# neka-nat/cupoch

Measured on AMD Instinct MI355X. Metric: ICP iterations/sec (incl. kNN) on 10M-pt point-to-plane, 1/2/4/8 MI355X, higher is better.
Workload: dtype f32; 1 GPU; 10M-vs-10M point-to-plane ICP, radius 1-NN on an 8-ary kd-cell tree, r=2*N^(-1/3), uniform random clouds (BASELINE.md section 3); points=10000000, parallelism=single GPU, accumulate=f64

## Files before the change

cupoch_amd/_lib.py:

```python
import ctypes as C
import os
import shutil
import subprocess

_HERE = os.path.dirname(os.path.abspath(__file__))
ROOT = os.path.dirname(_HERE)
CSRC = os.path.join(_HERE, "csrc")
LIB_DIR = os.path.join(_HERE, "lib")
LIB_PATH = os.path.join(LIB_DIR, "libmi_icp.so")
INCLUDE = os.path.join(ROOT, "include")

HIPCC_FLAGS = ["--offload-arch=gfx950", "-O3", "-std=c++17", "-ffp-contract=off", "-fPIC", "-I/opt/rocm/include"]
UNITS = ["mi_icp", "mi_build", "mi_geometry", "mi_voxel", "mi_rgbd", "mi_tsdf", "mi_knn", "mi_comm", "mi_debug"]
OBJ_DIR = os.path.join(LIB_DIR, "obj")

MI_ICP_HOST, MI_ICP_DEVICE = 0, 1
EST_POINT_TO_POINT, EST_POINT_TO_PLANE, EST_SYMMETRIC, EST_GENERALIZED = 1, 2, 3, 5
EST_COLORED = 4


class MiIcpError(RuntimeError):
    pass


def _sources():
    return sorted(os.path.join(CSRC, f) for f in os.listdir(CSRC)
                  if f.endswith((".hip", ".h"))) + [os.path.join(INCLUDE, "mi_icp.h"),
                                                 os.path.join(INCLUDE, "mi_icp_debug.h")]


def needs_build():
    if not os.path.exists(LIB_PATH):
        return True
    t = os.path.getmtime(LIB_PATH)
    return any(os.path.getmtime(s) > t for s in _sources())


def build(force=False, verbose=False, variant=None, defines=()):
    lib_path = LIB_PATH if not variant else os.path.join(LIB_DIR, "libmi_icp_%s.so" % variant)
    obj_dir = OBJ_DIR if not variant else OBJ_DIR + "_" + variant
    if not force and not variant and not needs_build():
        return LIB_PATH
    hipcc = shutil.which("hipcc") or "/opt/rocm/bin/hipcc"
    if not os.path.exists(hipcc):
        raise MiIcpError("hipcc not found; cannot build libmi_icp.so")
    os.makedirs(obj_dir, exist_ok=True)
    import fcntl
    import hashlib
    with open(os.path.join(LIB_DIR, ".build.lock"), "w") as lock:
        fcntl.flock(lock, fcntl.LOCK_EX)
        try:
            if not force and not variant and not needs_build():
                return LIB_PATH
            return _build_locked(hipcc, lib_path, obj_dir, force, verbose, tuple(defines), hashlib)
        finally:
            fcntl.flock(lock, fcntl.LOCK_UN)


def _build_locked(hipcc, lib_path, obj_dir, force, verbose, defines, hashlib):
    headers = [s for s in _sources() if s.endswith(".h")]
    newest_header = max(os.path.getmtime(h) for h in headers)
    flags_hash = hashlib.sha1(" ".join(HIPCC_FLAGS + list(defines)).encode()).hexdigest()
    stamp = os.path.join(obj_dir, "flags.stamp")
    if not (os.path.exists(stamp) and open(stamp).read().strip() == flags_hash):
        force = True

    def compile_unit(u):
        src, obj = os.path.join(CSRC, u + ".hip"), os.path.join(obj_dir, u + ".o")
        if not force and os.path.exists(obj) and os.path.getmtime(obj) > max(newest_header, os.path.getmtime(src)):
            return obj
        tmp = "%s.tmp.%d" % (obj, os.getpid())
        cmd = [hipcc] + HIPCC_FLAGS + list(defines) + ["-c", src, "-o", tmp]
        if verbose:
            print(" ".join(cmd[:-1] + [obj]), flush=True)
        subprocess.check_call(cmd)
        os.replace(tmp, obj)
        return obj

    from concurrent.futures import ThreadPoolExecutor
    with ThreadPoolExecutor(max_workers=len(UNITS)) as pool:
        objs = list(pool.map(compile_unit, UNITS))
    with open(stamp + ".tmp", "w") as f:
        f.write(flags_hash + "\n")
    os.replace(stamp + ".tmp", stamp)
    tmp = "%s.tmp.%d" % (lib_path, os.getpid())
    cmd = [hipcc, "--offload-arch=gfx950", "-shared", "-fPIC"] + objs + ["-o", tmp]
    if verbose:
        print(" ".join(cmd), flush=True)
    subprocess.check_call(cmd)
    os.replace(tmp, lib_path)
    return lib_path


ITERATION_FN = C.CFUNCTYPE(None, C.c_void_p, C.c_int, C.c_float, C.c_float)


class Params(C.Structure):
    _fields_ = [("relative_fitness", C.c_float), ("relative_rmse", C.c_float),
                ("max_iteration", C.c_int32), ("det_thresh", C.c_float)]


class Result(C.Structure):
    _fields_ = [("transformation", C.c_float * 16), ("fitness", C.c_float),
                ("inlier_rmse", C.c_float), ("n_correspondences", C.c_int64),
                ("iterations", C.c_int32), ("nn_passes", C.c_int32)]


class OdometryOption(C.Structure):
    _fields_ = [("num_levels", C.c_int32), ("iterations", C.c_int32 * 8), ("max_depth_diff", C.c_float),
                ("min_depth", C.c_float), ("max_depth", C.c_float), ("nu", C.c_float), ("sigma2_init", C.c_float),
                ("inv_sigma_mat_diag", C.c_float * 6)]


_P, _I, _L, _F = C.c_void_p, C.c_int, C.c_int64, C.c_float
SIGNATURES = {
    "mi_icp_create": (_I, [_I, C.POINTER(_P)]),
    "mi_icp_destroy": (None, [_P]),
    "mi_icp_last_error": (C.c_char_p, [_P]),
    "mi_icp_version": (C.c_char_p, []),
    "mi_icp_set_stream": (_I, [_P, _P]),
    "mi_icp_synchronize": (_I, [_P]),
    "mi_icp_set_target": (_I, [_P, _P, _P, _P, _L, _I]),
    "mi_icp_set_source": (_I, [_P, _P, _P, _P, _L, _I]),
    "mi_icp_search_radius_1nn": (_I, [_P, _P, _F, _P, _P, _I, _P]),
    "mi_icp_get_correspondences": (_I, [_P, _P, _L, C.POINTER(_L), _I]),
    "mi_icp_set_correspondences": (_I, [_P, _P, _L, _I]),
    "mi_icp_compute_system": (_I, [_P, _I, _P, _P]),
    "mi_icp_compute_transformation": (_I, [_P, _I, _P, _F, _P]),
    "mi_icp_compute_rmse": (_I, [_P, _I, _P, C.POINTER(_F)]),
    "mi_icp_solve_system": (_I, [_P, _F, _P]),
    "mi_icp_kabsch_from_sums": (_I, [_P, _L, _P]),
    "mi_icp_vector6_to_matrix4": (None, [_P, _P]),
    "mi_icp_lzf_decompress": (_L, [_P, _L, _P, _L]),
    "mi_icp_lzf_compress": (_L, [_P, _L, _P, _L]),
    "mi_icp_evaluate_registration": (_I, [_P, _F, _P, C.POINTER(Result)]),
    "mi_icp_registration_icp": (_I, [_P, _I, _F, _P, C.POINTER(Params), C.POINTER(Result)]),
    "mi_icp_icp_begin": (_I, [_P, _I, _F, _P, _F, C.POINTER(Result)]),
    "mi_icp_icp_iterate": (_I, [_P, _I, C.POINTER(Result)]),
    "mi_icp_transform": (_I, [_P, _P, _P, _P, _P, _L, _I]),
    "mi_icp_compute_bounds": (_I, [_P, _P, _L, _I, _P, _P, _P]),
    "mi_icp_affine": (_I, [_P, _P, _F, _I, _P, _P, _P, _P, _P, _L, _I]),
    "mi_icp_voxel_downsample": (_I, [_P, _P, _P, _P, _L, _F, _P, _P, _P, C.POINTER(_L), _I]),
    "mi_icp_select_by_index": (_I, [_P, _P, _P, _P, _L, _P, _L, _I, _P, _P, _P, C.POINTER(_L), _I]),
    "mi_icp_select_by_mask": (_I, [_P, _P, _P, _P, _L, _P, _L, _I, _P, _P, _P, C.POINTER(_L), _I]),
    "mi_icp_uniform_downsample": (_I, [_P, _P, _P, _P, _L, _L, _P, _P, _P, C.POINTER(_L), _I]),
    "mi_icp_remove_statistical_outliers": (_I, [_P, _P, _P, _P, _L, _I, _F, _P, _P, _P, _P, _P, C.POINTER(_L), _I]),
    "mi_icp_remove_radius_outliers": (_I, [_P, _P, _P, _P, _L, _I, _F, _P, _P, _P, _P, _P, C.POINTER(_L), _I]),
    "mi_icp_cluster_dbscan": (_I, [_P, _P, _L, _F, _L, _I, _P, _P, C.POINTER(_L), _I]),
    "mi_icp_segment_plane": (_I, [_P, _P, _L, _F, _L, _L, C.c_uint64, _P, _P, _P, C.POINTER(_L), C.POINTER(_L), C.POINTER(_L), _I]),
    "mi_icp_iss_keypoints": (_I, [_P, _P, _L, _F, _F, _F, _F, _I, _I, _P, _P, _P, _P, _P, C.POINTER(_L), _I]),
    "mi_icp_farthest_point_downsample": (_I, [_P, _P, _P, _P, _L, _L, _P, _P, _P, _P, C.POINTER(_L), _I]),
    "mi_icp_pass_through_filter": (_I, [_P, _P, _P, _P, _L, _I, _F, _F, _P, _P, _P, _P, C.POINTER(_L), _I]),
    "mi_icp_crop_aabb": (_I, [_P, _P, _P, _P, _L, _P, _P, _P, _P, _P, _P, C.POINTER(_L), _I]),
    "mi_icp_remove_none_finite": (_I, [_P, _P, _P, _P, _L, _I, _I, _P, _P, _P, _P, C.POINTER(_L), _I]),
    "mi_icp_gaussian_filter": (_I, [_P, _P, _P, _P, _L, _F, _F, _I, _P, _P, _P, _I]),
    "mi_icp_create_from_depth": (_I, [_P, _P, _I, _P, _I, _I, _I, _P, _P, _F, _F, _F, _I, _I, _I, _I,
                                      _P, _P, _P, C.POINTER(_L), _I]),
    "mi_icp_compute_rgbd_odometry": (_I, [_P, _P, _P, _P, _P, _I, _I, _P, _P, _I, _P, C.POINTER(_I), _P, _P, _I]),
    "mi_icp_compute_weighted_rgbd_odometry": (_I, [_P, _P, _P, _P, _P, _I, _I, _P, _P, _P, _P, C.POINTER(_I), _P, _P, _P, _I]),
    "mi_icp_tsdf_create": (_I, [_P, _F, _I, _F, _I, _P, C.POINTER(_P)]),
    "mi_icp_tsdf_destroy": (_I, [_P, _P]),
    "mi_icp_tsdf_reset": (_I, [_P, _P]),
    "mi_icp_tsdf_integrate": (_I, [_P, _P, _P, _I, _I, _I, _I, _P, _I, _I, _I, _I, _I, _I, _P, _P, _I]),
    "mi_icp_tsdf_extract_point_cloud": (_I, [_P, _P, _P, _P, _P, _L, C.POINTER(_L), _I]),
    "mi_icp_tsdf_extract_voxel_point_cloud": (_I, [_P, _P, _P, _P, _L, C.POINTER(_L), _I]),
    "mi_icp_tsdf_raycast": (_I, [_P, _P, _I, _I, _P, _P, _F, _I, _P, _P, _P, _L, C.POINTER(_L), _I]),
    "mi_icp_tsdf_get_voxels": (_I, [_P, _P, _P, _P, _P, _I]),
    "mi_icp_covariances_from_normals": (_I, [_P, _P, _L, _F, _P, _I]),
    "mi_icp_estimate_normals_knn": (_I, [_P, _P, _L, _I, _P, _I]),
    "mi_icp_estimate_normals_radius": (_I, [_P, _P, _L, _F, _I, _P, _I]),
    "mi_icp_search_knn": (_I, [_P, _P, _L, _I, _F, _P, _P, C.POINTER(_L), _I]),
    "mi_icp_set_target_colors": (_I, [_P, _P, _I]),
    "mi_icp_set_source_colors": (_I, [_P, _P, _I]),
    "mi_icp_set_lambda_geometric": (_I, [_P, _F]),
    "mi_icp_compute_color_gradients": (_I, [_P, _F, _I, _P, _I]),
    "mi_icp_registration_colored_icp": (_I, [_P, _F, _P, C.POINTER(Params), _F, C.POINTER(Result)]),
    "mi_icp_comm_unique_id": (_I, [_P]),
    "mi_icp_comm_init": (_I, [_P, _P, _I, _I]),
    "mi_icp_comm_init_local": (_I, [_P, C.c_char_p, _I, _I]),
    "mi_icp_comm_kind": (_I, [_P]),
    "mi_icp_comm_autotune": (_I, [_P, _I, _P, _P]),
    "mi_icp_comm_destroy": (_I, [_P]),
    "mi_icp_set_global_source_count": (_I, [_P, _L]),
    "mi_icp_spatial_order": (_I, [_P, _P, _L, _P, _I]),
    "mi_icp_set_iteration_callback": (_I, [_P, _P, _P]),
    "mi_icp_set_profiling": (_I, [_P, _I]),
    "mi_icp_get_profile": (_I, [_P, _P]),
    "mi_icp_debug_sort_pairs": (_I, [_P, _P, _P, _L, _I]),
    "mi_icp_debug_exclusive_scan": (_I, [_P, _P, _P, _L, _P]),
    "mi_icp_debug_morton_order": (_I, [_P, _P, _L, _P]),
    "mi_icp_debug_nn_stats": (_I, [_P, _P, _F, _I, _P]),
    "mi_icp_debug_nn_stats8": (_I, [_P, _P, _F, _I, _P]),
    "mi_icp_debug_get_tree": (_I, [_P, C.POINTER(_L), _P, _P]),
    "mi_icp_debug_drop_seeds": (_I, [_P]),
    "mi_icp_debug_last_search_kind": (_I, [_P]),
    "mi_icp_debug_last_voxel_path": (_I, [_P]),
    "mi_icp_debug_occupancy": (_I, [_I]),
    "mi_icp_debug_loop_counters": (_I, [_P, _P]),
    "mi_icp_debug_search_skip": (_I, [_P, _P, _P, _L, C.POINTER(_L), C.POINTER(_I)]),
    "mi_icp_debug_locate": (_I, [_P, _P, _P]),
    "mi_icp_debug_set_step_stamps": (_I, [_P, _I]),
    "mi_icp_debug_get_step_stamps": (_I, [_P, _P, C.POINTER(C.c_double)]),
    "mi_icp_debug_solve_both": (_I, [_I, _P, _I, C.c_float, _P, _P, _P, _P]),
    "mi_icp_debug_get_leaf_regions": (_I, [_P, _P]),
    "mi_icp_debug_get_leaf_halos": (_I, [_P, _P]),
    "mi_icp_debug_eigen3": (_I, [_I, _P, _L, _P, _P, _P]),
    "mi_icp_debug_odometry_image": (_I, [_P, _I, _I, _P, C.POINTER(_I), C.POINTER(_I)]),
}

_lib = None


def load():
    global _lib
    if _lib is not None:
        return _lib
    override = os.environ.get("MI_ICP_LIB_PATH")
    path = override or LIB_PATH
    if not os.path.exists(path):
        raise MiIcpError(
            "libmi_icp.so is not built (%s). Run `python -c 'import __graft_entry__ as g; "
            "g.build()'` or cupoch_amd._lib.build(); there is no CPU fallback." % LIB_PATH)
    try:
        lib = C.CDLL(path, mode=C.RTLD_GLOBAL)
    except OSError as e:
        raise MiIcpError("cannot load %s: %s" % (path, e))
    for name, (res, args) in SIGNATURES.items():
        if override and name.startswith("mi_icp_debug_") and not hasattr(lib, name):
            continue
        fn = getattr(lib, name)
        fn.restype = res
        fn.argtypes = args
    _lib = lib
    return lib
```

cupoch_amd/csrc/ctx.h:

```cpp
#pragma once
#include <hip/hip_runtime.h>
#include <rccl/rccl.h>

#include <algorithm>
#include <cmath>
#include <cstdarg>
#include <cstdio>
#include <cstdlib>
#include <cstring>
#include <string>
#include <vector>

#include "../../include/mi_icp.h"
#include "../../include/mi_icp_debug.h"
#include "device_utils.h"
#include "host_solver.h"
#include "loop.h"
#include "loop_policy.h"
#include "mailbox.h"
#include "primitives.h"

namespace mi {
namespace eng {

using host::Mat4;

struct DevBuf {
    void* p = nullptr;
    size_t bytes = 0;
};

}
}

struct mi_icp_ctx {
    int device = 0;
    hipStream_t stream = nullptr;
    std::string err;

    int64_t nt = 0;
    int nleaf = 0;
    int64_t nts = 0;
    uint32_t leaf_first = 1, nrecords = 0;
    bool t_has_nrm = false, t_has_cov = false, t_has_int = false, t_has_grad = false, t_has_rec = false;
    mi::eng::DevBuf tblk, tnrm, trec, tcov, tgrad, nodes, inv_t, tidx, thalo, tlinks_tmp;
    mi::eng::DevBuf cell_planes, cell_samples, cell_cstart, cell_gstart, cell_boxes, cell_hist;
    mi::eng::DevBuf gplanes;
    int cell_levels = -1;
    uint32_t* cell_total_host = nullptr;
    bool inv_t_valid = false;
    bool links_ready = false, links_allowed = false;
    hipStream_t side = nullptr;
    hipEvent_t ev_fork = nullptr, ev_links = nullptr;
    bool links_inflight = false;
    int last_search_kind = -1;
    int last_voxel_path = -1;
    mi::eng::HaloPolicy halo;
    bool halo_use = false;
    mi::eng::DevBuf halo_want;

    int64_t ns = 0, ns_global = 0;
    bool s_has_nrm = false, s_has_cov = false, s_has_int = false;
    float lambda_geometric = 0.968f;
    mi::eng::DevBuf sx, sy, sz, sperm, snrm, scov, sint, nn_idx, nn_d2, inv_s;
    mi::eng::DevBuf alt[9];
    bool inv_s_valid = false;
    bool nn_valid = false;
    mi::eng::DevBuf expiry;
    bool expiry_live = false;
    float skip_r2 = NAN;
    mi::eng::DevBuf src_bounds;
    mi::eng::Relocation relocate;

    mi::eng::DevBuf user_pairs;
    int64_t n_user_pairs = -1;

    mi::eng::DevBuf keys0, keys1, vals0, vals1, hist, scan_tmp, bounds_part, bounds;
    mi::eng::DevBuf partial, sys_dev, dense_idx, flags, pairs_out, seg_start;
    mi::eng::DevBuf stage[6];
    mi::eng::DevBuf tscale;
    mi::eng::DevBuf knn_idx, knn_flags;
    mi::eng::DevBuf dbs[4];
    mi::eng::DevBuf seg[4];
    float vx_refused_voxel = 0.0f;
    int64_t vx_refused_n = 0;
    int vx_order = 0;
    mi::eng::DevBuf vx_tab;
    mi::eng::DevBuf vpay[6];
    double* sys_host = nullptr;
    float* f_host = nullptr;
    uint32_t* u_host = nullptr;
    void* od_host = nullptr;
    int od_levels = 0, od_lw[MI_ICP_ODOMETRY_MAX_LEVELS] = {}, od_lh[MI_ICP_ODOMETRY_MAX_LEVELS] = {};
    const float* od_img[MI_ICP_ODOMETRY_MAX_LEVELS][8] = {};

    mi::eng::DevBuf loop_dev, ticket;
    mi::DevLoop* loop_host = nullptr;
    bool loop_active = false;
    mi_icp_iteration_fn iter_fn = nullptr;
    void* iter_user = nullptr;
    mi::eng::DevBuf loop_hist;
    float* hist_host = nullptr;
    int iter_reported = 0;
    float loop_r2 = 0.0f;
    int loop_est = 0;

    ncclComm_t comm = nullptr;
    int nranks = 1, rank = 0;
    mi::MailBox* mail_host = nullptr;
    mi::MailBox* mail_dev = nullptr;
    size_t mail_bytes = 0;
    std::string mail_name;
    bool mail_linked = false;
    unsigned long long* inbox = nullptr;
    unsigned long long* inbox_peer[mi::kMailRanks] = {};
    mi::eng::DevBuf inbox_table;
    bool comm_broken = false;
    int xchg = 0;
    uint32_t tune_epoch = 0;
    mi::eng::DevBuf mail_state;

    mi_icp_ctx* aux = nullptr;

    std::vector<mi_icp_tsdf*> tsdf_volumes;

    mi::eng::DevBuf stamps;
    bool stamps_on = false;
    bool profiling = false;
    static constexpr int kEvPairs = 16;
    hipEvent_t ev[4] = {nullptr, nullptr, nullptr, nullptr};
    hipEvent_t evp[2][kEvPairs][2] = {};
    int evp_n[2] = {0, 0};
    bool ev_pending_nn = false, ev_pending_red = false;
    double prof[8] = {0, 0, 0, 0, 0, 0, 0, 0};
};

namespace mi {
namespace eng {

inline float* lreg_of(const mi_icp_ctx* c) { return c->tblk.p ? (float*)c->tblk.p + mi::kLeafRegOffset : nullptr; }

inline int fail(mi_icp_ctx* c, int code, const char* fmt, ...) {
    char buf[512];
    va_list ap;
    va_start(ap, fmt);
    vsnprintf(buf, sizeof(buf), fmt, ap);
    va_end(ap);
    if (c) c->err = buf;
    return code;
}

#define HIPCHK(c, expr)                                                                       \
    do {                                                                                      \
        hipError_t e_ = (expr);                                                               \
        if (e_ != hipSuccess)                                                                 \
            return fail((c), MI_ICP_ERR_HIP, "%s failed: %s (%s:%d)", #expr,                  \
                        hipGetErrorString(e_), __FILE__, __LINE__);                           \
    } while (0)

#define KCHK(c) HIPCHK(c, hipGetLastError())

#define TRY(expr)                \
    do {                         \
        int rc_ = (expr);        \
        if (rc_ != MI_ICP_OK) return rc_; \
    } while (0)

template <class T>
int ensure(mi_icp_ctx* c, DevBuf& b, size_t count, T** out) {
    const size_t bytes = std::max<size_t>(count * sizeof(T), 256);
    if (b.bytes < bytes) {
        if (b.p) {
            HIPCHK(c, hipStreamSynchronize(c->stream));
            HIPCHK(c, hipFree(b.p));
            b.p = nullptr;
            b.bytes = 0;
        }
        HIPCHK(c, hipMalloc(&b.p, bytes));
        b.bytes = bytes;
    }
    *out = (T*)b.p;
    return MI_ICP_OK;
}

inline void release(DevBuf& b) {
    if (b.p) (void)hipFree(b.p);
    b.p = nullptr;
    b.bytes = 0;
}

template <class T>
int to_device(mi_icp_ctx* c, const T* src, size_t count, int mem_kind, DevBuf& stage,
              const T** out) {
    if (!src || count == 0) {
        *out = nullptr;
        return MI_ICP_OK;
    }
    if (mem_kind == MI_ICP_DEVICE) {
        *out = src;
        return MI_ICP_OK;
    }
    T* d;
    TRY(ensure(c, stage, count, &d));
    HIPCHK(c, hipMemcpyAsync(d, src, count * sizeof(T), hipMemcpyHostToDevice, c->stream));
    *out = d;
    return MI_ICP_OK;
}

template <class T>
int out_slot(mi_icp_ctx* c, T* dst, size_t count, int mem_kind, DevBuf& stage, T** out) {
    if (!dst || mem_kind == MI_ICP_DEVICE) {
        *out = dst;
        return MI_ICP_OK;
    }
    return ensure(c, stage, count, out);
}

template <class T>
int from_device(mi_icp_ctx* c, const T* dev, T* dst, size_t count, int mem_kind) {
    if (!dst || dst == dev || count == 0) return MI_ICP_OK;
    HIPCHK(c, hipMemcpyAsync(dst, dev, count * sizeof(T),
                             mem_kind == MI_ICP_DEVICE ? hipMemcpyDeviceToDevice
                                                       : hipMemcpyDeviceToHost,
                             c->stream));
    return MI_ICP_OK;
}

inline int drop_expiry(mi_icp_ctx* c) {
    c->skip_r2 = NAN;
    if (c->expiry_live && c->expiry.p) HIPCHK(c, hipMemsetAsync(c->expiry.p, 0xff, c->expiry.bytes, c->stream));
    c->expiry_live = false;
    return MI_ICP_OK;
}

static_assert(sizeof(DevLoop::live) == kSkipSamples, "loop_policy.h skip_pays reads DevLoop::live[]");

inline int blocks_for(int64_t n, int per = 256) { return (int)std::max<int64_t>(1, (n + per - 1) / per); }

inline Xform make_xform(const Mat4& T) { return xform_from(T); }

inline Mat4 load_T(const float* T) {
    if (!T) return host::identity4();
    Mat4 m;
    std::memcpy(m.data(), T, sizeof(float) * 16);
    return m;
}

struct EvTimer {
    mi_icp_ctx* c;
    int slot;
    hipEvent_t stop = nullptr;
    bool pooled;
    EvTimer(mi_icp_ctx* ctx, int s, bool in_loop) : c(ctx), slot(s), pooled(in_loop) {
        if (!c->profiling) return;
        if (pooled) {
            if (c->evp_n[slot] >= mi_icp_ctx::kEvPairs) return;
            const int i = c->evp_n[slot]++;
            (void)hipEventRecord(c->evp[slot][i][0], c->stream);
            stop = c->evp[slot][i][1];
        } else {
            (void)hipEventRecord(c->ev[slot * 2], c->stream);
            stop = c->ev[slot * 2 + 1];
        }
    }
    ~EvTimer() {
        if (!stop) return;
        (void)hipEventRecord(stop, c->stream);
        if (!pooled) (slot == 0 ? c->ev_pending_nn : c->ev_pending_red) = true;
    }
};

inline void collect_events(mi_icp_ctx* c) {
    float ms = 0.0f;
    if (c->ev_pending_nn && hipEventElapsedTime(&ms, c->ev[0], c->ev[1]) == hipSuccess) {
        c->prof[0] += ms;
        c->prof[1] += 1;
    }
    if (c->ev_pending_red && hipEventElapsedTime(&ms, c->ev[2], c->ev[3]) == hipSuccess) {
        c->prof[2] += ms;
        c->prof[3] += 1;
    }
    c->ev_pending_nn = c->ev_pending_red = false;
}

inline void collect_pooled(mi_icp_ctx* c, int executed) {
    for (int slot = 0; slot < 2; ++slot) {
        for (int i = 0; i < c->evp_n[slot] && i < executed; ++i) {
            float ms = 0.0f;
            if (hipEventElapsedTime(&ms, c->evp[slot][i][0], c->evp[slot][i][1]) == hipSuccess) {
                c->prof[slot * 2] += ms;
                c->prof[slot * 2 + 1] += 1;
            }
        }
        c->evp_n[slot] = 0;
    }
}

inline bool mail_on(const mi_icp_ctx* c) { return c->mail_dev != nullptr && (c->xchg == 1 || c->xchg == 2); }

inline int check_ctx(mi_icp_ctx* c) {
    if (!c) return MI_ICP_ERR_INVALID;
    hipError_t e = hipSetDevice(c->device);
    if (e != hipSuccess) return fail(c, MI_ICP_ERR_HIP, "hipSetDevice(%d): %s", c->device, hipGetErrorString(e));
    return MI_ICP_OK;
}

inline int check_ctx(mi_icp_ctx* c, int mem_kind, const char* what) {
    TRY(check_ctx(c));
    if (mem_kind != MI_ICP_HOST && mem_kind != MI_ICP_DEVICE) return fail(c, MI_ICP_ERR_INVALID, "%s: bad mem_kind", what);
    return MI_ICP_OK;
}

inline int check_sizes(mi_icp_ctx* c, const char* what, int64_t n, int64_t* m, int mem_kind) {
    TRY(check_ctx(c, mem_kind, what));
    if (!m) return fail(c, MI_ICP_ERR_INVALID, "%s: m is null", what);
    *m = 0;
    if (n < 0 || n > 0x7fffff00ll) return fail(c, MI_ICP_ERR_INVALID, "%s: bad size", what);
    return MI_ICP_OK;
}

struct Cloud {
    const float* in[3];
    float* out[3];
};

inline int cloud_check(mi_icp_ctx* c, const char* what, const Cloud& a) {
    if (!a.in[0] || !a.out[0] || (a.in[1] && !a.out[1]) || (a.in[2] && !a.out[2]))
        return fail(c, MI_ICP_ERR_INVALID, "%s: null buffer", what);
    return MI_ICP_OK;
}

inline int cloud_upload(mi_icp_ctx* c, Cloud* a, int64_t n, int mem_kind, DevBuf* stage) {
    for (int k = 0; k < 3; ++k) TRY(to_device(c, a->in[k], (size_t)n * 3, mem_kind, stage[k], &a->in[k]));
    return MI_ICP_OK;
}

inline int cloud_in(mi_icp_ctx* c, const char* what, Cloud* a, int64_t n, int mem_kind, DevBuf* stage) {
    TRY(cloud_check(c, what, *a));
    return cloud_upload(c, a, n, mem_kind, stage);
}

inline int cloud_out(mi_icp_ctx* c, const float* const in[3], float* const out[3], int64_t count, int mem_kind,
                     DevBuf* stage, float* dst[3]) {
    for (int k = 0; k < 3; ++k) TRY(out_slot(c, in[k] ? out[k] : nullptr, (size_t)count * 3, mem_kind, stage[k], &dst[k]));
    return MI_ICP_OK;
}

inline int cloud_out_back(mi_icp_ctx* c, float* const dst[3], float* const out[3], int64_t m, int mem_kind) {
    for (int k = 0; k < 3; ++k)
        if (dst[k]) TRY(from_device(c, (const float*)dst[k], out[k], (size_t)m * 3, mem_kind));
    return MI_ICP_OK;
}

template <class Launch>
int cloud_emit(mi_icp_ctx* c, const float* const in[3], float* const out[3], int64_t count, int64_t m, int mem_kind,
               DevBuf* stage, Launch launch) {
    float* dst[3];
    TRY(cloud_out(c, in, out, count, mem_kind, stage, dst));
    launch(dst);
    KCHK(c);
    TRY(cloud_out_back(c, dst, out, m, mem_kind));
    HIPCHK(c, hipStreamSynchronize(c->stream));
    return MI_ICP_OK;
}

inline int scan_into(mi_icp_ctx* c, const uint32_t* flags, uint32_t* pos, int64_t n, const uint32_t** total) {
    uint32_t* tmp;
    TRY(ensure(c, c->scan_tmp, (size_t)scan_num_tiles(n) + 2, &tmp));
    exclusive_scan_u32(c->stream, flags, pos, n, tmp);
    KCHK(c);
    *total = tmp + scan_num_tiles(n);
    return MI_ICP_OK;
}

inline int scan_flags(mi_icp_ctx* c, const uint32_t* flags, int64_t n, uint32_t** pos, const uint32_t** total) {
    TRY(ensure(c, c->dense_idx, (size_t)n, pos));
    return scan_into(c, flags, *pos, n, total);
}

inline int read_total(mi_icp_ctx* c, const uint32_t* total, int slot = 0) {
    HIPCHK(c, hipMemcpyAsync(c->u_host + slot, total, sizeof(uint32_t), hipMemcpyDeviceToHost, c->stream));
    return MI_ICP_OK;
}

template <class Launch>
int cloud_emit_counted(mi_icp_ctx* c, const char* what, const uint32_t* flags, int64_t n, float* const out_all[3],
                       const bool (&want)[3], int64_t capacity, int64_t* m, int mem_kind, Launch launch) {
    uint32_t* pos;
    const uint32_t* total;
    TRY(scan_flags(c, flags, n, &pos, &total));
    TRY(read_total(c, total));
    HIPCHK(c, hipStreamSynchronize(c->stream));
    const int64_t cnt = (int64_t)c->u_host[0];
    *m = cnt;
    if (cnt == 0 || capacity < cnt) return MI_ICP_OK;
    float* out[3];
    for (int k = 0; k < 3; ++k) {
        if (want[k] && !out_all[k]) return fail(c, MI_ICP_ERR_INVALID, "%s: null buffer", what);
        out[k] = want[k] ? out_all[k] : nullptr;
    }
    return cloud_emit(c, out, out, cnt, cnt, mem_kind, c->vpay, [&](float* const dst[3]) { launch(pos, dst); });
}

template <class Body>
int in_scratch(mi_icp_ctx* c, const char* what, Body body) {
    if (!c->aux) {
        const int rc = mi_icp_create(c->device, &c->aux);
        if (rc != MI_ICP_OK) return fail(c, rc, "%s: cannot create the scratch context", what);
    }
    mi_icp_ctx* a = c->aux;
    a->stream = c->stream;
    const int rc = body(a);
    if (rc != MI_ICP_OK) return fail(c, rc, "%s: %s", what, a->err.c_str());
    return MI_ICP_OK;
}

int compute_bounds(mi_icp_ctx* c, const float* pts, int64_t n, float** bounds_out);
int sort_buffers(mi_icp_ctx* c, int64_t n, SortBuffers* sb);
int morton_order(mi_icp_ctx* c, const float* pts, int64_t n, const uint32_t** order, const float* grid_bounds = nullptr,
                 int grid_bits = 0, float** own_bounds = nullptr);
int ensure_links(mi_icp_ctx* c);
int start_links_async(mi_icp_ctx* c);
bool halo_poll(mi_icp_ctx* c);
int drain_links(mi_icp_ctx* c);
void release_links_scratch(mi_icp_ctx* c);
int resort_source_by_match(mi_icp_ctx* c);
int occupancy_build(int which);
int launch_nn(mi_icp_ctx* c, const Mat4& T, float r2, bool seed, unsigned long long* stats = nullptr,
              const DevLoop* loop = nullptr);
int occupancy_loop(int which);
bool planes_available(const mi_icp_ctx* c);
int launch_locate_by_planes(mi_icp_ctx* c, const Xform& X, const DevLoop* loop, int gated);
int occupancy_geometry(int which);
void tsdf_release_all(mi_icp_ctx* c);
int compact_by_flags(mi_icp_ctx* c, const uint32_t* flags, int64_t n, const float* const in[3], float* const out[3],
                     int64_t* out_idx, int mem_kind, const uint32_t* status, int64_t* m, uint32_t* status_out);
MailArgs mail_args(const mi_icp_ctx* c);
void mailbox_close(mi_icp_ctx* c);
int comm_failed(mi_icp_ctx* c, const char* what);
int comm_usable(mi_icp_ctx* c);
int allreduce_system(mi_icp_ctx* c);
void comm_release(mi_icp_ctx* c);

}
}
```

cupoch_amd/csrc/mi_build.hip:

```cpp
#include "ctx.h"
#include "kd_build.h"
#include "kd_cells.h"
#include "kd_planes.h"
#include "kd_refine.h"
#include "lbvh.h"
#include "leaf_halo.h"

using namespace mi;
using namespace mi::eng;
using host::Mat4;

namespace mi {
namespace eng {

int morton_bits_for(int64_t n) {
    int lg = 0;
    while ((1ll << lg) < n) ++lg;
    const int per_axis = (lg + 2) / 3;
    const int fine = std::min(21, std::max(6, per_axis + 2));
    const int coarse = (((3 * fine + 7) / 8 - 1) * 8) / 3;
    return coarse >= std::max(6, per_axis) ? coarse : fine;
}

int compute_bounds(mi_icp_ctx* c, const float* pts, int64_t n, float** bounds_out) {
// ... 129 lines not shown
    if (ngroups <= 0 || ngroups > (int64_t)ncells + n / kKdGroup + 1)
        return fail(c, MI_ICP_ERR_HIP, "kd cell layout: implausible group count %lld", (long long)ngroups);
    out->vals = sb.vals[cur];
    out->cstart = cstart;
    out->gstart = gstart;
    out->ncells = ncells;
    out->ngroups = ngroups;
    out->planes = planes;
    out->levels = lv;
    return MI_ICP_OK;
}

int build_links(mi_icp_ctx* c, hipStream_t st) {
    if (!c->links_allowed) return MI_ICP_OK;
    float* halo;
    const size_t ntiles = ((size_t)c->nleaf + 63) / 64;
    TRY(ensure(c, c->thalo, ntiles * 64 * kHaloLines * kHaloLineFloats, &halo));
    uint2* cand;
    TRY(ensure(c, c->tlinks_tmp, ntiles * 64 * kLinkCand, &cand));
    const uint32_t lblocks = (uint32_t)ntiles;
    leaf_halo_collect<<<((lblocks + 7u) / 8u) * 8u, 64, 0, st>>>(
            (const float*)c->nodes.p, c->leaf_first, c->nleaf, lblocks, lreg_of(c), cand);
    KCHK(c);
    leaf_halo_build<<<(unsigned)(((size_t)c->nleaf + kHaloTile - 1) / kHaloTile), 64, 0, st>>>(lreg_of(c), c->nleaf, cand, (const float*)c->tblk.p, halo);
    KCHK(c);
    return MI_ICP_OK;
}

int ensure_links(mi_icp_ctx* c) {
    if (c->nt <= 0) return MI_ICP_OK;
    if (c->links_inflight) {
        HIPCHK(c, hipStreamWaitEvent(c->stream, c->ev_links, 0));
        c->links_inflight = false;
        c->links_ready = true;
    }
    if (c->links_ready) return MI_ICP_OK;
    TRY(build_links(c, c->stream));
    c->links_ready = true;
    return MI_ICP_OK;
}

void release_links_scratch(mi_icp_ctx* c) {
    constexpr size_t kKeepBelow = (size_t)64 << 20;
    if (c->links_ready && !c->links_inflight && c->tlinks_tmp.p && c->tlinks_tmp.bytes >= kKeepBelow) release(c->tlinks_tmp);
}

bool halo_poll(mi_icp_ctx* c) {
    if (c->links_inflight && hipEventQuery(c->ev_links) == hipSuccess) {
        c->links_inflight = false;
        c->links_ready = true;
    }
    (void)hipGetLastError();
    return c->links_ready && c->links_allowed && c->thalo.p != nullptr;
}

int start_links_async(mi_icp_ctx* c) {
    if (c->nt <= 0 || c->links_ready || c->links_inflight || !c->links_allowed) return MI_ICP_OK;
    HIPCHK(c, hipEventRecord(c->ev_fork, c->stream));
    HIPCHK(c, hipStreamWaitEvent(c->side, c->ev_fork, 0));
    TRY(build_links(c, c->side));
    HIPCHK(c, hipEventRecord(c->ev_links, c->side));
    c->links_inflight = true;
    return MI_ICP_OK;
}

int drain_links(mi_icp_ctx* c) {
    if (c->links_inflight) {
        HIPCHK(c, hipStreamWaitEvent(c->stream, c->ev_links, 0));
        HIPCHK(c, hipStreamSynchronize(c->side));
        c->links_inflight = false;
    }
    c->links_ready = false;
    return MI_ICP_OK;
}

int resort_source_by_match(mi_icp_ctx* c) {
    const int64_t n = c->ns;
    if (n <= 0 || c->nt <= 0 || !c->nn_valid) return MI_ICP_OK;
    TRY(drop_expiry(c));
    SortBuffers sb;
    TRY(sort_buffers(c, n, &sb));
    int bits = 1;
    while (bits < 32 && (1ull << bits) <= (uint64_t)c->nleaf) ++bits;
    match_order_keys<<<blocks_for(n), 256, 0, c->stream>>>((const int32_t*)c->nn_idx.p, (int)n, (uint32_t)c->nleaf,
                                                           (uint32_t*)sb.keys[0], sb.vals[0]);
    KCHK(c);
    const uint32_t* ord = sb.vals[radix_sort_pairs<uint32_t>(c->stream, sb, n, bits)];
    KCHK(c);
    SourceArrays in, out;
    in.sx = (float*)c->sx.p; in.sy = (float*)c->sy.p; in.sz = (float*)c->sz.p;
    in.sperm = (int32_t*)c->sperm.p;
    in.snrm = c->s_has_nrm ? (float4*)c->snrm.p : nullptr;
    in.scov = c->s_has_cov ? (float*)c->scov.p : nullptr;
    in.sint = c->s_has_int ? (float*)c->sint.p : nullptr;
    in.nn_idx = (int32_t*)c->nn_idx.p; in.nn_d2 = (float*)c->nn_d2.p;
    TRY(ensure(c, c->alt[0], (size_t)n, &out.sx));
    TRY(ensure(c, c->alt[1], (size_t)n, &out.sy));
    TRY(ensure(c, c->alt[2], (size_t)n, &out.sz));
    TRY(ensure(c, c->alt[3], (size_t)n, &out.sperm));
    TRY(ensure(c, c->alt[4], (size_t)n, &out.nn_idx));
    TRY(ensure(c, c->alt[5], (size_t)n, &out.nn_d2));
    out.snrm = nullptr;
    out.scov = nullptr;
    out.sint = nullptr;
    if (in.snrm) TRY(ensure(c, c->alt[6], (size_t)n, &out.snrm));
    if (in.scov) TRY(ensure(c, c->alt[7], (size_t)n * 9, &out.scov));
    if (in.sint) TRY(ensure(c, c->alt[8], (size_t)n, &out.sint));
    permute_source<<<blocks_for(n), 256, 0, c->stream>>>(ord, (int)n, in, out);
    KCHK(c);
    std::swap(c->sx, c->alt[0]);
    std::swap(c->sy, c->alt[1]);
    std::swap(c->sz, c->alt[2]);
    std::swap(c->sperm, c->alt[3]);
    std::swap(c->nn_idx, c->alt[4]);
    std::swap(c->nn_d2, c->alt[5]);
    if (in.snrm) std::swap(c->snrm, c->alt[6]);
    if (in.scov) std::swap(c->scov, c->alt[7]);
    if (in.sint) std::swap(c->sint, c->alt[8]);
    c->inv_s_valid = false;
    return MI_ICP_OK;
}

int occupancy_build(int which) {
    int blocks = -1;
    hipError_t e = hipErrorInvalidValue;
    if (which == 0) e = hipOccupancyMaxActiveBlocksPerMultiprocessor(&blocks, kd_build_groups, kKdThreads, 0);
    else if (which == 4) e = hipOccupancyMaxActiveBlocksPerMultiprocessor(&blocks, leaf_halo_build, 64, 0);
    else return -1;
    return e == hipSuccess ? blocks : -2;
}

}
}

extern "C" {

int mi_icp_set_target(mi_icp_ctx* c, const float* xyz, const float* normals, const float* covs,
                      int64_t n, int mem_kind) {
    TRY(check_ctx(c, mem_kind, "set_target"));
    if (n < 0 || n > 0x7fffff00ll || (n > 0 && !xyz)) return fail(c, MI_ICP_ERR_INVALID, "set_target: bad size/pointer");
    TRY(drain_links(c));
    TRY(drop_expiry(c));
    c->nt = 0;
    c->inv_t_valid = false;
    c->nn_valid = false;
    c->n_user_pairs = -1;
    c->loop_active = false;
    c->t_has_nrm = normals != nullptr && n > 0;
    c->t_has_cov = covs != nullptr && n > 0;
    c->t_has_int = c->t_has_grad = false;
    c->t_has_rec = false;
    if (n == 0) return MI_ICP_OK;
    hipEvent_t e0 = c->ev[2], e1 = c->ev[3];
    if (c->profiling) {
        (void)hipStreamSynchronize(c->stream);
        collect_events(c);
        (void)hipEventRecord(e0, c->stream);
    }

    const float *d_pts, *d_nrm, *d_cov;
    TRY(to_device(c, xyz, (size_t)n * 3, mem_kind, c->stage[0], &d_pts));
    TRY(to_device(c, normals, (size_t)n * 3, mem_kind, c->stage[1], &d_nrm));
    TRY(to_device(c, covs, (size_t)n * 9, mem_kind, c->stage[2], &d_cov));

    CellLayout lay;
    TRY(kd_cell_layout(c, d_pts, n, &lay));
    const int64_t nts = lay.ngroups * kKdGroup;

    const int nleaf = (int)((nts + kLeaf - 1) / kLeaf);
    int levels = 1;
    uint32_t leaf_first = 1u;
    while ((uint64_t)leaf_first * 8u < (uint64_t)nleaf) {
        leaf_first *= 8u;
        ++levels;
    }
    if (levels > kMaxLevels) return fail(c, MI_ICP_ERR_INVALID, "set_target: cloud too large for the 64-bit traversal stack");
    const uint32_t used_last = (uint32_t)((nleaf + 7) / 8);
    const uint32_t nrecords = full_levels_below(leaf_first) + used_last;
    if ((uint64_t)nrecords * kRecordFloats * sizeof(float) >= (1ull << 32))
        return fail(c, MI_ICP_ERR_INVALID, "set_target: cloud too large for 32-bit record offsets");
    float* tblk;
    float4* tnrm = nullptr;
    float* tcov = nullptr;
    float* nodes;
    TRY(ensure(c, c->tblk, (size_t)nleaf * kLeafFloats, &tblk));
    TRY(ensure(c, c->nodes, (size_t)nrecords * kRecordFloats, &nodes));
    float* lreg = tblk + kLeafRegOffset;
    int32_t* tidx;
    TRY(ensure(c, c->tidx, (size_t)nleaf * kLeaf, &tidx));
    float* trec = nullptr;
    if (d_nrm) TRY(ensure(c, c->tnrm, (size_t)nts, &tnrm));
    if (d_nrm) TRY(ensure(c, c->trec, (size_t)nts * 6, &trec));
    c->t_has_rec = trec != nullptr;
    if (d_cov) TRY(ensure(c, c->tcov, (size_t)nts * 9, &tcov));
    const uint32_t upper_flag = (lay.ngroups == (int64_t)lay.ncells) ? 1u : 0u;
    GroupBuildArgs ga;
    ga.pts = d_pts;
    ga.nrm = d_nrm;
    ga.cov = d_cov;
    ga.vals = lay.vals;
    ga.cstart = lay.cstart;
    ga.gstart = lay.gstart;
    ga.ncells = lay.ncells;
    ga.planes = lay.planes;
    ga.cell_levels = lay.levels;
    ga.ngroups = (uint32_t)lay.ngroups;
    ga.leaf_first = leaf_first;
    ga.tblk = tblk;
    ga.tnrm = tnrm;
    ga.trec = trec;
    ga.tcov = tcov;
    ga.records = nodes;
    ga.lreg = lreg;
    ga.tidx = tidx;
    TRY(ensure(c, c->gplanes, (size_t)lay.ngroups * 512, &ga.gplanes));
    ga.link_delta = 0.25f;
    ga.region_margin = 0.5f;
    kd_build_groups<<<(unsigned)lay.ngroups, kKdThreads, 0, c->stream>>>(ga);
    KCHK(c);
    uint32_t first = leaf_first >> 9;
    uint32_t used = ((uint32_t)lay.ngroups + 7u) / 8u;
    int above_groups = 1;
    for (; first > 1u; first /= 8u, ++above_groups) {
        const uint32_t count = ((used + 7u) / 8u) * 8u;
        const int region_depth = cell_depth(lay.levels) - 3 * above_groups;
        const uint32_t flag = (upper_flag && (!cell_tri(lay.levels) || region_depth >= 2)) ? 1u : 0u;
        build_level<<<blocks_for(count), 256, 0, c->stream>>>(nodes, first, used, count, flag, lay.planes,
                                                              lay.levels, region_depth);
        KCHK(c);
        used = (used + 7u) / 8u;
    }
    {
        float* ts;
        TRY(ensure(c, c->tscale, 4, &ts));
        HIPCHK(c, hipMemsetAsync(ts, 0, 16, c->stream));
        tree_scale<<<std::min(256u, (used_last + 255u) / 256u), 256, 0, c->stream>>>(nodes, leaf_first, used_last, ts);
        KCHK(c);
    }
    c->links_ready = false;
    c->halo.on_new_target();
    c->links_allowed = (uint32_t)nleaf <= kLinkIdMask;
    c->nt = n;
    c->nts = nts;
    c->nleaf = nleaf;
    c->leaf_first = leaf_first;
    c->nrecords = nrecords;
    c->cell_levels = lay.levels;
    if (c->halo.start_ahead(n, c->links_allowed)) TRY(start_links_async(c));
    if (c->profiling) {
        (void)hipEventRecord(e1, c->stream);
        (void)hipStreamSynchronize(c->stream);
        float ms = 0;
        if (hipEventElapsedTime(&ms, e0, e1) == hipSuccess) c->prof[4] = ms;
    }
    return MI_ICP_OK;
}

int mi_icp_set_source(mi_icp_ctx* c, const float* xyz, const float* normals, const float* covs,
                      int64_t n, int mem_kind) {
    TRY(check_ctx(c, mem_kind, "set_source"));
    if (n < 0 || n > 0x7fffff00ll || (n > 0 && !xyz)) return fail(c, MI_ICP_ERR_INVALID, "set_source: bad size/pointer");
    c->ns = 0;
    c->inv_s_valid = false;
    c->nn_valid = false;
    c->n_user_pairs = -1;
    c->loop_active = false;
    c->s_has_nrm = normals != nullptr && n > 0;
    c->s_has_cov = covs != nullptr && n > 0;
    c->s_has_int = false;
    if (c->nranks == 1) c->ns_global = 0;
    if (n == 0) return MI_ICP_OK;
    hipEvent_t e0 = c->ev[2], e1 = c->ev[3];
    if (c->profiling) {
        (void)hipStreamSynchronize(c->stream);
        collect_events(c);
        (void)hipEventRecord(e0, c->stream);
    }

    const float *d_pts, *d_nrm, *d_cov;
    TRY(to_device(c, xyz, (size_t)n * 3, mem_kind, c->stage[3], &d_pts));
    TRY(to_device(c, normals, (size_t)n * 3, mem_kind, c->stage[4], &d_nrm));
    TRY(to_device(c, covs, (size_t)n * 9, mem_kind, c->stage[5], &d_cov));

    const uint32_t* order;
    float* own_bounds = nullptr;
    TRY(morton_order(c, d_pts, n, &order, nullptr, 0, &own_bounds));
    {
        float* sb;
        TRY(ensure(c, c->src_bounds, 8, &sb));
        HIPCHK(c, hipMemcpyAsync(sb, own_bounds, 8 * sizeof(float), hipMemcpyDeviceToDevice, c->stream));
    }

    float *sx, *sy, *sz, *scov = nullptr, *d2;
    int32_t *sperm, *idx;
    float4* snrm = nullptr;
    TRY(ensure(c, c->sx, (size_t)n, &sx));
    TRY(ensure(c, c->sy, (size_t)n, &sy));
    TRY(ensure(c, c->sz, (size_t)n, &sz));
    TRY(ensure(c, c->sperm, (size_t)n, &sperm));
    TRY(ensure(c, c->nn_idx, (size_t)n, &idx));
    TRY(ensure(c, c->nn_d2, (size_t)n, &d2));
    {
        double* lim;
        TRY(ensure(c, c->expiry, (size_t)((n + 63) / 64), &lim));
        c->expiry_live = true;
        TRY(drop_expiry(c));
    }
    if (d_nrm) TRY(ensure(c, c->snrm, (size_t)n, &snrm));
    if (d_cov) TRY(ensure(c, c->scov, (size_t)n * 9, &scov));
    gather_source<<<blocks_for(n), 256, 0, c->stream>>>(order, d_pts, d_nrm, d_cov, (int)n, sx, sy, sz,
                                                        sperm, snrm, scov);
    KCHK(c);
    c->ns = n;
    if (c->profiling) {
        (void)hipEventRecord(e1, c->stream);
        (void)hipStreamSynchronize(c->stream);
        float ms = 0;
        if (hipEventElapsedTime(&ms, e0, e1) == hipSuccess) c->prof[5] = ms;
    }
    return MI_ICP_OK;
}

int mi_icp_spatial_order(mi_icp_ctx* c, const float* xyz, int64_t n, uint32_t* order_out, int mem_kind) {
    TRY(check_ctx(c, mem_kind, "spatial_order"));
    if (n < 0 || n > 0x7fffff00ll || (n > 0 && (!xyz || !order_out)))
        return fail(c, MI_ICP_ERR_INVALID, "spatial_order: bad arguments");
    if (n == 0) return MI_ICP_OK;
    const float* d_pts;
    TRY(to_device(c, xyz, (size_t)n * 3, mem_kind, c->stage[0], &d_pts));
    const uint32_t* order;
    TRY(morton_order(c, d_pts, n, &order));
    TRY(from_device(c, order, order_out, (size_t)n, mem_kind));
    HIPCHK(c, hipStreamSynchronize(c->stream));
    return MI_ICP_OK;
}

int mi_icp_debug_morton_order(mi_icp_ctx* c, const float* xyz, int64_t n, uint32_t* order_out) {
    if (n <= 0) return fail(c, MI_ICP_ERR_INVALID, "debug_morton_order: bad arguments");
    return mi_icp_spatial_order(c, xyz, n, order_out, MI_ICP_HOST);
}

}
```

cupoch_amd/csrc/mi_debug.hip:

```cpp
#include "ctx.h"
#include <vector>
#include "halo_format.h"
#include "traverse.h"
#include "wave_solver.h"
#include "eigen3.h"

using namespace mi;
using namespace mi::eng;
using host::Mat4;

namespace mi {
__global__ __launch_bounds__(64) void solve_both_kernel(const double* systems, float det_thresh, float* out_serial,
                                                        float* out_wave, int32_t* ok_serial, int32_t* ok_wave) {
    __shared__ double s_sys[32];
    const int n = (int)blockIdx.x;
    if (threadIdx.x < 32) s_sys[threadIdx.x] = systems[(int64_t)n * 32 + threadIdx.x];
    __syncthreads();
    host::Mat4 W;
    const bool okw = wave_solve_system(s_sys, det_thresh, W);
    if (threadIdx.x < 16) out_wave[(int64_t)n * 16 + threadIdx.x] = select16(W.m, (int)threadIdx.x);
    if (threadIdx.x == 0) {
        ok_wave[n] = okw ? 1 : 0;
        host::Mat4 S;
        ok_serial[n] = host::solve_system(s_sys, det_thresh, S) ? 1 : 0;
        for (int e = 0; e < 16; ++e) out_serial[(int64_t)n * 16 + e] = S.m[e];
    }
}
__host__ __device__ inline void eigen3_one(const float* A9, float* eval, float* evec, float* S) {
    M3 A;
    for (int r = 0; r < 3; ++r)
        for (int c = 0; c < 3; ++c) A.m[r][c] = A9[r * 3 + c];
    float ev[3], e[3][3], s[3][3];
    fast_eigen3x3(A, ev, e);
    gicp_weight(A, s);
    for (int k = 0; k < 3; ++k) {
        if (eval) eval[k] = ev[k];
        for (int d = 0; d < 3; ++d) {
            if (evec) evec[d * 3 + k] = e[k][d];
            if (S) S[k * 3 + d] = s[k][d];
        }
    }
}
__global__ __launch_bounds__(256) void eigen3_kernel(const float* A, int64_t n, float* eval, float* evec, float* S) {
    const int64_t i = (int64_t)blockIdx.x * blockDim.x + threadIdx.x;
    if (i < n) eigen3_one(A + 9 * i, eval ? eval + 3 * i : nullptr, evec ? evec + 9 * i : nullptr, S ? S + 9 * i : nullptr);
}
}

extern "C" {

int mi_icp_debug_sort_pairs(mi_icp_ctx* c, uint64_t* keys, uint32_t* vals, int64_t n, int key_bits) {
    TRY(check_ctx(c));
    if (n < 0 || key_bits < 1 || key_bits > 64 || (n > 0 && (!keys || !vals)))
        return fail(c, MI_ICP_ERR_INVALID, "debug_sort_pairs: bad arguments");
    if (n == 0) return MI_ICP_OK;
    SortBuffers sb;
    TRY(sort_buffers(c, n, &sb));
    HIPCHK(c, hipMemcpyAsync(sb.keys[0], keys, (size_t)n * 8, hipMemcpyHostToDevice, c->stream));
    HIPCHK(c, hipMemcpyAsync(sb.vals[0], vals, (size_t)n * 4, hipMemcpyHostToDevice, c->stream));
    const int cur = radix_sort_pairs<uint64_t>(c->stream, sb, n, key_bits);
    KCHK(c);
    HIPCHK(c, hipMemcpyAsync(keys, sb.keys[cur], (size_t)n * 8, hipMemcpyDeviceToHost, c->stream));
    HIPCHK(c, hipMemcpyAsync(vals, sb.vals[cur], (size_t)n * 4, hipMemcpyDeviceToHost, c->stream));
    HIPCHK(c, hipStreamSynchronize(c->stream));
    return MI_ICP_OK;
}

int mi_icp_debug_exclusive_scan(mi_icp_ctx* c, const uint32_t* in, uint32_t* out, int64_t n,
                                uint64_t* total) {
    TRY(check_ctx(c));
    if (n < 0 || (n > 0 && (!in || !out))) return fail(c, MI_ICP_ERR_INVALID, "debug_exclusive_scan: bad arguments");
    if (total) *total = 0;
    if (n == 0) return MI_ICP_OK;
    uint32_t* d;
    const uint32_t* sum;
    TRY(ensure(c, c->flags, (size_t)n, &d));
    HIPCHK(c, hipMemcpyAsync(d, in, (size_t)n * 4, hipMemcpyHostToDevice, c->stream));
    TRY(scan_into(c, d, d, n, &sum));
    HIPCHK(c, hipMemcpyAsync(out, d, (size_t)n * 4, hipMemcpyDeviceToHost, c->stream));
    TRY(read_total(c, sum));
    HIPCHK(c, hipStreamSynchronize(c->stream));
    if (total) *total = c->u_host[0];
    return MI_ICP_OK;
}

int mi_icp_debug_nn_stats8(mi_icp_ctx* c, const float* T, float radius, int use_seed, uint64_t* out8) {
    TRY(check_ctx(c));
    if (!out8 || c->ns <= 0 || c->nt <= 0) return fail(c, MI_ICP_ERR_INVALID, "debug_nn_stats: bad state/arguments");
    unsigned long long* d;
    TRY(ensure(c, c->flags, 16, (unsigned long long**)&d));
    HIPCHK(c, hipMemsetAsync(d, 0, 16 * sizeof(unsigned long long), c->stream));
    TRY(launch_nn(c, load_T(T), radius * radius, use_seed != 0, d));
    HIPCHK(c, hipMemcpyAsync(c->sys_host, d, 16 * sizeof(unsigned long long), hipMemcpyDeviceToHost, c->stream));
    HIPCHK(c, hipStreamSynchronize(c->stream));
    collect_events(c);
    std::memcpy(out8, c->sys_host, 8 * sizeof(uint64_t));
    return MI_ICP_OK;
}

int mi_icp_debug_nn_stats(mi_icp_ctx* c, const float* T, float radius, int use_seed, uint64_t* out4) {
    uint64_t all[8];
    if (!out4) return MI_ICP_ERR_INVALID;
    TRY(mi_icp_debug_nn_stats8(c, T, radius, use_seed, all));
    std::memcpy(out4, all, 4 * sizeof(uint64_t));
    return MI_ICP_OK;
}

int mi_icp_debug_get_leaf_regions(mi_icp_ctx* c, float* regions_out) {
    TRY(check_ctx(c));
    if (!regions_out || c->nt <= 0) return fail(c, MI_ICP_ERR_INVALID, "debug_get_leaf_regions: no target / bad arguments");
    HIPCHK(c, hipMemcpy2DAsync(regions_out, kLeafRegFloats * sizeof(float), lreg_of(c), kLeafRegStride * sizeof(float),
                               kLeafRegFloats * sizeof(float), (size_t)c->nleaf, hipMemcpyDeviceToHost, c->stream));
    HIPCHK(c, hipStreamSynchronize(c->stream));
    return MI_ICP_OK;
}

int mi_icp_debug_get_leaf_halos(mi_icp_ctx* c, float* halos_out) {
    TRY(check_ctx(c));
    if (!halos_out || c->nt <= 0) return fail(c, MI_ICP_ERR_INVALID, "debug_get_leaf_halos: no target / bad arguments");
    TRY(ensure_links(c));
    const size_t count = (size_t)c->nleaf * kHaloLines * kHaloLineFloats;
    if (!c->thalo.p) {
        std::memset(halos_out, 0, count * sizeof(float));
        return MI_ICP_OK;
    }
    HIPCHK(c, hipMemcpyAsync(halos_out, c->thalo.p, count * sizeof(float), hipMemcpyDeviceToHost, c->stream));
    HIPCHK(c, hipStreamSynchronize(c->stream));
    return MI_ICP_OK;
}

int mi_icp_debug_last_search_kind(const mi_icp_ctx* c) { return c ? c->last_search_kind : -1; }
int mi_icp_debug_last_voxel_path(const mi_icp_ctx* c) { return c ? c->last_voxel_path : -1; }

int mi_icp_debug_occupancy(int which) {
    if (which == 0 || which == 4) return occupancy_build(which);
    if (which >= 1 && which <= 3) return occupancy_loop(which);
    if (which >= 5 && which <= 8) return occupancy_geometry(which);
    return -1;
}

int mi_icp_debug_solve_both(int device, const double* systems, int n, float det_thresh, float* out_serial,
                            float* out_wave, int32_t* ok_serial, int32_t* ok_wave) {
    if (!systems || n <= 0 || !out_serial || !out_wave || !ok_serial || !ok_wave) return MI_ICP_ERR_INVALID;
    if (hipSetDevice(device) != hipSuccess) return MI_ICP_ERR_NO_DEVICE;
    double* d_sys = nullptr;
    float* d_out = nullptr;
    int32_t* d_ok = nullptr;
    int rc = MI_ICP_ERR_HIP;
    if (hipMalloc(&d_sys, (size_t)n * 32 * sizeof(double)) == hipSuccess &&
        hipMalloc(&d_out, (size_t)n * 32 * sizeof(float)) == hipSuccess &&
        hipMalloc(&d_ok, (size_t)n * 2 * sizeof(int32_t)) == hipSuccess &&
        hipMemcpy(d_sys, systems, (size_t)n * 32 * sizeof(double), hipMemcpyHostToDevice) == hipSuccess) {
        mi::solve_both_kernel<<<n, 64>>>(d_sys, det_thresh, d_out, d_out + (size_t)n * 16, d_ok, d_ok + n);
        if (hipDeviceSynchronize() == hipSuccess &&
            hipMemcpy(out_serial, d_out, (size_t)n * 16 * sizeof(float), hipMemcpyDeviceToHost) == hipSuccess &&
            hipMemcpy(out_wave, d_out + (size_t)n * 16, (size_t)n * 16 * sizeof(float), hipMemcpyDeviceToHost) == hipSuccess &&
            hipMemcpy(ok_serial, d_ok, (size_t)n * sizeof(int32_t), hipMemcpyDeviceToHost) == hipSuccess &&
            hipMemcpy(ok_wave, d_ok + n, (size_t)n * sizeof(int32_t), hipMemcpyDeviceToHost) == hipSuccess)
            rc = MI_ICP_OK;
    }
    (void)hipFree(d_sys);
    (void)hipFree(d_out);
    (void)hipFree(d_ok);
    return rc;
}

int mi_icp_debug_set_step_stamps(mi_icp_ctx* c, int enable) {
    TRY(check_ctx(c));
    c->stamps_on = enable != 0;
    return MI_ICP_OK;
}

int mi_icp_debug_get_step_stamps(mi_icp_ctx* c, uint64_t* out32, double* ticks_per_us) {
    TRY(check_ctx(c));
    if (!out32 || !c->stamps.p) return fail(c, MI_ICP_ERR_STATE, "debug_get_step_stamps: no stamped loop has run on this context");
    HIPCHK(c, hipStreamSynchronize(c->stream));
    HIPCHK(c, hipMemcpy(out32, c->stamps.p, sizeof(uint64_t) * kStampWords, hipMemcpyDeviceToHost));
    if (ticks_per_us) {
        int khz = 0;
        *ticks_per_us = (hipDeviceGetAttribute(&khz, hipDeviceAttributeWallClockRate, c->device) == hipSuccess && khz > 0) ? khz / 1000.0 : 100.0;
    }
    return MI_ICP_OK;
}

int mi_icp_debug_loop_counters(mi_icp_ctx* c, int32_t* out4) {
    TRY(check_ctx(c));
    if (!out4 || !c->loop_host) return fail(c, MI_ICP_ERR_INVALID, "debug_loop_counters: bad arguments");
    HIPCHK(c, hipStreamSynchronize(c->stream));
    out4[0] = c->loop_host->iterations;
    out4[1] = c->loop_host->passes;
    out4[2] = c->loop_host->relocations;
    out4[3] = c->relocate.armed ? 1 : 0;
    return MI_ICP_OK;
}

int mi_icp_debug_drop_seeds(mi_icp_ctx* c) {
    TRY(check_ctx(c));
    c->nn_valid = false;
    return drop_expiry(c);
}

int mi_icp_debug_search_skip(mi_icp_ctx* c, double* state2, double* limits_out, int64_t capacity, int64_t* npackets, int* armed) {
    TRY(check_ctx(c));
    if (!state2 || !npackets || !armed || capacity < 0) return fail(c, MI_ICP_ERR_INVALID, "debug_search_skip: bad arguments");
    if (!c->loop_active || !c->loop_dev.p || !c->expiry.p || c->ns <= 0)
        return fail(c, MI_ICP_ERR_STATE, "debug_search_skip: no registration loop on this context");
    const int64_t n = (c->ns + 63) / 64;
    *npackets = n;
    *armed = (c->expiry_live && c->skip_r2 == c->loop_r2 && skip_pays(c->loop_host->live, c->ns)) ? 1 : 0;
    const char* st = (const char*)c->loop_dev.p;
    HIPCHK(c, hipMemcpyAsync(state2, st + offsetof(DevLoop, travel), sizeof(double), hipMemcpyDeviceToHost, c->stream));
    HIPCHK(c, hipMemcpyAsync(state2 + 1, st + offsetof(DevLoop, fuzz), sizeof(double), hipMemcpyDeviceToHost, c->stream));
    if (limits_out && capacity >= n)
        HIPCHK(c, hipMemcpyAsync(limits_out, c->expiry.p, (size_t)n * sizeof(double), hipMemcpyDeviceToHost, c->stream));
    HIPCHK(c, hipStreamSynchronize(c->stream));
    return MI_ICP_OK;
}

int mi_icp_debug_locate(mi_icp_ctx* c, const float* T, int32_t* leaf_out) {
    TRY(check_ctx(c));
    if (!leaf_out || c->ns <= 0 || c->nt <= 0) return fail(c, MI_ICP_ERR_INVALID, "debug_locate: bad state/arguments");
    if (!planes_available(c)) return fail(c, MI_ICP_ERR_INVALID, "debug_locate: this tree has no split planes");
    TRY(drop_expiry(c));
    TRY(launch_locate_by_planes(c, make_xform(load_T(T)), nullptr, 0));
    c->nn_valid = true;
    c->n_user_pairs = -1;
    std::vector<int32_t> seeds((size_t)c->ns), perm((size_t)c->ns);
    HIPCHK(c, hipMemcpyAsync(seeds.data(), c->nn_idx.p, sizeof(int32_t) * (size_t)c->ns, hipMemcpyDeviceToHost, c->stream));
    HIPCHK(c, hipMemcpyAsync(perm.data(), c->sperm.p, sizeof(int32_t) * (size_t)c->ns, hipMemcpyDeviceToHost, c->stream));
    HIPCHK(c, hipStreamSynchronize(c->stream));
    for (int64_t i = 0; i < c->ns; ++i) leaf_out[perm[(size_t)i]] = seeds[(size_t)i] >> 3;
    return MI_ICP_OK;
}

int mi_icp_debug_get_tree(mi_icp_ctx* c, int64_t* info5, float* records_out, float* leaf_lines_out) {
    TRY(check_ctx(c));
    if (!info5 || c->nt <= 0) return fail(c, MI_ICP_ERR_INVALID, "debug_get_tree: no target / bad arguments");
    info5[0] = c->nts;
    info5[1] = c->nleaf;
    info5[2] = (int64_t)c->leaf_first;
    info5[3] = (int64_t)c->nrecords;
    info5[4] = c->nt;
    if (records_out)
        HIPCHK(c, hipMemcpyAsync(records_out, c->nodes.p, (size_t)c->nrecords * kRecordFloats * sizeof(float),
                                 hipMemcpyDeviceToHost, c->stream));
    if (leaf_lines_out) {
        HIPCHK(c, hipMemcpyAsync(leaf_lines_out, c->tblk.p, (size_t)c->nleaf * kLeafFloats * sizeof(float),
                                 hipMemcpyDeviceToHost, c->stream));
        HIPCHK(c, hipMemcpy2DAsync(leaf_lines_out + kLeafRegOffset, kLeafFloats * sizeof(float), c->tidx.p, kLeaf * sizeof(int32_t),
                                   kLeaf * sizeof(int32_t), (size_t)c->nleaf, hipMemcpyDeviceToHost, c->stream));
    }
    HIPCHK(c, hipStreamSynchronize(c->stream));
    return MI_ICP_OK;
}

int mi_icp_debug_odometry_image(mi_icp_ctx* c, int level, int which, float* out, int* width, int* height) {
    TRY(check_ctx(c));
    if (c->od_levels <= 0) return fail(c, MI_ICP_ERR_INVALID, "debug_odometry_image: no odometry call has run on this context");
    if (level < 0 || level >= c->od_levels || which < 0 || which > 7)
        return fail(c, MI_ICP_ERR_INVALID, "debug_odometry_image: level %d / image %d out of range", level, which);
    if (width) *width = c->od_lw[level];
    if (height) *height = c->od_lh[level];
    if (!out) return MI_ICP_OK;
    const size_t n = (size_t)c->od_lw[level] * c->od_lh[level];
    HIPCHK(c, hipMemcpyAsync(out, c->od_img[level][which], n * sizeof(float), hipMemcpyDeviceToHost, c->stream));
    HIPCHK(c, hipStreamSynchronize(c->stream));
    return MI_ICP_OK;
}

int mi_icp_debug_eigen3(int device, const float* A, int64_t n, float* eval, float* evec, float* S) {
    if (n < 0 || (n > 0 && !A)) return MI_ICP_ERR_INVALID;
    if (n == 0) return MI_ICP_OK;
    if (device < 0) {
        for (int64_t i = 0; i < n; ++i)
            eigen3_one(A + 9 * i, eval ? eval + 3 * i : nullptr, evec ? evec + 9 * i : nullptr, S ? S + 9 * i : nullptr);
        return MI_ICP_OK;
    }
    if (hipSetDevice(device) != hipSuccess) return MI_ICP_ERR_NO_DEVICE;
    float *dA = nullptr, *de = nullptr, *dv = nullptr, *dS = nullptr;
    int rc = MI_ICP_ERR_HIP;
    if (hipMalloc(&dA, (size_t)n * 36) == hipSuccess && hipMalloc(&de, (size_t)n * 12) == hipSuccess &&
        hipMalloc(&dv, (size_t)n * 36) == hipSuccess && hipMalloc(&dS, (size_t)n * 36) == hipSuccess &&
        hipMemcpy(dA, A, (size_t)n * 36, hipMemcpyHostToDevice) == hipSuccess) {
        hipLaunchKernelGGL(eigen3_kernel, dim3((unsigned)((n + 255) / 256)), dim3(256), 0, 0, dA, n, de, dv, dS);
        bool ok = hipDeviceSynchronize() == hipSuccess;
        if (ok && eval) ok = hipMemcpy(eval, de, (size_t)n * 12, hipMemcpyDeviceToHost) == hipSuccess;
        if (ok && evec) ok = hipMemcpy(evec, dv, (size_t)n * 36, hipMemcpyDeviceToHost) == hipSuccess;
        if (ok && S) ok = hipMemcpy(S, dS, (size_t)n * 36, hipMemcpyDeviceToHost) == hipSuccess;
        if (ok) rc = MI_ICP_OK;
    }
    (void)hipFree(dA);
    (void)hipFree(de);
    (void)hipFree(dv);
    (void)hipFree(dS);
    return rc;
}

}
```

cupoch_amd/csrc/mi_icp.hip:

```cpp
#include "ctx.h"
#include "fused_small.h"
#include "lzf.h"
#include "nn_search.h"
#include "reduce.h"

using namespace mi;
using namespace mi::eng;
using host::Mat4;

namespace mi {

static __global__ __launch_bounds__(kStepThreads) void loop_step_kernel(DevLoop* st_g, double* sys_in, int resume, MailArgs mail) {
    __shared__ DevLoop st_s;
    loop_step_block(st_g, sys_in, resume, st_s, StepPre{false, 0u, 0.0, 0u}, mail);
}

namespace eng {

constexpr int64_t kPt2PlTwoFrom = (int64_t)4 << 20;

static int64_t coarse_first_min() {
    static const int64_t v = [] { const char* s = std::getenv("MI_ICP_COARSE_MIN"); return s ? std::atoll(s) : (int64_t)1 << 16; }();
    return v;
}

bool planes_available(const mi_icp_ctx* c) {
    return c->cell_levels >= 0 && c->gplanes.p != nullptr && c->cell_planes.p != nullptr && c->cell_gstart.p != nullptr &&
           c->leaf_first > 1u && c->nleaf > 0;
}

int launch_locate_by_planes(mi_icp_ctx* c, const Xform& X, const DevLoop* loop, int gated) {
    const int grid = (int)std::min<int64_t>(blocks_for(c->ns), 8192);
    locate_by_planes<<<grid, 256, 0, c->stream>>>((const float*)c->sx.p, (const float*)c->sy.p, (const float*)c->sz.p, (int)c->ns,
                                                 (const float2*)c->cell_planes.p, c->cell_levels, (const uint32_t*)c->cell_gstart.p,
                                                 (const float2*)c->gplanes.p, (uint32_t)c->nleaf, X, loop, gated, (int32_t*)c->nn_idx.p,
                                                 (double*)c->expiry.p);
    KCHK(c);
    return MI_ICP_OK;
}

static int loop_halo(mi_icp_ctx* c, bool* have_halo, uint32_t** want) {
    static const bool always_wait = std::getenv("MI_ICP_WAIT_LINKS") != nullptr;
    if (always_wait) {
        TRY(start_links_async(c));
        TRY(ensure_links(c));
        c->halo_use = halo_poll(c);
    }
    *have_halo = c->halo_use;
    *want = (!*have_halo && !c->links_inflight && c->links_allowed) ? (uint32_t*)c->halo_want.p : nullptr;
    return MI_ICP_OK;
}

struct PacketGrid { uint32_t npackets, nblocks, grid; };
static PacketGrid packet_grid(int64_t ns, uint32_t per_block) {
    const uint32_t npackets = (uint32_t)((ns + 63) / 64);
    const uint32_t nblocks = (npackets + per_block - 1) / per_block;
    return PacketGrid{npackets, nblocks, ((nblocks + 7u) / 8u) * 8u};
}

static decltype(&nn_packet_kernel<false, false>) nn_kernel(bool seeded, bool stats, bool stamp, bool gate) {
    if (gate) return stamp ? nn_packet_kernel<true, false, true, true> : nn_packet_kernel<true, false, false, true>;
    if (stats) return seeded ? nn_packet_kernel<true, true> : nn_packet_kernel<false, true>;
    if (seeded && stamp) return nn_packet_kernel<true, false, true>;
    return seeded ? nn_packet_kernel<true, false> : nn_packet_kernel<false, false>;
}

int launch_nn(mi_icp_ctx* c, const Mat4& T, float r2, bool seed, unsigned long long* stats, const DevLoop* loop) {
    if (c->ns <= 0) return MI_ICP_OK;
    int32_t* idx = (int32_t*)c->nn_idx.p;
    if (c->nt <= 0) {
        TRY(drop_expiry(c));
        fill_i32<<<blocks_for(c->ns), 256, 0, c->stream>>>(idx, c->ns, -1);
        KCHK(c);
        c->nn_valid = true;
        c->n_user_pairs = -1;
        return MI_ICP_OK;
    }
    const Xform X = make_xform(T);
    bool have_halo;
    uint32_t* want = nullptr;
    if (loop) {
        TRY(loop_halo(c, &have_halo, &want));
    } else {
        if (seed && c->nn_valid) TRY(ensure_links(c));
        have_halo = halo_poll(c);
    }
    EvTimer t(c, 0, loop != nullptr);
    const SearchPlan p = plan_search(loop != nullptr, seed, c->nn_valid, stats != nullptr, c->ns, coarse_first_min(), have_halo, planes_available(c),
                                     c->expiry.p != nullptr, c->expiry_live, c->skip_r2, r2, c->loop_host->live, kSkipRun);
    if (!p.may_skip) TRY(drop_expiry(c));
    if (p.self_seeded) TRY(launch_locate_by_planes(c, X, loop, 0));
    c->last_search_kind = p.kind;
    const PacketGrid g = packet_grid(c->ns, p.run);
    nn_kernel(p.use_seed || p.self_seeded, stats != nullptr, loop && c->stamps_on, p.run > 1u)<<<g.grid, kNNThreads, 0, c->stream>>>(
            (const float*)c->sx.p, (const float*)c->sy.p, (const float*)c->sz.p, (int)c->ns, (const float*)c->nodes.p,
            (const float*)c->tblk.p, (const float*)lreg_of(c), have_halo ? (const float*)c->thalo.p : nullptr, c->leaf_first,
            X, loop, r2, g.nblocks, idx, loop ? nullptr : (float*)c->nn_d2.p, stats, want,
            p.limits ? (double*)c->expiry.p : nullptr,
            p.limits ? reinterpret_cast<uint8_t*>(c->loop_dev.p) + offsetof(DevLoop, live) : nullptr, skip_live_shift(c->ns), p.run);
    KCHK(c);
    if (p.limits) c->expiry_live = true, c->skip_r2 = r2;
    c->nn_valid = true;
    c->n_user_pairs = -1;
    return MI_ICP_OK;
}

int occupancy_loop(int which) {
    int blocks = -1;
    hipError_t e = hipErrorInvalidValue;
    if (which == 1) e = hipOccupancyMaxActiveBlocksPerMultiprocessor(&blocks, nn_packet_kernel<true, false>, kNNThreads, 0);
    else if (which == 2) e = hipOccupancyMaxActiveBlocksPerMultiprocessor(&blocks, nn_packet_kernel<false, false>, kNNThreads, 0);
    else if (which == 3) e = hipOccupancyMaxActiveBlocksPerMultiprocessor(&blocks, reduce_pt2pl_kernel<2, 1>, kReduceThreads, 0);
    else return -1;
    return e == hipSuccess ? blocks : -2;
}

}
}

namespace {

int ensure_inverse_maps(mi_icp_ctx* c) {
    if (!c->inv_s_valid && c->ns > 0) {
        int32_t* inv;
        TRY(ensure(c, c->inv_s, (size_t)c->ns, &inv));
        invert_perm_source<<<blocks_for(c->ns), 256, 0, c->stream>>>((const int32_t*)c->sperm.p, (int)c->ns, inv);
        KCHK(c);
        c->inv_s_valid = true;
    }
    if (!c->inv_t_valid && c->nt > 0) {
        int32_t* inv;
        TRY(ensure(c, c->inv_t, (size_t)c->nt, &inv));
        HIPCHK(c, hipMemsetAsync(inv, 0xff, sizeof(int32_t) * (size_t)c->nt, c->stream));
        invert_perm_target<<<blocks_for(c->nts), 256, 0, c->stream>>>((const int32_t*)c->tidx.p, (int)c->nts, inv);
        KCHK(c);
        c->inv_t_valid = true;
    }
    return MI_ICP_OK;
}

constexpr int kReduceElemsPerThread = 16;


bool known_estimator(int est) {
    return est == kEstP2P || est == kEstPt2Pl || est == kEstSym || est == kEstColored || est == kEstGICP;
}

bool estimator_ready(const mi_icp_ctx* c, int est) {
    switch (est) {
        case kEstP2P: return true;
        case kEstPt2Pl: return c->t_has_nrm;
        case kEstSym: return c->t_has_nrm && c->s_has_nrm;
        case kEstGICP: return c->t_has_cov && c->s_has_cov;
        case kEstColored:
            return c->t_has_nrm && c->t_has_int && c->t_has_grad && c->s_has_int;
        default: return false;
    }
}

int reduce_buffers(mi_icp_ctx* c, size_t rows, double** partial, double** sys, uint32_t** ticket) {
    TRY(ensure(c, c->partial, rows * kSysSize, partial));
    TRY(ensure(c, c->sys_dev, kSysSize, sys));
    if (!c->ticket.p) {
        TRY(ensure(c, c->ticket, 64, ticket));
        HIPCHK(c, hipMemsetAsync(*ticket, 0, 256, c->stream));
    }
    *ticket = (uint32_t*)c->ticket.p;
    return MI_ICP_OK;
}

bool pt2pl_reduction(const mi_icp_ctx* c, int est, int mode) {
    return est == kEstPt2Pl && mode == 0 && estimator_ready(c, est) && c->n_user_pairs < 0 && c->t_has_rec &&
           c->trec.p != nullptr && c->ns > 0 && c->nt > 0 && c->nn_valid;
}

template <int kU>
decltype(&reduce_pt2pl_kernel<kU, 0>) pt2pl_kernel(int step, bool stamp) {
    if (step == 2) return stamp ? reduce_pt2pl_kernel<kU, 2, true> : reduce_pt2pl_kernel<kU, 2>;
    if (step == 1) return stamp ? reduce_pt2pl_kernel<kU, 1, true> : reduce_pt2pl_kernel<kU, 1>;
    return reduce_pt2pl_kernel<kU, 0>;
}

template <int MODE>
decltype(&reduce_kernel<kEstP2P, MODE>) generic_reduce_kernel(int est) {
    switch (est) {
        case kEstP2P: return reduce_kernel<kEstP2P, MODE>;
        case kEstPt2Pl: return reduce_kernel<kEstPt2Pl, MODE>;
        case kEstSym: return reduce_kernel<kEstSym, MODE>;
        case kEstColored: return reduce_kernel<kEstColored, MODE>;
        case kEstGICP: return reduce_kernel<kEstGICP, MODE>;
        default: return nullptr;
    }
}

int launch_reduce(mi_icp_ctx* c, int est, int mode, const Mat4& T, DevLoop* loop = nullptr, int step = 0) {
    double *partial, *sys;
    uint32_t* ticket;
    TRY(reduce_buffers(c, kReduceBlocks, &partial, &sys, &ticket));
    ReduceArgs a;
    a.sx = (const float*)c->sx.p;
    a.sy = (const float*)c->sy.p;
    a.sz = (const float*)c->sz.p;
    a.snrm = (const float4*)c->snrm.p;
    a.scov = (const float*)c->scov.p;
    a.tblk = (const float*)c->tblk.p;
    a.tnrm = (const float4*)c->tnrm.p;
    a.trec = c->t_has_rec ? (const float*)c->trec.p : nullptr;
    a.tcov = (const float*)c->tcov.p;
    a.tgrad = (const float4*)c->tgrad.p;
    a.sint = (const float*)c->sint.p;
    a.sqrt_lambda_geometric = std::sqrt(c->lambda_geometric);
    a.sqrt_lambda_photometric = std::sqrt(1.0f - c->lambda_geometric);
    a.nn_idx = (const int32_t*)c->nn_idx.p;
    a.pairs = nullptr;
    a.inv_s = a.inv_t = nullptr;
    a.ns = (int)c->ns;
    a.nt = (int)c->nt;
    a.count = c->ns;
    if (c->n_user_pairs >= 0) {
        TRY(ensure_inverse_maps(c));
        a.pairs = (const int32_t*)c->user_pairs.p;
        a.inv_s = (const int32_t*)c->inv_s.p;
        a.inv_t = (const int32_t*)c->inv_t.p;
        a.count = c->n_user_pairs;
    }
    if (c->ns <= 0 || c->nt <= 0 || (!a.pairs && !c->nn_valid)) a.count = 0;
    const int64_t wide = std::min<int64_t>(256, blocks_for(a.count, kReduceThreads));
    const int grid = (int)std::max<int64_t>(
            wide, std::min<int64_t>(kReduceBlocks, blocks_for(a.count, kReduceThreads * kReduceElemsPerThread)));
    const Xform X = make_xform(T);
    if (pt2pl_reduction(c, est, mode)) {
        const auto kernel = (a.count >= kPt2PlTwoFrom) ? pt2pl_kernel<2>(step, c->stamps_on) : pt2pl_kernel<4>(step, c->stamps_on);
        EvTimer t(c, 1, loop != nullptr);
        kernel<<<std::min(grid, 512), kReduceThreads, 0, c->stream>>>(a, X, loop, partial, ticket, sys,
                                                                     (step == 2) ? mail_args(c) : MailArgs{});
        KCHK(c);
        return MI_ICP_OK;
    }
    if (!estimator_ready(c, est)) {
        est = kEstP2P;
        mode = 1;
    }
    const auto kernel = mode ? generic_reduce_kernel<1>(est) : generic_reduce_kernel<0>(est);
    if (!kernel) return fail(c, MI_ICP_ERR_INVALID, "unknown estimation type %d", est);
    EvTimer t(c, 1, loop != nullptr);
    kernel<<<grid, kReduceThreads, 0, c->stream>>>(a, X, loop, partial, ticket, sys);
    KCHK(c);
    return MI_ICP_OK;
}

int fetch_system(mi_icp_ctx* c, double* out) {
    double* sys = (double*)c->sys_dev.p;
    TRY(allreduce_system(c));
    HIPCHK(c, hipMemcpyAsync(c->sys_host, sys, kSysSize * sizeof(double), hipMemcpyDeviceToHost, c->stream));
    const bool mail = mail_on(c);
    int32_t* err_host = reinterpret_cast<int32_t*>(c->sys_host + 40);
    if (mail) HIPCHK(c, hipMemcpyAsync(err_host, (const int32_t*)c->mail_state.p + 1, sizeof(int32_t), hipMemcpyDeviceToHost, c->stream));
    HIPCHK(c, hipStreamSynchronize(c->stream));
    collect_events(c);
    if (mail && *err_host) return comm_failed(c, "the ranks' exchange timed out (mailbox): a peer did not post its sums");
    std::memcpy(out, c->sys_host, kSysSize * sizeof(double));
    return MI_ICP_OK;
}

Mat4 solve_update(const mi_icp_ctx* c, int est, const double* sys, float det_thresh) {
    const int64_t n_model = c->ns_global > 0 ? c->ns_global : c->ns;
    return mi::solve_update(est, estimator_ready(c, est), sys, det_thresh, n_model);
}

void stats_from_system(const mi_icp_ctx* c, const double* sys, float* fitness, float* rmse) {
    mi::stats_from_system(sys, c->ns_global > 0 ? c->ns_global : c->ns, fitness, rmse);
}

}

extern "C" {

const char* mi_icp_version(void) { return "mi_icp 0.1 (gfx950)"; }

int mi_icp_create(int device, mi_icp_ctx** out) {
    if (!out) return MI_ICP_ERR_INVALID;
    *out = nullptr;
    int count = 0;
    if (hipGetDeviceCount(&count) != hipSuccess || count <= 0 || device < 0 || device >= count)
        return MI_ICP_ERR_NO_DEVICE;
    if (hipSetDevice(device) != hipSuccess) return MI_ICP_ERR_NO_DEVICE;
    mi_icp_ctx* c = new mi_icp_ctx();
    c->device = device;
    bool ok = hipHostMalloc((void**)&c->sys_host, 64 * sizeof(double), hipHostMallocDefault) == hipSuccess &&
              hipHostMalloc((void**)&c->f_host, 64 * sizeof(float), hipHostMallocDefault) == hipSuccess &&
              hipHostMalloc((void**)&c->u_host, (16 + kWantSlots) * sizeof(uint32_t), hipHostMallocDefault) == hipSuccess;
    ok = ok && hipHostMalloc((void**)&c->loop_host, sizeof(DevLoop), hipHostMallocDefault) == hipSuccess;
    for (int i = 0; i < 4 && ok; ++i) ok = hipEventCreate(&c->ev[i]) == hipSuccess;
    int prio_least = 0, prio_greatest = 0;
    (void)hipDeviceGetStreamPriorityRange(&prio_least, &prio_greatest);
    ok = ok && hipStreamCreateWithPriority(&c->side, hipStreamNonBlocking, prio_least) == hipSuccess &&
         hipEventCreateWithFlags(&c->ev_fork, hipEventDisableTiming) == hipSuccess &&
         hipEventCreateWithFlags(&c->ev_links, hipEventDisableTiming) == hipSuccess;
    for (int k = 0; k < 2 && ok; ++k)
        for (int i = 0; i < mi_icp_ctx::kEvPairs && ok; ++i)
            ok = hipEventCreate(&c->evp[k][i][0]) == hipSuccess && hipEventCreate(&c->evp[k][i][1]) == hipSuccess;
    if (!ok) {
        mi_icp_destroy(c);
        return MI_ICP_ERR_HIP;
    }
    *out = c;
    return MI_ICP_OK;
}

void mi_icp_destroy(mi_icp_ctx* c) {
    if (!c) return;
    (void)hipSetDevice(c->device);
    (void)hipStreamSynchronize(c->stream);
    if (c->aux) mi_icp_destroy(c->aux);
    tsdf_release_all(c);
    if (c->side) {
        (void)hipStreamSynchronize(c->side);
        (void)hipStreamDestroy(c->side);
    }
    if (c->ev_fork) (void)hipEventDestroy(c->ev_fork);
    if (c->ev_links) (void)hipEventDestroy(c->ev_links);
    comm_release(c);
    DevBuf* all[] = {&c->trec, &c->tidx, &c->thalo, &c->tlinks_tmp, &c->halo_want, &c->loop_hist, &c->tblk, &c->tnrm, &c->tcov, &c->tgrad, &c->sint, &c->nodes, &c->inv_t, &c->cell_planes, &c->cell_samples, &c->cell_cstart,
                     &c->cell_gstart, &c->sx, &c->sy, &c->sz,
                     &c->sperm, &c->snrm, &c->scov, &c->nn_idx, &c->nn_d2, &c->expiry, &c->inv_s,
                     &c->user_pairs, &c->keys0, &c->keys1, &c->vals0, &c->vals1, &c->hist,
                     &c->scan_tmp, &c->bounds_part, &c->bounds, &c->partial, &c->sys_dev,
                     &c->dense_idx, &c->flags, &c->pairs_out, &c->seg_start, &c->loop_dev, &c->ticket, &c->mail_state, &c->alt[0],
                     &c->alt[1], &c->alt[2], &c->alt[3], &c->alt[4], &c->alt[5], &c->alt[6], &c->alt[7], &c->alt[8], &c->stage[0],
                     &c->stage[1], &c->stage[2], &c->stage[3], &c->stage[4], &c->stage[5], &c->knn_idx, &c->tscale, &c->vpay[0], &c->vpay[1],
                     &c->vpay[2], &c->vpay[3], &c->vpay[4], &c->vpay[5], &c->stamps, &c->knn_flags, &c->gplanes, &c->src_bounds, &c->cell_boxes, &c->cell_hist, &c->vx_tab,
                     &c->dbs[0], &c->dbs[1], &c->dbs[2], &c->dbs[3], &c->seg[0], &c->seg[1], &c->seg[2], &c->seg[3]};
    for (DevBuf* b : all) release(*b);
    if (c->sys_host) (void)hipHostFree(c->sys_host);
    if (c->cell_total_host) (void)hipHostFree(c->cell_total_host);
    if (c->f_host) (void)hipHostFree(c->f_host);
    if (c->u_host) (void)hipHostFree(c->u_host);
    if (c->od_host) (void)hipHostFree(c->od_host);
    if (c->loop_host) (void)hipHostFree(c->loop_host);
    if (c->hist_host) (void)hipHostFree(c->hist_host);
    for (int k = 0; k < 2; ++k)
        for (int i = 0; i < mi_icp_ctx::kEvPairs; ++i)
            for (int e = 0; e < 2; ++e)
                if (c->evp[k][i][e]) (void)hipEventDestroy(c->evp[k][i][e]);
    for (int i = 0; i < 4; ++i)
        if (c->ev[i]) (void)hipEventDestroy(c->ev[i]);
    delete c;
}

const char* mi_icp_last_error(const mi_icp_ctx* c) { return c ? c->err.c_str() : "null context"; }

int mi_icp_set_iteration_callback(mi_icp_ctx* c, mi_icp_iteration_fn fn, void* user) {
    if (!c) return MI_ICP_ERR_INVALID;
    c->iter_fn = fn;
    c->iter_user = user;
    return MI_ICP_OK;
}

int mi_icp_set_stream(mi_icp_ctx* c, void* hip_stream) {
    if (c && c->aux) c->aux->stream = (hipStream_t)hip_stream;
    TRY(check_ctx(c));
    HIPCHK(c, hipStreamSynchronize(c->stream));
    c->stream = (hipStream_t)hip_stream;
    return MI_ICP_OK;
}

int mi_icp_synchronize(mi_icp_ctx* c) {
    TRY(check_ctx(c));
    HIPCHK(c, hipStreamSynchronize(c->stream));
    collect_events(c);
    return MI_ICP_OK;
}

int mi_icp_set_profiling(mi_icp_ctx* c, int enable) {
    TRY(check_ctx(c));
    c->profiling = enable != 0;
    for (double& v : c->prof) v = 0.0;
    c->ev_pending_nn = c->ev_pending_red = false;
    return MI_ICP_OK;
}

int mi_icp_get_profile(mi_icp_ctx* c, double* out8) {
    if (!c || !out8) return MI_ICP_ERR_INVALID;
    std::memcpy(out8, c->prof, sizeof(c->prof));
    return MI_ICP_OK;
}

int mi_icp_set_global_source_count(mi_icp_ctx* c, int64_t n_total) {
    if (!c || n_total < 0) return MI_ICP_ERR_INVALID;
    c->ns_global = n_total;
    return MI_ICP_OK;
}

static int export_dense_idx(mi_icp_ctx* c, int32_t** dense_out) {
    int32_t* dense;
    TRY(ensure(c, c->dense_idx, (size_t)std::max<int64_t>(c->ns, 1), &dense));
    if (c->ns > 0) {
        export_dense<<<blocks_for(c->ns), 256, 0, c->stream>>>(
                (const int32_t*)c->nn_idx.p, (const float*)c->nn_d2.p, (const int32_t*)c->sperm.p,
                (const int32_t*)c->tidx.p, (int)c->ns, dense, nullptr);
        KCHK(c);
    }
    *dense_out = dense;
    return MI_ICP_OK;
}

int mi_icp_search_radius_1nn(mi_icp_ctx* c, const float* T, float radius, int32_t* idx_out,
                             float* d2_out, int mem_kind, double* stats) {
    TRY(check_ctx(c, mem_kind, "search"));
    if (c->ns <= 0) return fail(c, MI_ICP_ERR_STATE, "search: no source set");
    const Mat4 M = load_T(T);
    const float r2 = radius * radius;
    TRY(launch_nn(c, M, r2, true));
    if (c->nt <= 0) {
        float* d2 = (float*)c->nn_d2.p;
        fill_i32<<<blocks_for(c->ns), 256, 0, c->stream>>>((int32_t*)d2, c->ns, 0x7f800000);
        KCHK(c);
    }
    if (idx_out || d2_out) {
        int32_t* dense;
        float* dense_d2 = nullptr;
        TRY(ensure(c, c->dense_idx, (size_t)c->ns, &dense));
        if (d2_out) TRY(ensure(c, c->flags, (size_t)c->ns, (float**)&dense_d2));
        export_dense<<<blocks_for(c->ns), 256, 0, c->stream>>>(
                (const int32_t*)c->nn_idx.p, (const float*)c->nn_d2.p, (const int32_t*)c->sperm.p,
                (const int32_t*)c->tidx.p, (int)c->ns, dense, dense_d2);
        KCHK(c);
        TRY(from_device(c, dense, idx_out, (size_t)c->ns, mem_kind));
        if (d2_out) TRY(from_device(c, dense_d2, d2_out, (size_t)c->ns, mem_kind));
    }
    if (stats) {
        double sys[kSysSize];
        TRY(launch_reduce(c, kEstP2P, 1, M));
        TRY(fetch_system(c, sys));
        stats[0] = sys[29];
        stats[1] = sys[28];
        stats[2] = (double)(c->ns_global > 0 ? c->ns_global : c->ns);
    } else {
        HIPCHK(c, hipStreamSynchronize(c->stream));
        collect_events(c);
    }
    return MI_ICP_OK;
}

int mi_icp_get_correspondences(mi_icp_ctx* c, int32_t* pairs, int64_t capacity, int64_t* count,
                               int mem_kind) {
    TRY(check_ctx(c, mem_kind, "get_correspondences"));
    if (!count) return fail(c, MI_ICP_ERR_INVALID, "get_correspondences: count is null");
    *count = 0;
    if (c->n_user_pairs >= 0) {
        *count = c->n_user_pairs;
        if (pairs && capacity >= c->n_user_pairs)
            TRY(from_device(c, (const int32_t*)c->user_pairs.p, pairs, (size_t)c->n_user_pairs * 2, mem_kind));
        HIPCHK(c, hipStreamSynchronize(c->stream));
        return MI_ICP_OK;
    }
    if (!c->nn_valid || c->ns <= 0 || c->nt <= 0) return MI_ICP_OK;
    int32_t* dense;
    TRY(export_dense_idx(c, &dense));
    uint32_t* flags;
    const uint32_t* total;
    int32_t* out;
    TRY(ensure(c, c->flags, (size_t)c->ns, &flags));
    TRY(ensure(c, c->pairs_out, (size_t)c->ns * 2, &out));
    corr_flags<<<blocks_for(c->ns), 256, 0, c->stream>>>(dense, (int)c->ns, flags);
    KCHK(c);
    TRY(scan_into(c, flags, flags, c->ns, &total));
    corr_compact<<<blocks_for(c->ns), 256, 0, c->stream>>>(dense, flags, (int)c->ns, out);
    KCHK(c);
    TRY(read_total(c, total));
    HIPCHK(c, hipStreamSynchronize(c->stream));
    const int64_t m = (int64_t)c->u_host[0];
    *count = m;
    if (pairs && capacity >= m && m > 0) {
        TRY(from_device(c, out, pairs, (size_t)m * 2, mem_kind));
        HIPCHK(c, hipStreamSynchronize(c->stream));
    }
    return MI_ICP_OK;
}

int mi_icp_set_correspondences(mi_icp_ctx* c, const int32_t* pairs, int64_t count, int mem_kind) {
    TRY(check_ctx(c, mem_kind, "set_correspondences"));
    if (count < 0 || (count > 0 && !pairs)) return fail(c, MI_ICP_ERR_INVALID, "set_correspondences: bad arguments");
    int32_t* d;
    TRY(ensure(c, c->user_pairs, (size_t)std::max<int64_t>(count, 1) * 2, &d));
    if (count > 0)
        HIPCHK(c, hipMemcpyAsync(d, pairs, (size_t)count * 2 * sizeof(int32_t),
                                 mem_kind == MI_ICP_DEVICE ? hipMemcpyDeviceToDevice : hipMemcpyHostToDevice,
                                 c->stream));
    HIPCHK(c, hipStreamSynchronize(c->stream));
    c->n_user_pairs = count;
    return MI_ICP_OK;
}

int mi_icp_compute_system(mi_icp_ctx* c, int est, const float* T, double* out32) {
    TRY(check_ctx(c));
    if (!out32) return fail(c, MI_ICP_ERR_INVALID, "compute_system: out is null");
    if (!known_estimator(est))
        return fail(c, MI_ICP_ERR_INVALID, "unknown estimation type %d", est);
    if (!estimator_ready(c, est))
        return fail(c, MI_ICP_ERR_STATE, "estimation type %d needs normals/covariances that were not set", est);
    const Mat4 M = load_T(T);
    TRY(launch_reduce(c, est, 0, M));
    return fetch_system(c, out32);
}

int mi_icp_compute_transformation(mi_icp_ctx* c, int est, const float* T, float det_thresh,
                                  float* update16) {
    TRY(check_ctx(c));
    if (!update16) return fail(c, MI_ICP_ERR_INVALID, "compute_transformation: out is null");
    if (!known_estimator(est))
        return fail(c, MI_ICP_ERR_INVALID, "unknown estimation type %d", est);
    const Mat4 M = load_T(T);
    double sys[kSysSize];
    TRY(launch_reduce(c, est, 0, M));
    TRY(fetch_system(c, sys));
    const Mat4 u = solve_update(c, est, sys, det_thresh);
    std::memcpy(update16, u.data(), sizeof(float) * 16);
    return MI_ICP_OK;
}

int mi_icp_compute_rmse(mi_icp_ctx* c, int est, const float* T, float* rmse) {
    TRY(check_ctx(c));
    if (!rmse) return fail(c, MI_ICP_ERR_INVALID, "compute_rmse: out is null");
    if (!known_estimator(est))
        return fail(c, MI_ICP_ERR_INVALID, "unknown estimation type %d", est);
    *rmse = 0.0f;
    if (!estimator_ready(c, est)) return MI_ICP_OK;
    const Mat4 M = load_T(T);
    double sys[kSysSize];
    TRY(launch_reduce(c, est, 1, M));
    TRY(fetch_system(c, sys));
    if (est == kEstColored) {
        *rmse = (float)sys[27];
    } else if (sys[29] > 0.0) {
        *rmse = std::sqrt((float)sys[27] / (float)sys[29]);
    }
    return MI_ICP_OK;
}

int mi_icp_solve_system(const double* sys32, float det_thresh, float* T16) {
    if (!sys32 || !T16) return MI_ICP_ERR_INVALID;
    Mat4 T;
    const bool ok = host::solve_system(sys32, det_thresh, T);
    std::memcpy(T16, T.data(), sizeof(float) * 16);
    return ok ? 1 : 0;
}

int64_t mi_icp_lzf_decompress(const void* in, int64_t in_len, void* out, int64_t out_capacity) {
    if (!in || !out || in_len < 0 || out_capacity < 0) return 0;
    return (int64_t)lzf::decompress((const uint8_t*)in, (size_t)in_len, (uint8_t*)out, (size_t)out_capacity);
}

int64_t mi_icp_lzf_compress(const void* in, int64_t in_len, void* out, int64_t out_capacity) {
    if (!in || !out || in_len < 0 || out_capacity < 0) return 0;
    return (int64_t)lzf::compress((const uint8_t*)in, (size_t)in_len, (uint8_t*)out, (size_t)out_capacity);
}

int mi_icp_kabsch_from_sums(const double* sys32, int64_t n_model, float* T16) {
    if (!sys32 || !T16 || n_model <= 0) return MI_ICP_ERR_INVALID;
    const Mat4 T = host::kabsch_from_sums(sys32, (long long)n_model);
    std::memcpy(T16, T.data(), sizeof(float) * 16);
    return MI_ICP_OK;
}

void mi_icp_vector6_to_matrix4(const float* x6, float* T16) {
    const Mat4 T = host::vector6_to_matrix4(x6);
    std::memcpy(T16, T.data(), sizeof(float) * 16);
}

int mi_icp_evaluate_registration(mi_icp_ctx* c, float max_distance, const float* T,
                                 mi_icp_result* out) {
    TRY(check_ctx(c));
    if (!out) return fail(c, MI_ICP_ERR_INVALID, "evaluate_registration: out is null");
    const Mat4 M = load_T(T);
    std::memset(out, 0, sizeof(*out));
    std::memcpy(out->transformation, M.data(), sizeof(float) * 16);
    if (max_distance <= 0.0f || (c->ns <= 0 && c->nranks <= 1)) {
        c->nn_valid = false;
        return MI_ICP_OK;
    }
    const Mat4 apply = host::is_identity4(M) ? host::identity4() : M;
    double sys[kSysSize];
    TRY(launch_nn(c, apply, max_distance * max_distance, true));
    TRY(launch_reduce(c, kEstP2P, 1, apply));
    TRY(fetch_system(c, sys));
    stats_from_system(c, sys, &out->fitness, &out->inlier_rmse);
    out->n_correspondences = (int64_t)sys[29];
    out->nn_passes = 1;
    return MI_ICP_OK;
}


static void fill_result(const mi_icp_ctx* c, mi_icp_result* out) {
    const DevLoop& L = *c->loop_host;
    std::memcpy(out->transformation, L.T.data(), sizeof(float) * 16);
    out->fitness = L.fitness;
    out->inlier_rmse = L.rmse;
    out->n_correspondences = (int64_t)L.sys[29];
    out->iterations = L.iterations;
    out->nn_passes = L.passes;
}

static int loop_pull(mi_icp_ctx* c) {
    HIPCHK(c, hipMemcpyAsync(c->loop_host, c->loop_dev.p, sizeof(DevLoop), hipMemcpyDeviceToHost, c->stream));
    HIPCHK(c, hipStreamSynchronize(c->stream));
    if (c->loop_host->error) return comm_failed(c, "the ranks' exchange timed out (mailbox): a peer did not post its sums");
    if (c->iter_fn && c->loop_host->history != 0ull && c->loop_host->iterations > c->iter_reported) {
        const int upto = c->loop_host->iterations;
        const int from = std::max(c->iter_reported, upto - kLoopHistory);
        HIPCHK(c, hipMemcpyAsync(c->hist_host, c->loop_hist.p, sizeof(float) * 2 * kLoopHistory, hipMemcpyDeviceToHost, c->stream));
        HIPCHK(c, hipStreamSynchronize(c->stream));
        c->iter_reported = upto;
        for (int i = from; i < upto; ++i) {
            const float* e = c->hist_host + 2 * (size_t)(i & (kLoopHistory - 1));
            c->iter_fn(c->iter_user, i, e[0], e[1]);
        }
    }
    return MI_ICP_OK;
}

constexpr int64_t kFusedMax = 170000;
constexpr int64_t kFusedMaxP2P = 135000;
static bool fused_iteration_applies(const mi_icp_ctx* c, bool seed) {
    static const bool off = std::getenv("MI_ICP_NO_FUSED_ITERATION") != nullptr;
    const bool pt2pl = c->loop_est == kEstPt2Pl && estimator_ready(c, kEstPt2Pl) && c->t_has_rec && c->trec.p != nullptr;
    const bool p2p = c->loop_est == kEstP2P;
    const int64_t limit = p2p ? kFusedMaxP2P : kFusedMax;
    return !off && seed && c->nn_valid && (pt2pl || p2p) && !c->comm && !c->mail_dev &&
           c->n_user_pairs < 0 && c->ns > 0 && c->ns <= limit && c->nt > 0;
}

static int launch_fused_iteration(mi_icp_ctx* c, DevLoop* d) {
    bool have_halo;
    uint32_t* want;
    TRY(loop_halo(c, &have_halo, &want));
    TRY(drop_expiry(c));
    const PacketGrid g = packet_grid(c->ns, kFusedPackets);
    double *partial, *sys;
    uint32_t* ticket;
    TRY(reduce_buffers(c, std::max<uint32_t>(kReduceBlocks, g.grid), &partial, &sys, &ticket));
    EvTimer t(c, 0, true);
    const auto kernel = (c->loop_est == kEstP2P) ? icp_small_iteration_kernel<kEstP2P> : icp_small_iteration_kernel<kEstPt2Pl>;
    kernel<<<g.grid, kReduceThreads, 0, c->stream>>>(
            (const float*)c->sx.p, (const float*)c->sy.p, (const float*)c->sz.p, (int)c->ns, (const float*)c->nodes.p,
            (const float*)c->tblk.p, (const float*)lreg_of(c), have_halo ? (const float*)c->thalo.p : nullptr, c->leaf_first,
            c->loop_r2, g.npackets, g.nblocks, (int32_t*)c->nn_idx.p, want, (const float*)c->trec.p, d, partial, ticket, sys);
    KCHK(c);
    c->last_search_kind = 1;
    return MI_ICP_OK;
}

static int step_in_reduction(const mi_icp_ctx* c) {
    if (!pt2pl_reduction(c, c->loop_est, 0)) return 0;
    if (mail_on(c)) return 2;
    return (!c->comm && !c->mail_dev) ? 1 : 0;
}

static int loop_enqueue_evaluation(mi_icp_ctx* c, bool seed) {
    DevLoop* d = (DevLoop*)c->loop_dev.p;
    if (seed && c->relocate.armed && c->halo_use && c->nn_valid && c->n_user_pairs < 0 && c->ns > 0 && c->nt > 0) {
        const Xform none = {};
        TRY(launch_locate_by_planes(c, none, d, 1));
    }
    if (fused_iteration_applies(c, seed)) return launch_fused_iteration(c, d);
    const Mat4 I = host::identity4();
    TRY(launch_nn(c, I, c->loop_r2, seed, nullptr, d));
    const int step = step_in_reduction(c);
    TRY(launch_reduce(c, c->loop_est, 0, I, d, step));
    if (step) return MI_ICP_OK;
    const bool mail = mail_on(c);
    if (!mail) TRY(allreduce_system(c));
    loop_step_kernel<<<1, kStepThreads, 0, c->stream>>>(d, (double*)c->sys_dev.p, 0, mail ? mail_args(c) : MailArgs{});
    KCHK(c);
    return MI_ICP_OK;
}

static bool halo_memory_free(const mi_icp_ctx* c) {
    size_t free_b = 0, total_b = 0;
    return hipMemGetInfo(&free_b, &total_b) == hipSuccess && free_b >= (size_t)HaloPolicy::bytes_needed(c->nts);
}

static int loop_run(mi_icp_ctx* c, int budget) {
    ChunkSchedule chunks;
    while (budget > 0) {
        const bool no_halo = !c->links_ready && !c->links_inflight && c->links_allowed && c->nt > 0;
        const bool undecided = no_halo && !c->halo.declined;
        if (c->links_inflight && !c->halo.declined) TRY(ensure_links(c));
        const int n = chunks.plan(budget, HaloPolicy::single_iteration(undecided, c->ns, c->comm != nullptr || c->mail_dev != nullptr));
        const int passes_before = c->loop_host->passes, relocations_before = c->loop_host->relocations;
        c->halo_use = halo_poll(c);
        const bool carried = c->relocate.armed && c->halo_use;
        for (int i = 0; i < n; ++i) TRY(loop_enqueue_evaluation(c, true));
        const bool look = c->halo.wants_look(no_halo);
        if (look) HIPCHK(c, hipMemcpyAsync(c->u_host + 16, c->halo_want.p, kWantSlots * sizeof(uint32_t), hipMemcpyDeviceToHost, c->stream));
        TRY(loop_pull(c));
        const int executed = c->loop_host->passes - passes_before;
        collect_pooled(c, executed);
        c->relocate.after_chunk(carried, c->loop_host->relocations != relocations_before, c->ns);
        budget -= n;
        c->halo.account(executed);
        if (look) {
            uint32_t counted = 0u;
            for (uint32_t k = 0; k < kWantSlots; ++k) counted += c->u_host[16 + k];
            const HaloAction act = c->halo.observe(counted, executed, c->ns, undecided);
            if (act == HaloAction::BuildAndWait || (act == HaloAction::BuildInBackgroundIfMemory && halo_memory_free(c))) {
                ++c->prof[6];
                TRY(start_links_async(c));
            }
        }
        if (c->loop_host->done) break;
        chunks.ran(n);
    }
    return MI_ICP_OK;
}

static int loop_begin(mi_icp_ctx* c, int est, float max_distance, const float* init, float det_thresh,
                      int max_iterations, float rel_fitness, float rel_rmse) {
    if (!known_estimator(est))
        return fail(c, MI_ICP_ERR_INVALID, "unknown estimation type %d", est);
    TRY(comm_usable(c));
    DevLoop& L = *c->loop_host;
    std::memset(&L, 0, sizeof(L));
    L.est = est;
    L.det_thresh = det_thresh;
    L.T = load_T(init);
    L.A = host::is_identity4(L.T) ? host::identity4() : L.T;
    L.X = xform_from(L.A);
    L.max_iterations = max_iterations;
    L.rel_fitness = rel_fitness;
    L.rel_rmse = rel_rmse;
    L.n_source_global = c->ns_global > 0 ? c->ns_global : c->ns;
    L.ready = estimator_ready(c, est) ? 1 : 0;
    L.history = 0ull;
    L.stamps = 0ull;
    L.travel = 0.0;
    L.fuzz = INFINITY;
    TRY(drop_expiry(c));
    const bool can_locate = planes_available(c) && c->ns >= coarse_first_min() && c->src_bounds.p != nullptr && c->nt > 0;
    L.near2_ptr = can_locate ? (uint64_t)(uintptr_t)((const float*)c->nodes.p + kRecordNear2) : 0ull;
    L.src_bounds_ptr = can_locate ? (uint64_t)(uintptr_t)c->src_bounds.p : 0ull;
    c->relocate.on_loop_begin(can_locate);
    if (c->stamps_on) {
        unsigned long long* st;
        TRY(ensure(c, c->stamps, kStampWords, &st));
        unsigned long long init[kStampWords] = {};
        init[0] = init[2] = ~0ull;
        HIPCHK(c, hipMemcpyAsync(st, init, sizeof(init), hipMemcpyHostToDevice, c->stream));
        HIPCHK(c, hipStreamSynchronize(c->stream));
        L.stamps = (uint64_t)(uintptr_t)st;
    }
    c->iter_reported = 0;
    if (c->iter_fn) {
        float* hist;
        TRY(ensure(c, c->loop_hist, (size_t)2 * kLoopHistory, &hist));
        if (!c->hist_host) HIPCHK(c, hipHostMalloc((void**)&c->hist_host, sizeof(float) * 2 * kLoopHistory, hipHostMallocDefault));
        L.history = (uint64_t)(uintptr_t)hist;
    }
    c->loop_active = false;
    c->loop_est = est;
    c->loop_r2 = max_distance * max_distance;
    if (max_distance <= 0.0f || (c->ns <= 0 && c->nranks <= 1)) {
        c->nn_valid = false;
        L.done = 1;
        return MI_ICP_OK;
    }
    DevLoop* d;
    TRY(ensure(c, c->loop_dev, 1, &d));
    HIPCHK(c, hipMemcpyAsync(d, &L, sizeof(DevLoop), hipMemcpyHostToDevice, c->stream));
    c->loop_active = true;
    c->halo.on_loop_begin();
    {
        uint32_t* want;
        TRY(ensure(c, c->halo_want, kWantSlots, &want));
        HIPCHK(c, hipMemsetAsync(want, 0, kWantSlots * sizeof(uint32_t), c->stream));
    }
    c->halo_use = halo_poll(c);
    if (c->halo.sticky && !c->halo_use) {
        if (c->links_inflight) {
            TRY(start_links_async(c));
        } else {
            TRY(ensure_links(c));
            c->halo_use = halo_poll(c);
        }
    }
    const bool resort = c->ns >= 32768 && (max_iterations >= 4 || max_iterations == 0);
    TRY(loop_enqueue_evaluation(c, false));
    if (resort) TRY(resort_source_by_match(c));
    return MI_ICP_OK;
}

int mi_icp_icp_begin(mi_icp_ctx* c, int est, float max_distance, const float* init,
                     float det_thresh, mi_icp_result* out) {
    TRY(check_ctx(c));
    TRY(loop_begin(c, est, max_distance, init, det_thresh, 0, -1.0f, -1.0f));
    if (c->loop_active) {
        TRY(loop_pull(c));
        collect_pooled(c, 1);
    }
    if (out) {
        std::memset(out, 0, sizeof(*out));
        fill_result(c, out);
    }
    return MI_ICP_OK;
}

int mi_icp_icp_iterate(mi_icp_ctx* c, int n_iterations, mi_icp_result* out) {
    TRY(check_ctx(c));
    if (n_iterations < 0) return fail(c, MI_ICP_ERR_INVALID, "icp_iterate: negative count");
    if (c->loop_active && n_iterations > 0) {
        DevLoop* d = (DevLoop*)c->loop_dev.p;
        loop_step_kernel<<<1, kStepThreads, 0, c->stream>>>(d, (double*)c->sys_dev.p, n_iterations, MailArgs{});
        KCHK(c);
        TRY(loop_run(c, n_iterations));
        (void)halo_poll(c);
        release_links_scratch(c);
    }
    if (out) {
        std::memset(out, 0, sizeof(*out));
        fill_result(c, out);
    }
    return MI_ICP_OK;
}

int mi_icp_registration_icp(mi_icp_ctx* c, int est, float max_distance, const float* init,
                            const mi_icp_params* params, mi_icp_result* out) {
    TRY(check_ctx(c));
    if (!out) return fail(c, MI_ICP_ERR_INVALID, "registration_icp: out is null");
    mi_icp_params p = {1e-6f, 1e-6f, 30, 1e-6f};
    if (params) p = *params;
    TRY(loop_begin(c, est, max_distance, init, p.det_thresh, std::max(p.max_iteration, 0),
                   std::max(p.relative_fitness, 0.0f), std::max(p.relative_rmse, 0.0f)));
    if (c->loop_active) {
        TRY(loop_pull(c));
        collect_pooled(c, 1);
        if (!c->loop_host->done) TRY(loop_run(c, std::max(p.max_iteration, 0)));
        (void)halo_poll(c);
        release_links_scratch(c);
    }
    std::memset(out, 0, sizeof(*out));
    fill_result(c, out);
    return MI_ICP_OK;
}

}
```

cupoch_amd/csrc/nn_search.h:

```cpp
#pragma once
#include "device_utils.h"
#include "halo_format.h"
#include "kd_descend.h"
#include "loop.h"
#include "traverse.h"

namespace mi {

constexpr uint32_t kWantSlots = 1024u;
constexpr int kNNThreads = 64;
constexpr int kNNPacketsPerBlock = kNNThreads / 64;

constexpr int kItemQueue = 64 + 8 * 64;

struct PacketShared {
    unsigned long long best[64];
    uint32_t queue[kItemQueue];
};

__device__ __forceinline__ void eval_item(PacketShared& sh, const float* tblk_g, bool have, int ql, uint32_t L,
                                          float ox, float oy, float oz, float r2) {
    if (have) {
        const float4* line = reinterpret_cast<const float4*>(tblk_g + (size_t)L * kLeafFloats);
        const float4 x0 = line[0], x1 = line[1], y0 = line[2], y1 = line[3], z0 = line[4], z1 = line[5];
        const float px[8] = {x0.x, x0.y, x0.z, x0.w, x1.x, x1.y, x1.z, x1.w};
        const float py[8] = {y0.x, y0.y, y0.z, y0.w, y1.x, y1.y, y1.z, y1.w};
        const float pz[8] = {z0.x, z0.y, z0.z, z0.w, z1.x, z1.y, z1.z, z1.w};
        float d[8];
#pragma unroll
        for (int k = 0; k < 8; ++k) {
            const float dx = ox - px[k], dy = oy - py[k], dz = oz - pz[k];
            d[k] = __builtin_fmaf(dz, dz, __builtin_fmaf(dy, dy, dx * dx));
        }
        const float m = fminf(fminf(fminf(d[0], d[1]), fminf(d[2], d[3])), fminf(fminf(d[4], d[5]), fminf(d[6], d[7])));
        if (m < r2) {
            int k = 7;
            k = (d[6] == m) ? 6 : k;
            k = (d[5] == m) ? 5 : k;
            k = (d[4] == m) ? 4 : k;
            k = (d[3] == m) ? 3 : k;
            k = (d[2] == m) ? 2 : k;
            k = (d[1] == m) ? 1 : k;
            k = (d[0] == m) ? 0 : k;
            const unsigned long long cand =
                    ((unsigned long long)__float_as_uint(m) << 32) | (unsigned long long)(L * (uint32_t)kLeaf + (uint32_t)k);
            __hip_atomic_fetch_min(&sh.best[ql], cand, __ATOMIC_RELAXED, __HIP_MEMORY_SCOPE_WORKGROUP);
        }
    }
}

__device__ __forceinline__ void drain_items(PacketShared& sh, const float* tblk_g, uint32_t first, uint32_t count,
                                            float qx, float qy, float qz, float r2) {
    const int lane = lane_id();
    const bool have = (uint32_t)lane < count;
    const uint32_t item = have ? sh.queue[first + (uint32_t)lane] : 0u;
    const int ql = (int)(item >> 26);
    const uint32_t L = item & 0x3ffffffu;
    const float ox = __int_as_float(__builtin_amdgcn_ds_bpermute(ql << 2, __float_as_int(qx)));
    const float oy = __int_as_float(__builtin_amdgcn_ds_bpermute(ql << 2, __float_as_int(qy)));
    const float oz = __int_as_float(__builtin_amdgcn_ds_bpermute(ql << 2, __float_as_int(qz)));
    eval_item(sh, tblk_g, have, ql, L, ox, oy, oz, r2);
}

struct LineMin {
    float m;
    int k;
};
__device__ __forceinline__ LineMin line_min(const float4& x0, const float4& x1, const float4& y0, const float4& y1,
                                            const float4& z0, const float4& z1, float ox, float oy, float oz) {
    const float px[8] = {x0.x, x0.y, x0.z, x0.w, x1.x, x1.y, x1.z, x1.w};
    const float py[8] = {y0.x, y0.y, y0.z, y0.w, y1.x, y1.y, y1.z, y1.w};
    const float pz[8] = {z0.x, z0.y, z0.z, z0.w, z1.x, z1.y, z1.z, z1.w};
    float d[8];
#pragma unroll
    for (int k = 0; k < 8; ++k) {
        const float dx = ox - px[k], dy = oy - py[k], dz = oz - pz[k];
        d[k] = __builtin_fmaf(dz, dz, __builtin_fmaf(dy, dy, dx * dx));
    }
    LineMin r;
    r.m = fminf(fminf(fminf(d[0], d[1]), fminf(d[2], d[3])), fminf(fminf(d[4], d[5]), fminf(d[6], d[7])));
    int k = 7;
    k = (d[6] == r.m) ? 6 : k;
    k = (d[5] == r.m) ? 5 : k;
    k = (d[4] == r.m) ? 4 : k;
    k = (d[3] == r.m) ? 3 : k;
    k = (d[2] == r.m) ? 2 : k;
    k = (d[1] == r.m) ? 1 : k;
    k = (d[0] == r.m) ? 0 : k;
    r.k = k;
    return r;
}

__device__ __forceinline__ void drain_halo(PacketShared& sh, const float* halo_g, uint32_t first, uint32_t count,
                                           uint32_t seed_leaf, float qx, float qy, float qz, float r2) {
    const int lane = lane_id();
    const uint16_t* q16 = reinterpret_cast<const uint16_t*>(sh.queue);
    const bool have = (uint32_t)lane < count;
    const uint32_t item = have ? (uint32_t)q16[first + (uint32_t)lane] : 0u;
    const int ql = (int)(item >> 3);
    const uint32_t f = item & 7u;
    const uint32_t L = (uint32_t)__builtin_amdgcn_ds_bpermute(ql << 2, (int)seed_leaf);
    const float ox = __int_as_float(__builtin_amdgcn_ds_bpermute(ql << 2, __float_as_int(qx)));
    const float oy = __int_as_float(__builtin_amdgcn_ds_bpermute(ql << 2, __float_as_int(qy)));
    const float oz = __int_as_float(__builtin_amdgcn_ds_bpermute(ql << 2, __float_as_int(qz)));
    if (have) {
        const float* lf = halo_g + ((size_t)L * kHaloLines + f) * kHaloLineFloats;
        const float4* line = reinterpret_cast<const float4*>(lf);
        const float4 x0 = line[0], x1 = line[1], y0 = line[2], y1 = line[3], z0 = line[4], z1 = line[5];
        const uint32_t held_bits = (uint32_t)(sh.best[ql] >> 32);
        const LineMin w = line_min(x0, x1, y0, y1, z0, z1, ox, oy, oz);
        if (w.m < r2 && __float_as_uint(w.m) <= held_bits) {
            const uint32_t slot = __float_as_uint(lf[24 + w.k]);
            const unsigned long long cand = ((unsigned long long)__float_as_uint(w.m) << 32) | (unsigned long long)slot;
            __hip_atomic_fetch_min(&sh.best[ql], cand, __ATOMIC_RELAXED, __HIP_MEMORY_SCOPE_WORKGROUP);
        }
    }
}

constexpr float kSkipGrow = 1.0f + 0x1p-19f, kSkipShrink = 1.0f - 0x1p-19f;

template <int CTRL, int ROW_MASK>
__device__ __forceinline__ float dpp_min_hop(float v) {
    return fminf(v, __int_as_float(__builtin_amdgcn_update_dpp(__float_as_int(v), __float_as_int(v), CTRL, ROW_MASK, 0xf, false)));
}
__device__ __forceinline__ float wave_min_last(float v) {
    v = dpp_min_hop<0x111, 0xf>(v);
    v = dpp_min_hop<0x112, 0xf>(v);
    v = dpp_min_hop<0x114, 0xf>(v);
    v = dpp_min_hop<0x118, 0xf>(v);
    v = dpp_min_hop<0x142, 0xa>(v);
    v = dpp_min_hop<0x143, 0xc>(v);
    return v;
}

__device__ __forceinline__ float second_smallest8(const float* d) {
    const float l0 = fminf(d[0], d[1]), l1 = fminf(d[2], d[3]), l2 = fminf(d[4], d[5]), l3 = fminf(d[6], d[7]);
    const float h0 = fmaxf(d[0], d[1]), h1 = fmaxf(d[2], d[3]), h2 = fmaxf(d[4], d[5]), h3 = fmaxf(d[6], d[7]);
    const float s01 = fminf(fmaxf(l0, l1), fminf(h0, h1)), s23 = fminf(fmaxf(l2, l3), fminf(h2, h3));
    return fminf(fmaxf(fminf(l0, l1), fminf(l2, l3)), fminf(s01, s23));
}

struct PacketResult {
    bool valid;
    int i;
    int32_t bidx;
    float best;
    float qx, qy, qz;
};

template <bool SEED, bool STATS>
__device__ __forceinline__ bool nn_packet_body(
        PacketShared& sh, uint32_t packet,
        const float* __restrict__ sx, const float* __restrict__ sy, const float* __restrict__ sz,
        int ns, const float* __restrict__ records_g, const float* __restrict__ tblk_g,
        const float* __restrict__ lreg_g, const float* __restrict__ halo_g, uint32_t leaf_first, Xform Tv, const DevLoop* __restrict__ loop, float r2, int32_t* __restrict__ nn_idx,
        float* __restrict__ nn_d2, unsigned long long* __restrict__ stats, uint32_t* __restrict__ want, PacketResult& out,
        double* __restrict__ expiry = nullptr, uint8_t* __restrict__ live = nullptr, uint32_t live_shift = 0u) {
    const int lane = lane_id();
    const bool limits = SEED && !STATS && loop != nullptr && expiry != nullptr && nn_d2 == nullptr;
    const int i = (int)(packet * 64u) + lane;
    const bool valid = i < ns;
    const int ic = valid ? i : 0;
    int32_t seed_j = -1;
    if (SEED) seed_j = nn_idx[ic];
    const float rx = sx[ic], ry = sy[ic], rz = sz[ic];
    const float cap2 = ((cfloat_p)(uintptr_t)records_g)[kRecordCap2];
    Xform T = Tv;
    if (loop) {
        if (loop->done) return false;
        T = loop->X;
    }
    if (!valid) seed_j = -1;
    float qx = 0.0f, qy = 0.0f, qz = 0.0f;
    if (valid) xform_point(T, rx, ry, rz, qx, qy, qz);
    float best = valid ? r2 : -1.0f;
    int32_t bidx = -1;

    bool retired = !valid;
    bool linked = false;
    uint32_t nlines = 0u;
    uint32_t why = 0u;
    float margin = valid ? -1.0f : INFINITY, margin2 = INFINITY;
    if (SEED) {
        const int32_t j = seed_j;
        const uint32_t Lc = (j >= 0) ? ((uint32_t)j >> 3) : 0u;
        const float4* line = reinterpret_cast<const float4*>(tblk_g + (size_t)Lc * kLeafFloats);
        const float4* rg = reinterpret_cast<const float4*>(lreg_g + (size_t)Lc * kLeafRegStride);
        const float4 x0 = line[0], x1 = line[1], y0 = line[2], y1 = line[3], z0 = line[4], z1 = line[5];
        const float4 g0 = rg[0], g1 = rg[1];
        if (j >= 0) {
            const uint32_t L = Lc;
            const float px[8] = {x0.x, x0.y, x0.z, x0.w, x1.x, x1.y, x1.z, x1.w};
            const float py[8] = {y0.x, y0.y, y0.z, y0.w, y1.x, y1.y, y1.z, y1.w};
            const float pz[8] = {z0.x, z0.y, z0.z, z0.w, z1.x, z1.y, z1.z, z1.w};
            float d[8];
#pragma unroll
            for (int k = 0; k < 8; ++k) d[k] = sq3(qx - px[k], qy - py[k], qz - pz[k]);
            const float m = fminf(fminf(fminf(d[0], d[1]), fminf(d[2], d[3])), fminf(fminf(d[4], d[5]), fminf(d[6], d[7])));
            if (m < best) {
                int k = 7;
                k = (d[6] == m) ? 6 : k;
                k = (d[5] == m) ? 5 : k;
                k = (d[4] == m) ? 4 : k;
                k = (d[3] == m) ? 3 : k;
                k = (d[2] == m) ? 2 : k;
                k = (d[1] == m) ? 1 : k;
                k = (d[0] == m) ? 0 : k;
                best = m;
                bidx = (int32_t)(L * (uint32_t)kLeaf + (uint32_t)k);
            }
            const float rb = __builtin_amdgcn_sqrtf(best) * 1.0000005f;
            const float inside = fminf(fminf(fminf(qx - g0.x, qy - g0.y), fminf(qz - g0.z, g1.x - qx)),
                                       fminf(g1.y - qy, g1.z - qz));
            if (inside >= rb) {
                retired = true;
                if (limits && bidx >= 0) {
                    margin2 = second_smallest8(d);
                    margin = inside * kSkipShrink - rb * kSkipGrow;
                }
            } else {
                Cube cube;
                set_cube(cube, qx, qy, qz, best);
                const float ux = cube.hix - g1.x, uy = cube.hiy - g1.y, uz = cube.hiz - g1.z;
                const float lx = g0.x - cube.lox, ly = g0.y - cube.loy, lz = g0.z - cube.loz;
                const float over = fmaxf(fmaxf(fmaxf(ux, lx), fmaxf(uy, ly)), fmaxf(uz, lz)) * 1.000001f;
                nlines = halo_lines_needed(g0.w, g1.w, over);
                linked = halo_g != nullptr && nlines <= (uint32_t)kHaloLines;
                if (STATS) why = !(g0.x <= g1.x) ? 1u : (__float_as_uint(g1.w) == 0u ? 2u : (!linked ? 3u : 0u));
            }
        }
    }
    if (SEED && __builtin_expect(want != nullptr, 0)) {
        const uint64_t m = __ballot(valid && !retired && seed_j >= 0);
        if (m != 0ull && lane == 0) atomicAdd(want + (packet & (kWantSlots - 1u)), (uint32_t)__popcll(m));
    }
    if (limits) {
        bool has = false;
        if (__ballot(margin < 0.0f) == 0ull) {
            if (valid) {
                const float a1 = __builtin_amdgcn_sqrtf(best) * kSkipGrow;
                const float m = fminf(fminf(0.5f * (__builtin_amdgcn_sqrtf(margin2) * kSkipShrink - a1), 0.5f * margin),
                                      __builtin_amdgcn_sqrtf(r2) * kSkipShrink - a1);
                margin = (m > 0.0f) ? m : 0.0f;
            }
            const float pm = wave_min_last(margin);
            const double room = (double)pm - loop->fuzz;
            has = room > 0.0;
            if (lane == 63) expiry[packet] = has ? loop->travel + room : -(double)INFINITY;
        } else if (lane == 63) {
            expiry[packet] = -(double)INFINITY;
        }
        if (lane == 63 && (packet & ((1u << live_shift) - 1u)) == 0u && (packet >> live_shift) < 64u)
            live[packet >> live_shift] = has ? 1 : 0;
    }
    sh.best[lane] = ((unsigned long long)__float_as_uint(fmaxf(best, 0.0f)) << 32) | (unsigned long long)(uint32_t)bidx;
    __builtin_amdgcn_wave_barrier();

    uint32_t queued = 0u, batches = 0u, halo_items = 0u;
    if (SEED && __builtin_expect(__ballot(linked) != 0ull, 0)) {
        const uint32_t seed_leaf = linked ? ((uint32_t)seed_j >> 3) : 0u;
        const uint32_t nn = linked ? nlines : 0u;
        if (__ballot(nn > 1u) == 0ull) {
            if (STATS) ++batches, halo_items += (uint32_t)__popcll(__ballot(linked));
            const float* lf = halo_g + (size_t)seed_leaf * (kHaloLines * kHaloLineFloats);
            const float4* line = reinterpret_cast<const float4*>(lf);
            const float4 x0 = line[0], x1 = line[1], y0 = line[2], y1 = line[3], z0 = line[4], z1 = line[5];
            if (linked) {
                const LineMin w = line_min(x0, x1, y0, y1, z0, z1, qx, qy, qz);
                if (w.m < r2 && w.m <= best) {
                    const int32_t slot = __float_as_int(lf[24 + w.k]);
                    if (w.m < best || slot < bidx || bidx < 0) {
                        best = w.m;
                        bidx = slot;
                    }
                }
                retired = true;
            }
            if (__ballot(!retired) != 0ull)
                sh.best[lane] = ((unsigned long long)__float_as_uint(fmaxf(best, 0.0f)) << 32) | (unsigned long long)(uint32_t)bidx;
        } else {
            uint16_t* q16 = reinterpret_cast<uint16_t*>(sh.queue);
#pragma unroll
            for (int k = 0; k < kHaloLines; ++k) {
                const bool mine = nn > (uint32_t)k;
                const uint64_t m = __ballot(mine);
                if (m == 0ull) break;
                if (mine) {
                    const uint32_t pos = queued + __builtin_amdgcn_mbcnt_hi((uint32_t)(m >> 32),
                                                                            __builtin_amdgcn_mbcnt_lo((uint32_t)m, 0u));
                    q16[pos] = (uint16_t)(((uint32_t)lane << 3) | (uint32_t)k);
                }
                queued += (uint32_t)__popcll(m);
            }
            __builtin_amdgcn_wave_barrier();
            if (STATS) halo_items += queued;
            for (uint32_t first = 0u; first < queued; first += 64u) {
                if (STATS) ++batches;
                drain_halo(sh, halo_g, first, min(64u, queued - first), seed_leaf, qx, qy, qz, r2);
            }
            queued = 0u;
            __builtin_amdgcn_wave_barrier();
            if (linked) retired = true;
            {
                const unsigned long long bb = sh.best[lane];
                if (valid && (int32_t)(uint32_t)bb != bidx) {
                    best = __uint_as_float((uint32_t)(bb >> 32));
                    bidx = (int32_t)(uint32_t)bb;
                }
            }
        }
    }
    const bool any_walk = SEED ? (__ballot(!retired) != 0ull) : true;
    const uint64_t done_before = __ballot(retired);
    float wcap2 = cap2;
    if (!SEED) wcap2 = fminf(cap2, ((cfloat_p)(uintptr_t)records_g)[kRecordNear2]);
    Cube cube;
    if (retired) {
        cube.lox = cube.loy = cube.loz = INFINITY;
        cube.hix = cube.hiy = cube.hiz = -INFINITY;
    } else {
        set_cube(cube, qx, qy, qz, fminf(best, wcap2));
    }
    constexpr uint32_t kNoItem = 0xffffffffu;
    uint32_t held = kNoItem;
    bool spilled = false;
    auto take_results = [&]() {
        __builtin_amdgcn_wave_barrier();
        const unsigned long long b = sh.best[lane];
        const float nb = __uint_as_float((uint32_t)(b >> 32));
        if (valid && (int32_t)(uint32_t)b != bidx) {
            best = nb;
            bidx = (int32_t)(uint32_t)b;
            if (!retired) set_cube(cube, qx, qy, qz, fminf(best, wcap2));
        }
    };
    auto drain = [&](uint32_t first, uint32_t count) {
        if (STATS) ++batches;
        drain_items(sh, tblk_g, first, count, qx, qy, qz, r2);
        take_results();
    };
    auto on_leaf_record = [&](uint32_t lbase, uint32_t vm, uint32_t hit) {
        if (SEED) {
            const uint32_t seed_leaf = (uint32_t)seed_j >> 3;
            if ((seed_leaf & ~7u) == lbase) vm &= ~(1u << (seed_leaf & 7u));
        }
        if (!spilled) {
            const bool more = (vm & (vm - 1u)) != 0u || (vm != 0u && held != kNoItem);
            if (__ballot(more) == 0ull) {
                if (vm != 0u) held = lbase + (uint32_t)__builtin_ctz(vm);
                return;
            }
            spilled = true;
            const bool h = held != kNoItem;
            const uint64_t m = __ballot(h);
            if (h) {
                const uint32_t pos = queued + __builtin_amdgcn_mbcnt_hi((uint32_t)(m >> 32),
                                                                        __builtin_amdgcn_mbcnt_lo((uint32_t)m, 0u));
                sh.queue[pos] = ((uint32_t)lane << 26) | held;
            }
            queued += (uint32_t)__popcll(m);
            held = kNoItem;
        }
        while (hit) {
            const uint32_t c = (uint32_t)__builtin_ctz(hit);
            hit &= hit - 1u;
            const bool mine = (vm >> c) & 1u;
            const uint64_t m = __ballot(mine);
            if (mine) {
                const uint32_t pos = queued + __builtin_amdgcn_mbcnt_hi((uint32_t)(m >> 32),
                                                                        __builtin_amdgcn_mbcnt_lo((uint32_t)m, 0u));
                sh.queue[pos] = ((uint32_t)lane << 26) | (lbase + c);
            }
            queued += (uint32_t)__popcll(m);
        }
        __builtin_amdgcn_wave_barrier();
        while (queued >= 64u) {
            queued -= 64u;
            drain(queued, 64u);
        }
    };
    uint32_t steps = 0u;
    const uint32_t walkers = STATS ? (uint32_t)__popcll(__ballot(!retired)) : 0u;
    if (STATS && SEED) {
        for (uint32_t w = 0u; w < 5u; ++w) {
            const uint32_t nw = (uint32_t)__popcll(__ballot(!retired && (seed_j < 0 ? 0u : why) == w && (w != 0u || seed_j < 0)));
            if (lane == 0 && nw) atomicAdd(stats + 8 + w, (unsigned long long)nw);
        }
    }
    for (;;) {
        if (!SEED) steps += traverse_from(records_g, leaf_first, 1u, cube, on_leaf_record);
        else if (__builtin_expect(__ballot(!retired) != 0ull, 0)) {
            const uint32_t my_node = (seed_j >= 0) ? leaf_first + ((uint32_t)seed_j >> 6) : 0u;
            steps = traverse_seeded(records_g, leaf_first, my_node, cube, retired, on_leaf_record);
        }
        if (!spilled) {
            if (__ballot(held != kNoItem) != 0ull) {
                if (STATS) ++batches;
                eval_item(sh, tblk_g, held != kNoItem, lane, held, qx, qy, qz, r2);
                take_results();
            }
        } else if (queued) {
            drain(0u, queued);
        }
        if (SEED || !(wcap2 < cap2) || !(r2 > wcap2)) break;
        const bool again = valid && !(best < wcap2);
        if (__ballot(again) == 0ull) break;
        wcap2 = cap2;
        retired = !again;
        if (retired) {
            cube.lox = cube.loy = cube.loz = INFINITY;
            cube.hix = cube.hiy = cube.hiz = -INFINITY;
        } else {
            set_cube(cube, qx, qy, qz, fminf(best, wcap2));
        }
        held = kNoItem;
        spilled = false;
        queued = 0u;
    }
    if (any_walk && r2 > cap2) {
        const bool alone = valid && ((done_before >> lane) & 1ull) == 0ull && !(best < cap2);
        if (__ballot(alone) != 0ull) {
            solo_walk(records_g, leaf_first, alone, qx, qy, qz, [&]() { return best; }, [&](uint32_t L) {
                const float4* line = reinterpret_cast<const float4*>(tblk_g + (size_t)L * kLeafFloats);
                const LineMin w = line_min(line[0], line[1], line[2], line[3], line[4], line[5], qx, qy, qz);
                const int32_t j = (int32_t)(L * (uint32_t)kLeaf + (uint32_t)w.k);
                if (w.m < best || (w.m == best && bidx >= 0 && j < bidx)) {
                    best = w.m;
                    bidx = j;
                }
            });
        }
    }

    if (valid) {
        if (!SEED || bidx != seed_j) nn_idx[i] = bidx;
        if (nn_d2) nn_d2[i] = (bidx >= 0) ? best : INFINITY;
    }
    if (STATS && lane == 0) {
        atomicAdd(stats + 0, (unsigned long long)steps);
        atomicAdd(stats + 1, (unsigned long long)batches);
        atomicAdd(stats + 2, 1ull);
        atomicMax(stats + 3, (unsigned long long)steps + (unsigned long long)batches);
        atomicAdd(stats + 4, (unsigned long long)halo_items);
        atomicAdd(stats + 5, halo_items ? 1ull : 0ull);
        atomicAdd(stats + 6, steps ? 1ull : 0ull);
        atomicAdd(stats + 7, (unsigned long long)walkers);
    }
    out.valid = valid;
    out.i = i;
    out.bidx = bidx;
    out.best = best;
    out.qx = qx;
    out.qy = qy;
    out.qz = qz;
    return true;
}

constexpr uint32_t kSkipRun = 8;
template <bool SEED, bool STATS, bool STAMP = false, bool GATE = false>
__global__ __launch_bounds__(kNNThreads) __attribute__((amdgpu_waves_per_eu(GATE ? 6 : (SEED ? 8 : 7), 8))) void nn_packet_kernel(
        const float* __restrict__ sx, const float* __restrict__ sy, const float* __restrict__ sz,
        int ns, const float* __restrict__ records_g, const float* __restrict__ tblk_g,
        const float* __restrict__ lreg_g, const float* __restrict__ halo_g, uint32_t leaf_first, Xform Tv, const DevLoop* __restrict__ loop, float r2, uint32_t nblocks, int32_t* __restrict__ nn_idx,
        float* __restrict__ nn_d2, unsigned long long* __restrict__ stats, uint32_t* __restrict__ want,
        double* __restrict__ expiry, uint8_t* __restrict__ live, uint32_t live_shift, uint32_t run) {
    __shared__ PacketShared s_pk[kNNPacketsPerBlock];
    uint32_t logical;
    if (!xcd_remap(nblocks, logical)) return;
    PacketResult unused;
    unsigned long long* stamps = (STAMP && loop) ? reinterpret_cast<unsigned long long*>(loop->stamps) : nullptr;
    if (STAMP && stamps && threadIdx.x == 0 && blockIdx.x < 64u) atomicMin(stamps + 0, stamp_now());
    if (!GATE) {
        (void)nn_packet_body<SEED, STATS>(s_pk[0], logical, sx, sy, sz, ns, records_g, tblk_g, lreg_g, halo_g, leaf_first, Tv, loop,
                                          r2, nn_idx, nn_d2, stats, want, unused, expiry, live, live_shift);
    } else {
        const uint32_t npackets = ((uint32_t)ns + 63u) >> 6, lane = (uint32_t)lane_id();
        const uint32_t first = logical * run;
        const bool mine = lane < run && first + lane < npackets;
        const double limit = expiry[mine ? first + lane : first];
        const double reach = loop->travel + loop->fuzz;
        uint32_t need = (loop->done != 0) ? 0u : (uint32_t)__ballot(mine && !(reach < limit));
        while (need != 0u) {
            const uint32_t k = (uint32_t)__builtin_ctz(need);
            need &= need - 1u;
            (void)nn_packet_body<true, false>(s_pk[0], first + k, sx, sy, sz, ns, records_g, tblk_g, lreg_g, halo_g, leaf_first, Xform{},
                                              loop, r2, nn_idx, nullptr, nullptr, want, unused, expiry, live, live_shift);
            __builtin_amdgcn_wave_barrier();
        }
    }
    if (STAMP && stamps && threadIdx.x == 0 && blockIdx.x + 256u >= gridDim.x) atomicMax(stamps + 1, stamp_now());
}

static __global__ __launch_bounds__(256) void locate_by_planes(
        const float* __restrict__ sx, const float* __restrict__ sy, const float* __restrict__ sz, int ns,
        const float2* __restrict__ cell_planes, int cell_levels, const uint32_t* __restrict__ gstart,
        const float2* __restrict__ gplanes, uint32_t nleaf, Xform Tv, const DevLoop* __restrict__ loop, int gated,
        int32_t* __restrict__ nn_idx, double* __restrict__ expiry) {
    Xform T = Tv;
    if (loop) {
        if (loop->done) return;
        if (gated && loop->relocate == 0) return;
        T = loop->X;
    }
    for (int64_t i = (int64_t)blockIdx.x * 256 + threadIdx.x; i < ns; i += (int64_t)gridDim.x * 256) {
        float qx, qy, qz;
        xform_point(T, sx[i], sy[i], sz[i], qx, qy, qz);
        const uint32_t cell = descend_cell(cell_planes, cell_levels, qx, qy, qz);
        const uint32_t g = gstart[cell];
        const uint32_t leaf = min(g * 512u + descend_group(gplanes + (size_t)g * 512u, qx, qy, qz), nleaf - 1u);
        nn_idx[i] = (int32_t)(leaf * (uint32_t)kLeaf);
        if (expiry != nullptr && (i & 63) == 0) expiry[i >> 6] = -(double)INFINITY;
    }
}


static __global__ __launch_bounds__(256) void export_dense(const int32_t* __restrict__ nn_idx,
                                                    const float* __restrict__ nn_d2,
                                                    const int32_t* __restrict__ sperm,
                                                    const int32_t* __restrict__ tidx, int ns,
                                                    int32_t* __restrict__ idx_out,
                                                    float* __restrict__ d2_out) {
    const int64_t i = (int64_t)blockIdx.x * 256 + threadIdx.x;
    if (i >= ns) return;
    const int32_t j = nn_idx[i];
    const int32_t o = sperm[i];
    int32_t tj = -1;
    if (j >= 0) tj = tidx[j];
    if (idx_out) idx_out[o] = tj;
    if (d2_out) d2_out[o] = nn_d2[i];
}

static __global__ __launch_bounds__(256) void corr_flags(const int32_t* __restrict__ dense_idx, int ns,
                                                  uint32_t* __restrict__ flags) {
    const int64_t o = (int64_t)blockIdx.x * 256 + threadIdx.x;
    if (o >= ns) return;
    flags[o] = dense_idx[o] >= 0 ? 1u : 0u;
}

static __global__ __launch_bounds__(256) void corr_compact(const int32_t* __restrict__ dense_idx,
                                                    const uint32_t* __restrict__ pos, int ns,
                                                    int32_t* __restrict__ pairs) {
    const int64_t o = (int64_t)blockIdx.x * 256 + threadIdx.x;
    if (o >= ns) return;
    const int32_t tj = dense_idx[o];
    if (tj >= 0) {
        const int64_t p = pos[o];
        pairs[2 * p] = (int32_t)o;
        pairs[2 * p + 1] = tj;
    }
}

static __global__ __launch_bounds__(256) void fill_i32(int32_t* __restrict__ a, int64_t n, int32_t v) {
    const int64_t i = (int64_t)blockIdx.x * 256 + threadIdx.x;
    if (i < n) a[i] = v;
}

static __global__ __launch_bounds__(256) void invert_perm_source(const int32_t* __restrict__ sperm, int ns,
                                                          int32_t* __restrict__ inv) {
    const int64_t s = (int64_t)blockIdx.x * 256 + threadIdx.x;
    if (s < ns) inv[sperm[s]] = (int32_t)s;
}

static __global__ __launch_bounds__(256) void invert_perm_target(const int32_t* __restrict__ tidx, int nt,
                                                          int32_t* __restrict__ inv) {
    const int64_t s = (int64_t)blockIdx.x * 256 + threadIdx.x;
    if (s < nt) {
        const int32_t o = tidx[s];
        if (o >= 0) inv[o] = (int32_t)s;
    }
}

}
```

cupoch_amd/csrc/reduce.h:

```cpp
#pragma once
#include "device_utils.h"
#include "eigen3.h"
#include "loop.h"

namespace mi {

constexpr int kReduceThreads = 256;
constexpr int kReduceBlocks = 1024;

__device__ __forceinline__ void rotate_cov(const Xform& T, const float* C, M3& out) {
    const float R[3][3] = {{T.r00, T.r01, T.r02}, {T.r10, T.r11, T.r12}, {T.r20, T.r21, T.r22}};
    float RC[3][3];
#pragma unroll
    for (int c = 0; c < 3; ++c)
#pragma unroll
        for (int r = 0; r < 3; ++r)
            RC[r][c] = __builtin_fmaf(R[r][2], C[c * 3 + 2],
                                      __builtin_fmaf(R[r][1], C[c * 3 + 1], R[r][0] * C[c * 3 + 0]));
#pragma unroll
    for (int c = 0; c < 3; ++c)
#pragma unroll
        for (int r = 0; r < 3; ++r)
            out.m[r][c] = __builtin_fmaf(RC[r][2], R[c][2],
                                         __builtin_fmaf(RC[r][1], R[c][1], RC[r][0] * R[c][0]));
// ... 80 lines not shown
#pragma unroll
            for (int u = 0; u < kU; ++u) {
                const int bb = b + u * kParts;
                const double v = pk[(int64_t)(bb < nb ? bb : 0) * kSysSize];
                acc16[u] += (bb < nb) ? v : 0.0;
            }
        }
#pragma unroll
        for (int w = kU / 2; w > 0; w >>= 1)
#pragma unroll
            for (int u = 0; u < w; ++u) acc16[u] += acc16[u + w];
        red[part][k] = acc16[0];
        __syncthreads();
        if (threadIdx.x < kSysSize) {
            double t = 0.0;
#pragma unroll
            for (int p = 0; p < kParts; ++p) t += red[p][k];
            out32[k] = t;
            if (pre) pre->sum = t;
        }
        if (threadIdx.x == 0) __hip_atomic_store(ticket, 0u, __ATOMIC_RELAXED, __HIP_MEMORY_SCOPE_AGENT);
    }
    return true;
}

__device__ __forceinline__ bool block_finish(const double* acc, double* __restrict__ partial,
                                             uint32_t* __restrict__ ticket, double* __restrict__ out32,
                                             StepPre* pre = nullptr, const DevLoop* pre_state = nullptr,
                                             const uint32_t* pre_mail_seq = nullptr, unsigned long long* stamps = nullptr) {
    __shared__ ReduceRows red;
    const int lane = lane_id(), wid = (int)(threadIdx.x >> 6);
#pragma unroll
    for (int k = 0; k < 30; ++k) {
        const double v = wave_sum(acc[k]);
        if (lane == kWaveSumLane) red[wid][k] = v;
    }
    if (lane == kWaveSumLane) {
        red[wid][30] = 0.0;
        red[wid][31] = 0.0;
    }
    return block_finish_rows(red, partial, ticket, out32, pre, pre_state, pre_mail_seq, stamps);
}


__device__ __forceinline__ void leaf_point(const float* tblk, int32_t j, float* vt) {
    const float* line = tblk + (int64_t)(j >> 3) * kLeafFloats + (j & 7);
    vt[0] = line[0];
    vt[1] = line[8];
    vt[2] = line[16];
}

__device__ __forceinline__ void trec_gather(const float* trec, int32_t j, float* vt, float* nt) {
    const F3* r = reinterpret_cast<const F3*>(trec + (int64_t)j * 6);
    const F3 p = r[0], n = r[1];
    vt[0] = p.x;
    vt[1] = p.y;
    vt[2] = p.z;
    nt[0] = n.x;
    nt[1] = n.y;
    nt[2] = n.z;
}

__device__ __forceinline__ void pt2pl_row(const float* vs, const float* vt, const float* nt, float* J, float& r, float& d2) {
    const float d[3] = {vs[0] - vt[0], vs[1] - vt[1], vs[2] - vt[2]};
    d2 = sq3(d[0], d[1], d[2]);
    r = dot3(d, nt);
    cross3(vs, nt, J);
    J[3] = nt[0];
    J[4] = nt[1];
    J[5] = nt[2];
}

template <int MODE>
__device__ __forceinline__ void pt2pl_rows(double* acc, const float* vs, const float* vt, const float* nt) {
    float J[6], r, d2;
    pt2pl_row(vs, vt, nt, J, r, d2);
    acc[28] += (double)d2;
    acc[29] += 1.0;
    if (MODE == 0) accum_row(acc, J, r);
    else acc[27] += (double)(r * r);
}

template <int MODE>
__device__ __forceinline__ void sym_rows(double* acc, const Xform& T, const ReduceArgs& a, int64_t i, int32_t j,
                                         const float* vs, const float* vt, const float* d) {
    const float4 t4 = a.tnrm[j];
    const float4 s4 = a.snrm[i];
    float ns[3];
    rotate(T, s4.x, s4.y, s4.z, ns[0], ns[1], ns[2]);
    const float n[3] = {ns[0] + t4.x, ns[1] + t4.y, ns[2] + t4.z};
    const float r = dot3(d, n);
    if (MODE == 0) {
        const float s[3] = {vs[0] + vt[0], vs[1] + vt[1], vs[2] + vt[2]};
        float J[6];
        cross3(s, n, J);
        J[3] = n[0];
        J[4] = n[1];
        J[5] = n[2];
        accum_row(acc, J, r);
    } else {
        const float e2 = r * r;
        acc[27] += (double)(e2 * e2);
    }
}

template <int MODE>
__device__ __forceinline__ void colored_rows(double* acc, const ReduceArgs& a, int64_t i, int32_t j, const float* vs,
                                             const float* vt, const float* d) {
    const float4 n4 = a.tnrm[j];
    const float4 g4 = a.tgrad[j];
    const float nt[3] = {n4.x, n4.y, n4.z};
    const float dit[3] = {g4.x, g4.y, g4.z};
    const float it = n4.w, is = a.sint[i];
    const float slg = a.sqrt_lambda_geometric, slp = a.sqrt_lambda_photometric;
    const float dn = dot3(d, nt);
    const float r0 = slg * dn;
    const float e[3] = {(vs[0] - dn * nt[0]) - vt[0], (vs[1] - dn * nt[1]) - vt[1], (vs[2] - dn * nt[2]) - vt[2]};
    const float r1 = slp * (is - (dot3(dit, e) + it));
    if (MODE == 0) {
        float J[6], cr[3];
        cross3(vs, nt, cr);
#pragma unroll
        for (int p = 0; p < 3; ++p) {
            J[p] = slg * cr[p];
            J[3 + p] = slg * nt[p];
        }
        accum_row(acc, J, r0);
        float ditM[3];
#pragma unroll
        for (int col = 0; col < 3; ++col) {
            float s = 0.0f;
#pragma unroll
            for (int row = 0; row < 3; ++row) {
                const float m = (row == col) ? (1.0f - nt[row] * nt[col]) : (-(nt[row] * nt[col]));
                s += dit[row] * m;
            }
            ditM[col] = -s;
        }
        cross3(vs, ditM, cr);
#pragma unroll
        for (int p = 0; p < 3; ++p) {
            J[p] = slp * cr[p];
            J[3 + p] = slp * ditM[p];
        }
        accum_row(acc, J, r1);
    } else {
        acc[27] += (double)(r0 * r0 + r1 * r1);
    }
}

template <int MODE>
__device__ __forceinline__ void gicp_rows(double* acc, const Xform& T, const ReduceArgs& a, int64_t i, int32_t j,
                                          const float* vs, const float* d) {
    M3 Cs, M, Mi;
    rotate_cov(T, a.scov + i * 9, Cs);
    const float* Ct = a.tcov + (int64_t)j * 9;
#pragma unroll
    for (int r = 0; r < 3; ++r)
#pragma unroll
        for (int c = 0; c < 3; ++c) M.m[r][c] = Ct[c * 3 + r] + Cs.m[r][c];
    inverse3(M, Mi);
    if (MODE == 0) {
        float S[3][3];
        gicp_weight(Mi, S);
        const float x = vs[0], y = vs[1], z = vs[2];
        const float Sd[3] = {S[0][0] * d[0] + S[0][1] * d[1] + S[0][2] * d[2],
                             S[1][0] * d[0] + S[1][1] * d[1] + S[1][2] * d[2],
                             S[2][0] * d[0] + S[2][1] * d[1] + S[2][2] * d[2]};
        float P[3][3], Q[3][3];
#pragma unroll
        for (int r = 0; r < 3; ++r) {
            P[r][0] = S[r][2] * y - S[r][1] * z;
            P[r][1] = S[r][0] * z - S[r][2] * x;
            P[r][2] = S[r][1] * x - S[r][0] * y;
        }
#pragma unroll
        for (int c = 0; c < 3; ++c) {
            Q[0][c] = y * P[2][c] - z * P[1][c];
            Q[1][c] = z * P[0][c] - x * P[2][c];
            Q[2][c] = x * P[1][c] - y * P[0][c];
        }
        const float g[3] = {y * Sd[2] - z * Sd[1], z * Sd[0] - x * Sd[2], x * Sd[1] - y * Sd[0]};
        int k = 0;
#pragma unroll
        for (int p = 0; p < 6; ++p)
#pragma unroll
            for (int q = p; q < 6; ++q, ++k) {
                const float v = (q < 3) ? Q[p][q] : ((p < 3) ? P[q - 3][p] : S[p - 3][q - 3]);
                acc[k] += (double)v;
            }
#pragma unroll
        for (int p = 0; p < 3; ++p) {
            acc[21 + p] += (double)g[p];
            acc[24 + p] += (double)Sd[p];
        }
        acc[27] += (double)dot3(d, Sd);
    } else {
        M3 W;
        sqrt_matrix3x3(Mi, W);
        float Wd[3];
#pragma unroll
        for (int r = 0; r < 3; ++r) Wd[r] = W.m[r][0] * d[0] + W.m[r][1] * d[1] + W.m[r][2] * d[2];
        acc[27] += (double)dot3(d, Wd);
    }
}

template <int MODE>
__device__ __forceinline__ void p2p_rows(double* acc, const float* vs, const float* vt, const float* d) {
    if (MODE == 0) {
#pragma unroll
        for (int p = 0; p < 3; ++p) {
            acc[p] += (double)vs[p];
            acc[3 + p] += (double)vt[p];
#pragma unroll
            for (int q = 0; q < 3; ++q) acc[6 + p * 3 + q] = __builtin_fma((double)vs[p], (double)vt[q], acc[6 + p * 3 + q]);
        }
        acc[27] += (double)sq3(d[0], d[1], d[2]);
    } else {
        acc[27] += (double)dot3(d, d);
    }
}

template <int EST, int MODE>
__global__ __launch_bounds__(kReduceThreads) void reduce_kernel(ReduceArgs a, Xform Tv,
                                                                const DevLoop* __restrict__ loop,
                                                                double* __restrict__ partial,
                                                                uint32_t* __restrict__ ticket,
                                                                double* __restrict__ out32) {
    Xform T = Tv;
    if (loop) {
        if (loop->done) return;
        T = loop->X;
    }
    double acc[30];
#pragma unroll
    for (int k = 0; k < 30; ++k) acc[k] = 0.0;

    const int64_t stride = (int64_t)gridDim.x * kReduceThreads;
    const int64_t k0 = (int64_t)blockIdx.x * kReduceThreads + threadIdx.x;
    int32_t nj = -1;
    float npx = 0.0f, npy = 0.0f, npz = 0.0f;
    if (!a.pairs && a.count > 0) {
        const int64_t kc = (k0 < a.count) ? k0 : 0;
        nj = a.nn_idx[kc];
        npx = a.sx[kc];
        npy = a.sy[kc];
        npz = a.sz[kc];
    }
    for (int64_t k = k0; k < a.count; k += stride) {
        int64_t i;
        int32_t j;
        float spx, spy, spz;
        if (a.pairs) {
            const int32_t pi = a.pairs[2 * k], pj = a.pairs[2 * k + 1];
            if ((uint32_t)pi >= (uint32_t)a.ns || (uint32_t)pj >= (uint32_t)a.nt) continue;
            i = a.inv_s[pi];
            j = a.inv_t[pj];
            if (j < 0) continue;
            spx = a.sx[i];
            spy = a.sy[i];
            spz = a.sz[i];
        } else {
            i = k;
            j = nj;
            spx = npx;
            spy = npy;
            spz = npz;
            const int64_t kc = (k + stride < a.count) ? k + stride : 0;
            nj = a.nn_idx[kc];
            npx = a.sx[kc];
            npy = a.sy[kc];
            npz = a.sz[kc];
        }
        if (j < 0) continue;
        float vs[3], vt[3];
        xform_point(T, spx, spy, spz, vs[0], vs[1], vs[2]);
        if (EST == kEstPt2Pl) {
            float nt[3];
            if (a.trec) {
                trec_gather(a.trec, j, vt, nt);
            } else {
                leaf_point(a.tblk, j, vt);
                const float4 n4 = a.tnrm[j];
                nt[0] = n4.x;
                nt[1] = n4.y;
                nt[2] = n4.z;
            }
            pt2pl_rows<MODE>(acc, vs, vt, nt);
        } else {
            leaf_point(a.tblk, j, vt);
            const float d[3] = {vs[0] - vt[0], vs[1] - vt[1], vs[2] - vt[2]};
            acc[28] += (double)sq3(d[0], d[1], d[2]);
            acc[29] += 1.0;
            if (EST == kEstSym) sym_rows<MODE>(acc, T, a, i, j, vs, vt, d);
            else if (EST == kEstColored) colored_rows<MODE>(acc, a, i, j, vs, vt, d);
            else if (EST == kEstGICP) gicp_rows<MODE>(acc, T, a, i, j, vs, d);
            else p2p_rows<MODE>(acc, vs, vt, d);
        }
    }

    block_finish(acc, partial, ticket, out32);
}

template <int kU, int STEP, bool STAMP = false>
__global__ __launch_bounds__(kReduceThreads) void reduce_pt2pl_kernel(ReduceArgs a, Xform Tv,
                                                                      DevLoop* __restrict__ loop,
                                                                      double* __restrict__ partial,
                                                                      uint32_t* __restrict__ ticket,
                                                                      double* __restrict__ out32, MailArgs mail) {
    const int64_t stride = (int64_t)gridDim.x * kReduceThreads;
    const int64_t k0 = (int64_t)blockIdx.x * kReduceThreads + threadIdx.x;
    int32_t j[kU];
    float px[kU], py[kU], pz[kU];
    auto fetch = [&](int64_t kb) {
#pragma unroll
        for (int u = 0; u < kU; ++u) {
            const int64_t k = kb + (int64_t)u * stride;
            const int64_t kc = (k < a.count) ? k : 0;
            j[u] = a.nn_idx[kc];
            px[u] = a.sx[kc];
            py[u] = a.sy[kc];
            pz[u] = a.sz[kc];
        }
    };
    fetch(k0);
    Xform T = Tv;
    unsigned long long* stamps = nullptr;
    if (loop) {
        if (loop->done) return;
        T = loop->X;
        if (STAMP) stamps = reinterpret_cast<unsigned long long*>(loop->stamps);
    }
    if (STAMP && stamps && threadIdx.x == 0) atomicMin(stamps + 2, stamp_now());
    double acc[30];
#pragma unroll
    for (int k = 0; k < 30; ++k) acc[k] = 0.0;
    for (int64_t kb = k0; kb < a.count; kb += stride * kU) {
        float vt[kU][3], nt[kU][3];
        bool have[kU];
#pragma unroll
        for (int u = 0; u < kU; ++u) {
            have[u] = (kb + (int64_t)u * stride) < a.count && j[u] >= 0;
            trec_gather(a.trec, have[u] ? j[u] : 0, vt[u], nt[u]);
        }
        float vs[kU][3];
#pragma unroll
        for (int u = 0; u < kU; ++u) xform_point(T, px[u], py[u], pz[u], vs[u][0], vs[u][1], vs[u][2]);
        fetch(kb + stride * kU);
#pragma unroll
        for (int u = 0; u < kU; ++u)
            if (have[u]) pt2pl_rows<0>(acc, vs[u], vt[u], nt[u]);
    }
    StepPre pre{STEP != 0, 0u, 0.0, 0u};
    const bool last = block_finish(acc, partial, ticket, out32, &pre, STEP ? loop : nullptr,
                                   (STEP == 2) ? mail.seq_dev : nullptr, STAMP ? stamps : nullptr);
    if (STEP && last) {
        __shared__ DevLoop st_s;
        if (STAMP && stamps && threadIdx.x == 0) stamps[4] = stamp_now();
        loop_step_block(loop, out32, 0, st_s, pre, (STEP == 2) ? mail : MailArgs{}, STAMP ? stamps : nullptr);
    }
}

}
```

cupoch_amd/engine.py:

```python
import ctypes as C

import numpy as np

from . import _lib
from ._lib import MI_ICP_DEVICE, MI_ICP_HOST, MiIcpError, Params, Result

try:
    import torch
except Exception:
    torch = None


def _is_tensor(a):
    return torch is not None and isinstance(a, torch.Tensor)


class _Buf:

    def __init__(self, a, dtype, cols, device_index, copy=False):
        self.keep = None
        self.ptr = None
        self.kind = MI_ICP_HOST
        self.device = None
        self.n = 0
        if a is None:
            return
        if _is_tensor(a):
            tdt = {np.float32: torch.float32, np.int32: torch.int32}[dtype]
            t = a
            if t.dtype != tdt:
                t = t.to(tdt)
            t = t.reshape(-1, cols).contiguous()
            if t.is_cuda:
                if t.device.index != device_index:
                    raise MiIcpError("tensor on cuda:%s passed to an engine on cuda:%s"
                                     % (t.device.index, device_index))
                self.kind = MI_ICP_DEVICE
                self.device = t.device
                self.ptr = C.c_void_p(t.data_ptr())
            else:
                t = t.numpy()
                self.ptr = t.ctypes.data_as(C.c_void_p)
            self.keep = t
            self.n = int(t.shape[0])
        else:
            arr = np.ascontiguousarray(np.asarray(a, dtype=dtype).reshape(-1, cols))
            if copy and np.shares_memory(arr, a):
                arr = arr.copy()
            self.keep = arr
            self.ptr = arr.ctypes.data_as(C.c_void_p)
            self.n = int(arr.shape[0])


def _T_in(T):
    if T is None:
        return None, None
    if _is_tensor(T):
        T = T.detach().cpu().numpy()
    a = np.ascontiguousarray(np.asarray(T, dtype=np.float32).reshape(4, 4).T)
    return a, a.ctypes.data_as(C.c_void_p)


def _T_out(buf16):
    return np.array(buf16, dtype=np.float32).reshape(4, 4).T.copy()


class Engine:

    def __init__(self, device=0, use_torch_stream=True):
        self._L = _lib.load()
        self._ctx = C.c_void_p()
        rc = self._L.mi_icp_create(int(device), C.byref(self._ctx))
        if rc != 0:
            self._ctx = None
            raise MiIcpError("mi_icp_create(device=%d) failed with status %d "
                             "(no MI355X visible?)" % (device, rc))
        self.device = int(device)
        self.n_source = 0
        self.n_target = 0
        if use_torch_stream and torch is not None and torch.cuda.is_available():
            with torch.cuda.device(self.device):
                self.set_stream(torch.cuda.current_stream().cuda_stream)

    def _chk(self, rc):
        if rc < 0:
            msg = self._L.mi_icp_last_error(self._ctx)
            raise MiIcpError("mi_icp error %d: %s" % (rc, (msg or b"").decode()))
        return rc

    def close(self):
        if getattr(self, "_ctx", None):
            self._L.mi_icp_destroy(self._ctx)
            self._ctx = None

    def __del__(self):
        try:
            self.close()
        except Exception:
            pass

    def set_stream(self, hip_stream):
        self._chk(self._L.mi_icp_set_stream(self._ctx, C.c_void_p(int(hip_stream))))

    def synchronize(self):
        self._chk(self._L.mi_icp_synchronize(self._ctx))

    def _same_kind(self, *bufs):
        kinds = {b.kind for b in bufs if b.ptr is not None}
        if len(kinds) > 1:
            raise MiIcpError("all arrays of one call must live on the same side (host or device)")
        return kinds.pop() if kinds else MI_ICP_HOST

    @staticmethod
    def _out(kind, device, shape, dtype=np.float32):
        if kind == MI_ICP_DEVICE:
            tdt = {np.float32: torch.float32, np.int32: torch.int32, np.int64: torch.int64, np.uint8: torch.uint8}[dtype]
            t = torch.empty(shape, dtype=tdt, device=device)
            return t, C.c_void_p(t.data_ptr())
        a = np.empty(shape, dtype)
        return a, a.ctypes.data_as(C.c_void_p)

    @staticmethod
    def _trim(t, k):
        return None if t is None else t[:k]

    def _set_cloud(self, fn, points, normals, covariances):
        self.generation = getattr(self, "generation", 0) + 1
        p = _Buf(points, np.float32, 3, self.device)
        n = _Buf(normals, np.float32, 3, self.device)
        c = _Buf(_cov_in(covariances), np.float32, 9, self.device)
        kind = self._same_kind(p, n, c)
        self._chk(fn(self._ctx, p.ptr, n.ptr, c.ptr, p.n, kind))
        self.synchronize()
        return p.n

    def set_target(self, points, normals=None, covariances=None):
        self.n_target = self._set_cloud(self._L.mi_icp_set_target, points, normals, covariances)

    def set_source(self, points, normals=None, covariances=None):
        self.n_source = self._set_cloud(self._L.mi_icp_set_source, points, normals, covariances)

    def search_knn(self, queries, knn, radius=0.0):
        q = _Buf(queries, np.float32, 3, self.device)
        knn = int(knn)
        idx, ip = self._out(q.kind, q.device, (q.n, knn), np.int32)
        d2, dp = self._out(q.kind, q.device, (q.n, knn))
        found = C.c_int64(0)
        self._chk(self._L.mi_icp_search_knn(self._ctx, q.ptr, q.n, knn, float(radius), ip, dp,
                                            C.byref(found), q.kind))
        self.n_source = q.n
        self.generation = getattr(self, "generation", 0) + 1
        return int(found.value), idx, d2

    def set_target_colors(self, colors):
        b = _Buf(colors, np.float32, 3, self.device)
        if b.n and b.n != self.n_target:
            raise MiIcpError("set_target_colors: %d colours for %d target points" % (b.n, self.n_target))
        self._chk(self._L.mi_icp_set_target_colors(self._ctx, b.ptr, b.kind))
        self.synchronize()

    def set_source_colors(self, colors):
        b = _Buf(colors, np.float32, 3, self.device)
        if b.n and b.n != self.n_source:
            raise MiIcpError("set_source_colors: %d colours for %d source points" % (b.n, self.n_source))
        self._chk(self._L.mi_icp_set_source_colors(self._ctx, b.ptr, b.kind))
        self.synchronize()

    def set_lambda_geometric(self, lambda_geometric):
        self._chk(self._L.mi_icp_set_lambda_geometric(self._ctx, float(lambda_geometric)))

    def compute_color_gradients(self, radius, max_nn=30, want_output=True):
        out, optr = self._out(MI_ICP_HOST, None, (self.n_target, 3)) if want_output else (None, None)
        self._chk(self._L.mi_icp_compute_color_gradients(self._ctx, float(radius), int(max_nn), optr,
                                                         MI_ICP_HOST))
        return out

    def registration_colored_icp(self, max_distance, init=None, relative_fitness=1e-6,
                                 relative_rmse=1e-6, max_iteration=30, lambda_geometric=0.968,
                                 det_thresh=1e-6):
        res = Result()
        prm = Params(float(relative_fitness), float(relative_rmse), int(max_iteration),
                     float(det_thresh))
        _, tp = _T_in(init)
        self._chk(self._L.mi_icp_registration_colored_icp(self._ctx, float(max_distance), tp,
                                                          C.byref(prm), float(lambda_geometric),
                                                          C.byref(res)))
        return res

    def morton_order(self, points):
        p = _Buf(points, np.float32, 3, self.device)
        if p.n == 0:
            return np.zeros(0, np.int64)
        out, optr = self._out(p.kind, p.device, (p.n,), np.int32)
        self._chk(self._L.mi_icp_spatial_order(self._ctx, p.ptr, p.n, optr, p.kind))
        if p.kind == MI_ICP_DEVICE:
            out = out.cpu().numpy()
        return out.view(np.uint32).astype(np.int64)

    def set_global_source_count(self, n_total):
        self._chk(self._L.mi_icp_set_global_source_count(self._ctx, int(n_total)))

    def search_radius_1nn(self, radius, T=None, want_d2=True):
        idx, ip = self._out(MI_ICP_HOST, None, (self.n_source,), np.int32)
        d2, dp = self._out(MI_ICP_HOST, None, (self.n_source,)) if want_d2 else (None, None)
        stats = np.zeros(3, np.float64)
        _, tp = _T_in(T)
        self._chk(self._L.mi_icp_search_radius_1nn(self._ctx, tp, float(radius), ip, dp, MI_ICP_HOST,
                                                   stats.ctypes.data_as(C.c_void_p)))
        return idx, d2, stats

    def drop_seeds(self):
        self._chk(self._L.mi_icp_debug_drop_seeds(self._ctx))

    def loop_counters(self):
        out = np.zeros(4, np.int32)
        self._chk(self._L.mi_icp_debug_loop_counters(self._ctx, out.ctypes.data_as(C.c_void_p)))
        return out

    def search_skip_state(self):
        n, armed = C.c_int64(0), C.c_int(0)
        st = np.zeros(2, np.float64)
        self._chk(self._L.mi_icp_debug_search_skip(self._ctx, st.ctypes.data_as(C.c_void_p), None, 0, C.byref(n), C.byref(armed)))
        lim = np.zeros(n.value, np.float64)
        self._chk(self._L.mi_icp_debug_search_skip(self._ctx, st.ctypes.data_as(C.c_void_p), lim.ctypes.data_as(C.c_void_p),
                                                   n.value, C.byref(n), C.byref(armed)))
        with np.errstate(invalid="ignore"):
            will = (st[0] + st[1] < lim) if armed.value else np.zeros(n.value, bool)
        return {"travel": float(st[0]), "fuzz": float(st[1]), "limits": lim, "armed": bool(armed.value), "will_skip": will}

    def last_search_kind(self):
        return int(self._L.mi_icp_debug_last_search_kind(self._ctx))

    def get_correspondences(self):
        cnt = C.c_int64(0)
        self._chk(self._L.mi_icp_get_correspondences(self._ctx, None, 0, C.byref(cnt), MI_ICP_HOST))
        out, optr = self._out(MI_ICP_HOST, None, (max(cnt.value, 0), 2), np.int32)
        if cnt.value > 0:
            self._chk(self._L.mi_icp_get_correspondences(self._ctx, optr, cnt.value, C.byref(cnt), MI_ICP_HOST))
        return out

    def set_correspondences(self, pairs):
        b = _Buf(pairs, np.int32, 2, self.device)
        self._chk(self._L.mi_icp_set_correspondences(self._ctx, b.ptr, b.n, b.kind))

    def compute_system(self, est, T=None):
        out = np.zeros(32, np.float64)
        _, tp = _T_in(T)
        self._chk(self._L.mi_icp_compute_system(self._ctx, int(est), tp,
                                                out.ctypes.data_as(C.c_void_p)))
        return out

    def compute_transformation(self, est, T=None, det_thresh=1e-6):
        out = (C.c_float * 16)()
        _, tp = _T_in(T)
        self._chk(self._L.mi_icp_compute_transformation(self._ctx, int(est), tp,
                                                        float(det_thresh), out))
        return _T_out(out)

    def compute_rmse(self, est, T=None):
        out = C.c_float(0)
        _, tp = _T_in(T)
        self._chk(self._L.mi_icp_compute_rmse(self._ctx, int(est), tp, C.byref(out)))
        return float(out.value)

    def evaluate_registration(self, max_distance, T=None):
        res = Result()
        _, tp = _T_in(T)
        self._chk(self._L.mi_icp_evaluate_registration(self._ctx, float(max_distance), tp,
                                                       C.byref(res)))
        return res

    def registration_icp(self, est, max_distance, init=None, relative_fitness=1e-6,
                         relative_rmse=1e-6, max_iteration=30, det_thresh=1e-6):
        res = Result()
        prm = Params(float(relative_fitness), float(relative_rmse), int(max_iteration),
                     float(det_thresh))
        _, tp = _T_in(init)
        self._chk(self._L.mi_icp_registration_icp(self._ctx, int(est), float(max_distance), tp,
                                                  C.byref(prm), C.byref(res)))
        return res

    def icp_begin(self, est, max_distance, init=None, det_thresh=1e-6):
        res = Result()
        _, tp = _T_in(init)
        self._chk(self._L.mi_icp_icp_begin(self._ctx, int(est), float(max_distance), tp,
                                           float(det_thresh), C.byref(res)))
        return res

    def icp_iterate(self, n_iterations=1):
        res = Result()
        self._chk(self._L.mi_icp_icp_iterate(self._ctx, int(n_iterations), C.byref(res)))
        return res

    def transform(self, T, points=None, normals=None, covariances=None):
        p = _Buf(points, np.float32, 3, self.device, copy=True)
        n = _Buf(normals, np.float32, 3, self.device, copy=True)
        c = _Buf(_cov_in(covariances), np.float32, 9, self.device, copy=True)
        kind = self._same_kind(p, n, c)
        cnt = max(p.n, n.n, c.n)
        _, tp = _T_in(T)
        self._chk(self._L.mi_icp_transform(self._ctx, tp, p.ptr, n.ptr, c.ptr, cnt, kind))
        return p.keep, n.keep, _cov_out(c.keep)

    def compute_bounds(self, points):
        p = _Buf(points, np.float32, 3, self.device)
        out = np.zeros((3, 3), np.float32)
        ptr = lambda r: out[r].ctypes.data_as(C.c_void_p)
        self._chk(self._L.mi_icp_compute_bounds(self._ctx, p.ptr, p.n, p.kind, ptr(0), ptr(1), ptr(2)))
        return out[0].copy(), out[1].copy(), out[2].copy()

    def affine(self, points=None, normals=None, covariances=None, R=None, scale=None, center=None, translate=None):
        p = _Buf(points, np.float32, 3, self.device, copy=True)
        n = _Buf(normals, np.float32, 3, self.device, copy=True)
        c = _Buf(_cov_in(covariances), np.float32, 9, self.device, copy=True)
        kind = self._same_kind(p, n, c)
        cnt = max(p.n, n.n, c.n)
        vec = lambda v: None if v is None else np.ascontiguousarray(np.asarray(v, np.float32).reshape(3))
        Rc = None if R is None else np.ascontiguousarray(np.asarray(R, np.float32).reshape(3, 3).T)
        cv, tv = vec(center), vec(translate)
        ptr = lambda a: None if a is None else a.ctypes.data_as(C.c_void_p)
        self._chk(self._L.mi_icp_affine(self._ctx, ptr(Rc), float(scale if scale is not None else 1.0),
                                        0 if scale is None else 1, ptr(cv), ptr(tv), p.ptr, n.ptr, c.ptr, cnt, kind))
        self.synchronize()
        return p.keep, n.keep, _cov_out(c.keep)

    def _cloud_args(self, points, normals, colors):
        p = _Buf(points, np.float32, 3, self.device)
        n = _Buf(normals, np.float32, 3, self.device)
        c = _Buf(colors, np.float32, 3, self.device)
        return p, n, c, self._same_kind(p, n, c)

    def _cloud_outputs(self, kind, p, n, c, rows):
        op = self._out(kind, p.device, (rows, 3))
        on = self._out(kind, p.device, (rows, 3)) if n.ptr is not None else (None, None)
        oc = self._out(kind, p.device, (rows, 3)) if c.ptr is not None else (None, None)
        return op, on, oc

    def voxel_downsample(self, points, voxel_size, normals=None, colors=None):
        p, n, c, kind = self._cloud_args(points, normals, colors)
        (op, pp), (on, pn), (oc, pc) = self._cloud_outputs(kind, p, n, c, p.n)
        m = C.c_int64(0)
        self._chk(self._L.mi_icp_voxel_downsample(self._ctx, p.ptr, n.ptr, c.ptr, p.n, float(voxel_size), pp, pn, pc,
                                                  C.byref(m), kind))
        k = int(m.value)
        return (self._trim(op, k) if p.ptr is not None else np.empty((0, 3), np.float32)), self._trim(on, k), \
            self._trim(oc, k)

    def _outlier_filter(self, fn, points, k, param, normals, colors, stat_dtype):
        p, n, c, kind = self._cloud_args(points, normals, colors)
        (op, pp), (on, pn), (oc, pc) = self._cloud_outputs(kind, p, n, c, p.n)
        idx, pidx = self._out(kind, p.device, (p.n,), np.int64)
        stat, pstat = self._out(kind, p.device, (p.n,), stat_dtype)
        m = C.c_int64(0)
        self._chk(fn(self._ctx, p.ptr, n.ptr, c.ptr, p.n, int(k), float(param), pp, pn, pc, pidx, pstat, C.byref(m), kind))
        k = int(m.value)
        return self._trim(op, k), self._trim(on, k), self._trim(oc, k), idx[:k], stat

    def remove_statistical_outliers(self, points, nb_neighbors, std_ratio, normals=None, colors=None):
        return self._outlier_filter(self._L.mi_icp_remove_statistical_outliers, points, nb_neighbors, std_ratio,
                                    normals, colors, np.float32)

    def remove_radius_outliers(self, points, nb_points, radius, normals=None, colors=None):
        return self._outlier_filter(self._L.mi_icp_remove_radius_outliers, points, nb_points, radius,
                                    normals, colors, np.int32)

    def cluster_dbscan(self, points, eps, min_points, max_edges=100):
        p = _Buf(points, np.float32, 3, self.device)
        kind = self._same_kind(p)
        labels, plab = self._out(kind, p.device, (p.n,), np.int32)
        degrees, pdeg = self._out(kind, p.device, (p.n,), np.int32)
        nc = C.c_int64(0)
        self._chk(self._L.mi_icp_cluster_dbscan(self._ctx, p.ptr, p.n, float(eps), int(min_points), int(max_edges),
                                                plab, pdeg, C.byref(nc), kind))
        return labels, degrees, int(nc.value)

    def segment_plane(self, points, distance_threshold, ransac_n=3, num_iterations=100, seed=0):
        p = _Buf(points, np.float32, 3, self.device)
        kind = self._same_kind(p)
        idx, pidx = self._out(kind, p.device, (p.n,), np.int64)
        plane, ransac = np.zeros(4, np.float32), np.zeros(4, np.float32)
        m, best, count = C.c_int64(0), C.c_int64(-1), C.c_int64(0)
        self._chk(self._L.mi_icp_segment_plane(self._ctx, p.ptr, p.n, float(distance_threshold), int(ransac_n),
                                               int(num_iterations), C.c_uint64(int(seed) & (2 ** 64 - 1)),
                                               plane.ctypes.data_as(C.c_void_p), ransac.ctypes.data_as(C.c_void_p), pidx,
                                               C.byref(m), C.byref(best), C.byref(count), kind))
        return plane, idx[:int(m.value)], ransac, int(best.value), int(count.value)

    def select_by_index(self, points, indices, invert=False, normals=None, colors=None):
        p, n, c, kind = self._cloud_args(points, normals, colors)
        if kind == MI_ICP_DEVICE:
            ix = torch.as_tensor(indices).to(device=p.device, dtype=torch.int64).reshape(-1).contiguous() \
                if _is_tensor(indices) else torch.from_numpy(np.ascontiguousarray(np.asarray(indices, np.int64).reshape(-1))).to(p.device)
            pix, nix = C.c_void_p(ix.data_ptr()), int(ix.shape[0])
        else:
            ix = indices.detach().cpu().numpy() if _is_tensor(indices) else indices
            ix = np.ascontiguousarray(np.asarray(ix, np.int64).reshape(-1))
            pix, nix = ix.ctypes.data_as(C.c_void_p), int(ix.shape[0])
        rows = p.n if invert else nix
        (op, pp), (on, pn), (oc, pc) = self._cloud_outputs(kind, p, n, c, rows)
        m = C.c_int64(0)
        self._chk(self._L.mi_icp_select_by_index(self._ctx, p.ptr, n.ptr, c.ptr, p.n, pix, nix, int(bool(invert)),
                                                 pp, pn, pc, C.byref(m), kind))
        k = int(m.value)
        return self._trim(op, k), self._trim(on, k), self._trim(oc, k)

    def iss_keypoints(self, points, salient_radius=0.0, non_max_radius=0.0, gamma_21=0.975, gamma_32=0.975,
                      min_neighbors=5, max_neighbors=100, want_response=False):
        p = _Buf(points, np.float32, 3, self.device)
        kind = self._same_kind(p)
        mask, pmask = self._out(kind, p.device, (p.n,), np.uint8)
        sal = eig = cnt = psal = peig = pcnt = None
        if want_response:
            sal, psal = self._out(kind, p.device, (p.n,), np.float32)
            eig, peig = self._out(kind, p.device, (p.n, 3), np.float32)
            cnt, pcnt = self._out(kind, p.device, (p.n,), np.int32)
        radii = np.zeros(2, np.float32)
        m = C.c_int64(0)
        self._chk(self._L.mi_icp_iss_keypoints(self._ctx, p.ptr, p.n, float(salient_radius), float(non_max_radius),
                                               float(gamma_21), float(gamma_32), int(min_neighbors), int(max_neighbors),
                                               pmask, psal, peig, pcnt, radii.ctypes.data_as(C.c_void_p), C.byref(m), kind))
        out = (mask, int(m.value), (float(radii[0]), float(radii[1])))
        return out + (sal, eig, cnt) if want_response else out

    def select_by_mask(self, points, mask, invert=False, normals=None, colors=None):
        p, n, c, kind = self._cloud_args(points, normals, colors)
        if kind == MI_ICP_DEVICE:
            mk = mask if _is_tensor(mask) else torch.from_numpy(np.ascontiguousarray(np.asarray(mask).reshape(-1) != 0))
            mk = (mk.reshape(-1) != 0).to(device=p.device, dtype=torch.uint8).contiguous()
            pmk, nmk = C.c_void_p(mk.data_ptr()), int(mk.shape[0])
        else:
            mk = mask.detach().cpu().numpy() if _is_tensor(mask) else mask
            mk = np.ascontiguousarray((np.asarray(mk).reshape(-1) != 0).astype(np.uint8))
            pmk, nmk = mk.ctypes.data_as(C.c_void_p), int(mk.shape[0])
        (op, pp), (on, pn), (oc, pc) = self._cloud_outputs(kind, p, n, c, p.n)
        m = C.c_int64(0)
        self._chk(self._L.mi_icp_select_by_mask(self._ctx, p.ptr, n.ptr, c.ptr, p.n, pmk, nmk, int(bool(invert)),
                                                pp, pn, pc, C.byref(m), kind))
        k = int(m.value)
        return self._trim(op, k), self._trim(on, k), self._trim(oc, k)

    def farthest_point_downsample(self, points, num_samples, normals=None, colors=None):
        p, n, c, kind = self._cloud_args(points, normals, colors)
        rows = max(0, min(int(num_samples), p.n))
        (op, pp), (on, pn), (oc, pc) = self._cloud_outputs(kind, p, n, c, rows)
        idx, pidx = self._out(kind, p.device, (rows,), np.int64)
        m = C.c_int64(0)
        self._chk(self._L.mi_icp_farthest_point_downsample(self._ctx, p.ptr, n.ptr, c.ptr, p.n, int(num_samples),
                                                           pp, pn, pc, pidx, C.byref(m), kind))
        k = int(m.value)
        return self._trim(op, k), self._trim(on, k), self._trim(oc, k), idx[:k]

    def gaussian_filter(self, points, search_radius, sigma2, num_max_search_points=50, normals=None, colors=None):
        p, n, c, kind = self._cloud_args(points, normals, colors)
        (op, pp), (on, pn), (oc, pc) = self._cloud_outputs(kind, p, n, c, p.n)
        self._chk(self._L.mi_icp_gaussian_filter(self._ctx, p.ptr, n.ptr, c.ptr, p.n, float(search_radius), float(sigma2),
                                                 int(num_max_search_points), pp, pn, pc, kind))
        return op, on, oc

    def _predicate_filter(self, points, normals, colors, call):
        p, n, c, kind = self._cloud_args(points, normals, colors)
        (op, pp), (on, pn), (oc, pc) = self._cloud_outputs(kind, p, n, c, p.n)
        idx, pidx = self._out(kind, p.device, (p.n,), np.int64)
        m = C.c_int64(0)
        self._chk(call(p, n, c, pp, pn, pc, pidx, C.byref(m), kind))
        k = int(m.value)
        return self._trim(op, k), self._trim(on, k), self._trim(oc, k), idx[:k]

    def pass_through_filter(self, points, axis_no, min_bound, max_bound, normals=None, colors=None):
        return self._predicate_filter(points, normals, colors, lambda p, n, c, *out: self._L.mi_icp_pass_through_filter(
            self._ctx, p.ptr, n.ptr, c.ptr, p.n, int(axis_no), float(min_bound), float(max_bound), *out))

    def crop_aabb(self, points, min_bound, max_bound, normals=None, colors=None):
        lo = np.ascontiguousarray(np.asarray(min_bound, np.float32).reshape(3))
        hi = np.ascontiguousarray(np.asarray(max_bound, np.float32).reshape(3))
        return self._predicate_filter(points, normals, colors, lambda p, n, c, *out: self._L.mi_icp_crop_aabb(
            self._ctx, p.ptr, n.ptr, c.ptr, p.n, lo.ctypes.data_as(C.c_void_p), hi.ctypes.data_as(C.c_void_p), *out))

    def remove_none_finite(self, points, remove_nan=True, remove_infinite=True, normals=None, colors=None):
        return self._predicate_filter(points, normals, colors, lambda p, n, c, *out: self._L.mi_icp_remove_none_finite(
            self._ctx, p.ptr, n.ptr, c.ptr, p.n, int(bool(remove_nan)), int(bool(remove_infinite)), *out))

    def uniform_downsample(self, points, every_k_points, normals=None, colors=None):
        p, n, c, kind = self._cloud_args(points, normals, colors)
        k = int(every_k_points)
        rows = p.n // k if k > 0 else 0
        (op, pp), (on, pn), (oc, pc) = self._cloud_outputs(kind, p, n, c, rows)
        m = C.c_int64(0)
        self._chk(self._L.mi_icp_uniform_downsample(self._ctx, p.ptr, n.ptr, c.ptr, p.n, k, pp, pn, pc,
                                                    C.byref(m), kind))
        return op[:int(m.value)], on, oc

    def create_from_depth(self, depth, intrinsic4, extrinsic=None, color=None, depth_scale=1000.0,
                          depth_trunc=1000.0, depth_cutoff=-1.0, stride=1, rgbd=False,
                          compute_normals=False, valid_only=True):
        on_dev = _is_tensor(depth) and depth.is_cuda
        def prep(x, kinds):
            if x is None:
                return None, None
            if _is_tensor(x):
                if x.dtype not in kinds:
                    raise TypeError("unsupported image dtype %s" % x.dtype)
                if x.is_cuda != on_dev:
                    raise ValueError("depth and color must live on the same side")
                x = x.contiguous() if on_dev else np.ascontiguousarray(x.numpy())
            else:
                if on_dev:
                    raise ValueError("depth and color must live on the same side")
                x = np.ascontiguousarray(x)
            return x, (C.c_void_p(x.data_ptr()) if on_dev else x.ctypes.data_as(C.c_void_p))
        if _is_tensor(depth):
            dkinds, ckinds = (torch.float32, torch.uint16), (torch.uint8, torch.float32)
        else:
            dkinds = ckinds = None
        d, dptr = prep(depth, dkinds)
        col, cptr = prep(color, ckinds)
        if d.ndim != 2:
            raise ValueError("depth must be [H, W]")
        dname = str(d.dtype).replace("torch.", "")
        if dname not in ("float32", "uint16"):
            raise TypeError("depth must be float32 or uint16")
        h, w = int(d.shape[0]), int(d.shape[1])
        ctype = 0
        if col is not None:
            cname = str(col.dtype).replace("torch.", "")
            if cname == "uint8" and tuple(col.shape) == (h, w, 3):
                ctype = 1
            elif cname == "float32" and tuple(col.shape)[:2] == (h, w) and \
                    (col.numel() if on_dev else col.size) == h * w:
                ctype = 2
            else:
                raise TypeError("[PointCloud::CreateFromRGBDImage] Unsupported image format.")
# ... 286 lines not shown
```

include/mi_icp_debug.h:

```cpp
#ifndef MI_ICP_DEBUG_H_
#define MI_ICP_DEBUG_H_
#include "mi_icp.h"
#ifdef __cplusplus
extern "C" {
#endif
MI_ICP_API int mi_icp_debug_sort_pairs(mi_icp_ctx* ctx, uint64_t* keys, uint32_t* vals,
                                       int64_t n, int key_bits);
MI_ICP_API int mi_icp_debug_exclusive_scan(mi_icp_ctx* ctx, const uint32_t* in, uint32_t* out,
                                           int64_t n, uint64_t* total);
MI_ICP_API int mi_icp_debug_morton_order(mi_icp_ctx* ctx, const float* xyz, int64_t n,
                                         uint32_t* order);
MI_ICP_API int mi_icp_debug_nn_stats(mi_icp_ctx* ctx, const float* T, float radius, int use_seed,
                                     uint64_t* out4);
MI_ICP_API int mi_icp_debug_nn_stats8(mi_icp_ctx* ctx, const float* T, float radius, int use_seed,
                                      uint64_t* out8);
MI_ICP_API int mi_icp_debug_drop_seeds(mi_icp_ctx* ctx);
MI_ICP_API int mi_icp_debug_last_search_kind(const mi_icp_ctx* ctx);
MI_ICP_API int mi_icp_debug_last_voxel_path(const mi_icp_ctx* ctx);
MI_ICP_API int mi_icp_debug_occupancy(int which);
MI_ICP_API int mi_icp_debug_loop_counters(mi_icp_ctx* ctx, int32_t* out4);
MI_ICP_API int mi_icp_debug_search_skip(mi_icp_ctx* ctx, double* state2, double* limits_out, int64_t capacity,
                                        int64_t* npackets, int* armed);
MI_ICP_API int mi_icp_debug_locate(mi_icp_ctx* ctx, const float* T, int32_t* leaf_out);
MI_ICP_API int mi_icp_debug_set_step_stamps(mi_icp_ctx* ctx, int enable);
MI_ICP_API int mi_icp_debug_get_step_stamps(mi_icp_ctx* ctx, uint64_t* out32, double* ticks_per_us);
MI_ICP_API int mi_icp_debug_solve_both(int device, const double* systems, int n, float det_thresh,
                                       float* out_serial, float* out_wave, int32_t* ok_serial, int32_t* ok_wave);
MI_ICP_API int mi_icp_debug_eigen3(int device, const float* A, int64_t n, float* eval, float* evec, float* S);
MI_ICP_API int mi_icp_debug_odometry_image(mi_icp_ctx* ctx, int level, int which, float* out, int* width, int* height);
MI_ICP_API int mi_icp_debug_get_tree(mi_icp_ctx* ctx, int64_t* info5, float* records_out,
                                     float* leaf_lines_out);
MI_ICP_API int mi_icp_debug_get_leaf_regions(mi_icp_ctx* ctx, float* regions_out);
MI_ICP_API int mi_icp_debug_get_leaf_halos(mi_icp_ctx* ctx, float* halos_out);
#ifdef __cplusplus
}
#endif
#endif
```

Measured before the change: 10220 iterations/s.

## Cache per-packet paired target records for stable correspondences in pt2pl reduction

Adds a per-packet pair-state machine (0/1/2) with a contiguous tpair buffer that stores the gathered target vertex and normal for each source point once its correspondence has stayed unchanged for a packet. The NN search clears the state whenever any index in a packet changes. The point-to-plane reduction then reads the coalesced cached records instead of doing random trec gathers. This is meant to remove the scattered gather traffic in the reduction on later ICP iterations. In exchange it adds about 24 bytes per point of extra memory, extra writes when packets are promoted, and extra state-read latency.

Measured after the change: 10650 iterations/s, median of 6. +4.2%, better.

```diff
diff --git a/cupoch_amd/_lib.py b/cupoch_amd/_lib.py
--- a/cupoch_amd/_lib.py
+++ b/cupoch_amd/_lib.py
@@ -198,6 +198,8 @@
     "mi_icp_debug_occupancy": (_I, [_I]),
     "mi_icp_debug_loop_counters": (_I, [_P, _P]),
     "mi_icp_debug_search_skip": (_I, [_P, _P, _P, _L, C.POINTER(_L), C.POINTER(_I)]),
+    "mi_icp_debug_pair_state": (_I, [_P, _P, _P, _L, C.POINTER(_L)]),
+    "mi_icp_debug_drop_pairs": (_I, [_P]),
     "mi_icp_debug_locate": (_I, [_P, _P, _P]),
     "mi_icp_debug_set_step_stamps": (_I, [_P, _I]),
     "mi_icp_debug_get_step_stamps": (_I, [_P, _P, C.POINTER(C.c_double)]),
diff --git a/cupoch_amd/csrc/ctx.h b/cupoch_amd/csrc/ctx.h
--- a/cupoch_amd/csrc/ctx.h
+++ b/cupoch_amd/csrc/ctx.h
@@ -69,6 +69,9 @@
     mi::eng::DevBuf expiry;
     bool expiry_live = false;
     float skip_r2 = NAN;
+    mi::eng::DevBuf pair_state, pair_mask, tpair;
+    bool pairs_on = false;
+    bool pairs_live = false;
     mi::eng::DevBuf src_bounds;
     mi::eng::Relocation relocate;
 
@@ -226,11 +229,17 @@
     return MI_ICP_OK;
 }
 
-inline int drop_expiry(mi_icp_ctx* c) {
+inline int drop_pairs(mi_icp_ctx* c) {
+    if (c->pairs_live && c->pair_state.p) HIPCHK(c, hipMemsetAsync(c->pair_state.p, 0, c->pair_state.bytes, c->stream));
+    c->pairs_live = false;
+    return MI_ICP_OK;
+}
+
+inline int drop_expiry(mi_icp_ctx* c, bool keep_pairs = false) {
     c->skip_r2 = NAN;
     if (c->expiry_live && c->expiry.p) HIPCHK(c, hipMemsetAsync(c->expiry.p, 0xff, c->expiry.bytes, c->stream));
     c->expiry_live = false;
-    return MI_ICP_OK;
+    return keep_pairs ? MI_ICP_OK : drop_pairs(c);
 }
 
 static_assert(sizeof(DevLoop::live) == kSkipSamples, "loop_policy.h skip_pays reads DevLoop::live[]");
diff --git a/cupoch_amd/csrc/mi_build.hip b/cupoch_amd/csrc/mi_build.hip
--- a/cupoch_amd/csrc/mi_build.hip
+++ b/cupoch_amd/csrc/mi_build.hip
@@ -455,8 +455,12 @@
     TRY(ensure(c, c->nn_d2, (size_t)n, &d2));
     {
         double* lim;
+        uint8_t* pst;
+        uint64_t* pmask;
         TRY(ensure(c, c->expiry, (size_t)((n + 63) / 64), &lim));
-        c->expiry_live = true;
+        TRY(ensure(c, c->pair_state, (size_t)((n + 63) / 64), &pst));
+        TRY(ensure(c, c->pair_mask, (size_t)((n + 63) / 64), &pmask));
+        c->expiry_live = c->pairs_live = true;
         TRY(drop_expiry(c));
     }
     if (d_nrm) TRY(ensure(c, c->snrm, (size_t)n, &snrm));
diff --git a/cupoch_amd/csrc/mi_debug.hip b/cupoch_amd/csrc/mi_debug.hip
--- a/cupoch_amd/csrc/mi_debug.hip
+++ b/cupoch_amd/csrc/mi_debug.hip
@@ -134,7 +134,7 @@
 
 int mi_icp_debug_occupancy(int which) {
     if (which == 0 || which == 4) return occupancy_build(which);
-    if (which >= 1 && which <= 3) return occupancy_loop(which);
+    if ((which >= 1 && which <= 3) || which == 9) return occupancy_loop(which);
     if (which >= 5 && which <= 8) return occupancy_geometry(which);
     return -1;
 }
@@ -217,6 +217,25 @@
     return MI_ICP_OK;
 }
 
+int mi_icp_debug_pair_state(mi_icp_ctx* c, uint8_t* state_out, uint64_t* mask_out, int64_t capacity, int64_t* n_out) {
+    TRY(check_ctx(c));
+    if (!n_out || capacity < 0) return fail(c, MI_ICP_ERR_INVALID, "debug_pair_state: bad arguments");
+    if (c->ns <= 0 || !c->pair_state.p || !c->pair_mask.p) return fail(c, MI_ICP_ERR_STATE, "debug_pair_state: no source set");
+    const int64_t n = (c->ns + 63) / 64;
+    *n_out = n;
+    if (capacity >= n) {
+        if (state_out) HIPCHK(c, hipMemcpyAsync(state_out, c->pair_state.p, (size_t)n, hipMemcpyDeviceToHost, c->stream));
+        if (mask_out) HIPCHK(c, hipMemcpyAsync(mask_out, c->pair_mask.p, (size_t)n * sizeof(uint64_t), hipMemcpyDeviceToHost, c->stream));
+    }
+    HIPCHK(c, hipStreamSynchronize(c->stream));
+    return MI_ICP_OK;
+}
+
+int mi_icp_debug_drop_pairs(mi_icp_ctx* c) {
+    TRY(check_ctx(c));
+    return drop_pairs(c);
+}
+
 int mi_icp_debug_locate(mi_icp_ctx* c, const float* T, int32_t* leaf_out) {
     TRY(check_ctx(c));
     if (!leaf_out || c->ns <= 0 || c->nt <= 0) return fail(c, MI_ICP_ERR_INVALID, "debug_locate: bad state/arguments");
diff --git a/cupoch_amd/csrc/mi_icp.hip b/cupoch_amd/csrc/mi_icp.hip
--- a/cupoch_amd/csrc/mi_icp.hip
+++ b/cupoch_amd/csrc/mi_icp.hip
@@ -34,7 +34,7 @@
     locate_by_planes<<<grid, 256, 0, c->stream>>>((const float*)c->sx.p, (const float*)c->sy.p, (const float*)c->sz.p, (int)c->ns,
                                                  (const float2*)c->cell_planes.p, c->cell_levels, (const uint32_t*)c->cell_gstart.p,
                                                  (const float2*)c->gplanes.p, (uint32_t)c->nleaf, X, loop, gated, (int32_t*)c->nn_idx.p,
-                                                 (double*)c->expiry.p);
+                                                 (double*)c->expiry.p, (uint8_t*)c->pair_state.p);
     KCHK(c);
     return MI_ICP_OK;
 }
@@ -88,7 +88,8 @@
     EvTimer t(c, 0, loop != nullptr);
     const SearchPlan p = plan_search(loop != nullptr, seed, c->nn_valid, stats != nullptr, c->ns, coarse_first_min(), have_halo, planes_available(c),
                                      c->expiry.p != nullptr, c->expiry_live, c->skip_r2, r2, c->loop_host->live, kSkipRun);
-    if (!p.may_skip) TRY(drop_expiry(c));
+    const bool pairs_stand = loop != nullptr && c->pairs_on && p.use_seed && !stats && c->pair_state.p != nullptr;
+    if (!p.may_skip) TRY(drop_expiry(c, pairs_stand));
     if (p.self_seeded) TRY(launch_locate_by_planes(c, X, loop, 0));
     c->last_search_kind = p.kind;
     const PacketGrid g = packet_grid(c->ns, p.run);
@@ -97,7 +98,8 @@
             (const float*)c->tblk.p, (const float*)lreg_of(c), have_halo ? (const float*)c->thalo.p : nullptr, c->leaf_first,
             X, loop, r2, g.nblocks, idx, loop ? nullptr : (float*)c->nn_d2.p, stats, want,
             p.limits ? (double*)c->expiry.p : nullptr,
-            p.limits ? reinterpret_cast<uint8_t*>(c->loop_dev.p) + offsetof(DevLoop, live) : nullptr, skip_live_shift(c->ns), p.run);
+            p.limits ? reinterpret_cast<uint8_t*>(c->loop_dev.p) + offsetof(DevLoop, live) : nullptr, skip_live_shift(c->ns), p.run,
+            pairs_stand ? (uint8_t*)c->pair_state.p : nullptr);
     KCHK(c);
     if (p.limits) c->expiry_live = true, c->skip_r2 = r2;
     c->nn_valid = true;
@@ -110,7 +112,8 @@
     hipError_t e = hipErrorInvalidValue;
     if (which == 1) e = hipOccupancyMaxActiveBlocksPerMultiprocessor(&blocks, nn_packet_kernel<true, false>, kNNThreads, 0);
     else if (which == 2) e = hipOccupancyMaxActiveBlocksPerMultiprocessor(&blocks, nn_packet_kernel<false, false>, kNNThreads, 0);
-    else if (which == 3) e = hipOccupancyMaxActiveBlocksPerMultiprocessor(&blocks, reduce_pt2pl_kernel<2, 1>, kReduceThreads, 0);
+    else if (which == 3) e = hipOccupancyMaxActiveBlocksPerMultiprocessor(&blocks, reduce_pt2pl_kernel<2, 1, false, true>, kReduceThreads, 0);
+    else if (which == 9) e = hipOccupancyMaxActiveBlocksPerMultiprocessor(&blocks, reduce_pt2pl_kernel<4, 1, false, true>, kReduceThreads, 0);
     else return -1;
     return e == hipSuccess ? blocks : -2;
 }
@@ -169,13 +172,16 @@
     return MI_ICP_OK;
 }
 
+bool pt2pl_inputs(const mi_icp_ctx* c, int est, int mode) {
+    return est == kEstPt2Pl && mode == 0 && estimator_ready(c, est) && c->t_has_rec && c->trec.p != nullptr && c->ns > 0 && c->nt > 0;
+}
 bool pt2pl_reduction(const mi_icp_ctx* c, int est, int mode) {
-    return est == kEstPt2Pl && mode == 0 && estimator_ready(c, est) && c->n_user_pairs < 0 && c->t_has_rec &&
-           c->trec.p != nullptr && c->ns > 0 && c->nt > 0 && c->nn_valid;
+    return pt2pl_inputs(c, est, mode) && c->n_user_pairs < 0 && c->nn_valid;
 }
 
 template <int kU>
-decltype(&reduce_pt2pl_kernel<kU, 0>) pt2pl_kernel(int step, bool stamp) {
+decltype(&reduce_pt2pl_kernel<kU, 0>) pt2pl_kernel(int step, bool stamp, bool pairs) {
+    if (pairs) return step == 2 ? reduce_pt2pl_kernel<kU, 2, false, true> : (step == 1 ? reduce_pt2pl_kernel<kU, 1, false, true> : reduce_pt2pl_kernel<kU, 0, false, true>);
     if (step == 2) return stamp ? reduce_pt2pl_kernel<kU, 2, true> : reduce_pt2pl_kernel<kU, 2>;
     if (step == 1) return stamp ? reduce_pt2pl_kernel<kU, 1, true> : reduce_pt2pl_kernel<kU, 1>;
     return reduce_pt2pl_kernel<kU, 0>;
@@ -230,10 +236,13 @@
             wide, std::min<int64_t>(kReduceBlocks, blocks_for(a.count, kReduceThreads * kReduceElemsPerThread)));
     const Xform X = make_xform(T);
     if (pt2pl_reduction(c, est, mode)) {
-        const auto kernel = (a.count >= kPt2PlTwoFrom) ? pt2pl_kernel<2>(step, c->stamps_on) : pt2pl_kernel<4>(step, c->stamps_on);
+        const bool pairs = loop != nullptr && c->pairs_on && !c->stamps_on && c->tpair.p != nullptr;
+        const auto kernel = (a.count >= kPt2PlTwoFrom) ? pt2pl_kernel<2>(step, c->stamps_on, pairs) : pt2pl_kernel<4>(step, c->stamps_on, pairs);
+        const PairArgs pr = pairs ? PairArgs{(uint8_t*)c->pair_state.p, (uint64_t*)c->pair_mask.p, (float2*)c->tpair.p} : PairArgs{};
+        if (pairs) c->pairs_live = true;
         EvTimer t(c, 1, loop != nullptr);
         kernel<<<std::min(grid, 512), kReduceThreads, 0, c->stream>>>(a, X, loop, partial, ticket, sys,
-                                                                     (step == 2) ? mail_args(c) : MailArgs{});
+                                                                     (step == 2) ? mail_args(c) : MailArgs{}, pr);
         KCHK(c);
         return MI_ICP_OK;
     }
@@ -323,7 +332,7 @@
     comm_release(c);
     DevBuf* all[] = {&c->trec, &c->tidx, &c->thalo, &c->tlinks_tmp, &c->halo_want, &c->loop_hist, &c->tblk, &c->tnrm, &c->tcov, &c->tgrad, &c->sint, &c->nodes, &c->inv_t, &c->cell_planes, &c->cell_samples, &c->cell_cstart,
                      &c->cell_gstart, &c->sx, &c->sy, &c->sz,
-                     &c->sperm, &c->snrm, &c->scov, &c->nn_idx, &c->nn_d2, &c->expiry, &c->inv_s,
+                     &c->sperm, &c->snrm, &c->scov, &c->nn_idx, &c->nn_d2, &c->expiry, &c->pair_state, &c->pair_mask, &c->tpair, &c->inv_s,
                      &c->user_pairs, &c->keys0, &c->keys1, &c->vals0, &c->vals1, &c->hist,
                      &c->scan_tmp, &c->bounds_part, &c->bounds, &c->partial, &c->sys_dev,
                      &c->dense_idx, &c->flags, &c->pairs_out, &c->seg_start, &c->loop_dev, &c->ticket, &c->mail_state, &c->alt[0],
@@ -769,6 +778,22 @@
     TRY(ensure(c, c->loop_dev, 1, &d));
     HIPCHK(c, hipMemcpyAsync(d, &L, sizeof(DevLoop), hipMemcpyHostToDevice, c->stream));
     c->loop_active = true;
+    c->pairs_on = false;
+    if (pt2pl_inputs(c, est, 0) && c->ns > kFusedMax && c->pair_state.p != nullptr) {
+        const size_t bytes = (size_t)((c->ns + 63) / 64) * 64 * kPairPlanes * sizeof(float2);
+        if (c->tpair.bytes < bytes) {
+            void* grown = nullptr;
+            if (hipMalloc(&grown, bytes) == hipSuccess) {
+                if (c->tpair.p) HIPCHK(c, hipStreamSynchronize(c->stream));
+                release(c->tpair);
+                c->tpair.p = grown;
+                c->tpair.bytes = bytes;
+            } else {
+                (void)hipGetLastError();
+            }
+        }
+        c->pairs_on = c->tpair.p != nullptr && c->tpair.bytes >= bytes;
+    }
     c->halo.on_loop_begin();
     {
         uint32_t* want;
diff --git a/cupoch_amd/csrc/nn_search.h b/cupoch_amd/csrc/nn_search.h
--- a/cupoch_amd/csrc/nn_search.h
+++ b/cupoch_amd/csrc/nn_search.h
@@ -155,7 +155,8 @@
         int ns, const float* __restrict__ records_g, const float* __restrict__ tblk_g,
         const float* __restrict__ lreg_g, const float* __restrict__ halo_g, uint32_t leaf_first, Xform Tv, const DevLoop* __restrict__ loop, float r2, int32_t* __restrict__ nn_idx,
         float* __restrict__ nn_d2, unsigned long long* __restrict__ stats, uint32_t* __restrict__ want, PacketResult& out,
-        double* __restrict__ expiry = nullptr, uint8_t* __restrict__ live = nullptr, uint32_t live_shift = 0u) {
+        double* __restrict__ expiry = nullptr, uint8_t* __restrict__ live = nullptr, uint32_t live_shift = 0u,
+        uint8_t* __restrict__ pair_state = nullptr) {
     const int lane = lane_id();
     const bool limits = SEED && !STATS && loop != nullptr && expiry != nullptr && nn_d2 == nullptr;
     const int i = (int)(packet * 64u) + lane;
@@ -433,7 +434,10 @@
     }
 
     if (valid) {
-        if (!SEED || bidx != seed_j) nn_idx[i] = bidx;
+        if (!SEED || bidx != seed_j) {
+            nn_idx[i] = bidx;
+            if (SEED && pair_state != nullptr) pair_state[packet] = 0;
+        }
         if (nn_d2) nn_d2[i] = (bidx >= 0) ? best : INFINITY;
     }
     if (STATS && lane == 0) {
@@ -463,7 +467,7 @@
         int ns, const float* __restrict__ records_g, const float* __restrict__ tblk_g,
         const float* __restrict__ lreg_g, const float* __restrict__ halo_g, uint32_t leaf_first, Xform Tv, const DevLoop* __restrict__ loop, float r2, uint32_t nblocks, int32_t* __restrict__ nn_idx,
         float* __restrict__ nn_d2, unsigned long long* __restrict__ stats, uint32_t* __restrict__ want,
-        double* __restrict__ expiry, uint8_t* __restrict__ live, uint32_t live_shift, uint32_t run) {
+        double* __restrict__ expiry, uint8_t* __restrict__ live, uint32_t live_shift, uint32_t run, uint8_t* __restrict__ pair_state) {
     __shared__ PacketShared s_pk[kNNPacketsPerBlock];
     uint32_t logical;
     if (!xcd_remap(nblocks, logical)) return;
@@ -472,7 +476,7 @@
     if (STAMP && stamps && threadIdx.x == 0 && blockIdx.x < 64u) atomicMin(stamps + 0, stamp_now());
     if (!GATE) {
         (void)nn_packet_body<SEED, STATS>(s_pk[0], logical, sx, sy, sz, ns, records_g, tblk_g, lreg_g, halo_g, leaf_first, Tv, loop,
-                                          r2, nn_idx, nn_d2, stats, want, unused, expiry, live, live_shift);
+                                          r2, nn_idx, nn_d2, stats, want, unused, expiry, live, live_shift, pair_state);
     } else {
         const uint32_t npackets = ((uint32_t)ns + 63u) >> 6, lane = (uint32_t)lane_id();
         const uint32_t first = logical * run;
@@ -484,7 +488,7 @@
             const uint32_t k = (uint32_t)__builtin_ctz(need);
             need &= need - 1u;
             (void)nn_packet_body<true, false>(s_pk[0], first + k, sx, sy, sz, ns, records_g, tblk_g, lreg_g, halo_g, leaf_first, Xform{},
-                                              loop, r2, nn_idx, nullptr, nullptr, want, unused, expiry, live, live_shift);
+                                              loop, r2, nn_idx, nullptr, nullptr, want, unused, expiry, live, live_shift, pair_state);
             __builtin_amdgcn_wave_barrier();
         }
     }
@@ -495,7 +499,7 @@
         const float* __restrict__ sx, const float* __restrict__ sy, const float* __restrict__ sz, int ns,
         const float2* __restrict__ cell_planes, int cell_levels, const uint32_t* __restrict__ gstart,
         const float2* __restrict__ gplanes, uint32_t nleaf, Xform Tv, const DevLoop* __restrict__ loop, int gated,
-        int32_t* __restrict__ nn_idx, double* __restrict__ expiry) {
+        int32_t* __restrict__ nn_idx, double* __restrict__ expiry, uint8_t* __restrict__ pair_state) {
     Xform T = Tv;
     if (loop) {
         if (loop->done) return;
@@ -510,6 +514,7 @@
         const uint32_t leaf = min(g * 512u + descend_group(gplanes + (size_t)g * 512u, qx, qy, qz), nleaf - 1u);
         nn_idx[i] = (int32_t)(leaf * (uint32_t)kLeaf);
         if (expiry != nullptr && (i & 63) == 0) expiry[i >> 6] = -(double)INFINITY;
+        if (pair_state != nullptr && (i & 63) == 0) pair_state[i >> 6] = 0;
     }
 }
 
diff --git a/cupoch_amd/csrc/reduce.h b/cupoch_amd/csrc/reduce.h
--- a/cupoch_amd/csrc/reduce.h
+++ b/cupoch_amd/csrc/reduce.h
@@ -406,54 +406,181 @@
     block_finish(acc, partial, ticket, out32);
 }
 
-template <int kU, int STEP, bool STAMP = false>
+struct PairArgs {
+    uint8_t* state;
+    uint64_t* mask;
+    float2* tpair;
+};
+constexpr int kPairPlanes = 3;
+
+template <int kU>
+__device__ __forceinline__ void pt2pl_pair_sums(const ReduceArgs& a, const PairArgs& pr, const DevLoop* loop, Xform& T,
+                                                bool& finished, double* acc) {
+    const int64_t stride = (int64_t)gridDim.x * kReduceThreads;
+    const int64_t k0 = (int64_t)blockIdx.x * kReduceThreads + threadIdx.x;
+    const int64_t trip = stride * kU;
+    const int64_t npackets = (a.count + 63) >> 6;
+    const int lane = lane_id();
+    uint8_t* __restrict__ const state = pr.state;
+    uint64_t* __restrict__ const mask = pr.mask;
+    float2* __restrict__ const tpair = pr.tpair;
+    constexpr uint32_t kNone = 3u;
+    uint32_t st[kU], st_raw[kU], st_far[kU];
+    int32_t j[kU];
+    uint64_t m[kU];
+    float px[kU], py[kU], pz[kU];
+    float2 rec[kU][kPairPlanes];
+    auto ask = [&](int64_t kb, uint32_t* raw) {
+#pragma unroll
+        for (int u = 0; u < kU; ++u) {
+            const int64_t p = (kb + (int64_t)u * stride) >> 6;
+            raw[u] = state[p < npackets ? p : 0];
+        }
+    };
+    auto settle = [&](int64_t kb, const uint32_t* raw, uint32_t* s) {
+#pragma unroll
+        for (int u = 0; u < kU; ++u) {
+            const int64_t p = (kb + (int64_t)u * stride) >> 6;
+            s[u] = (uint32_t)__builtin_amdgcn_readfirstlane((int)((p < npackets) ? raw[u] : kNone));
+        }
+    };
+    auto fetch = [&](int64_t kb) {
+#pragma unroll
+        for (int u = 0; u < kU; ++u) {
+            const int64_t k = kb + (int64_t)u * stride;
+            const int64_t kc = (k < a.count) ? k : 0;
+            const bool paired = st[u] == 2u;
+            px[u] = a.sx[kc];
+            py[u] = a.sy[kc];
+            pz[u] = a.sz[kc];
+            j[u] = a.nn_idx[paired ? 0 : kc];
+            m[u] = mask[paired ? (k >> 6) : 0];
+            const float2* rp = tpair + (paired ? (k >> 6) * (kPairPlanes * 64) + lane : 0);
+#pragma unroll
+            for (int q = 0; q < kPairPlanes; ++q) rec[u][q] = rp[paired ? q * 64 : 0];
+        }
+    };
+    ask(k0, st_raw);
+    ask(k0 + trip, st_far);
+    settle(k0, st_raw, st);
+    fetch(k0);
+    if (loop) {
+        if (loop->done) {
+            finished = true;
+            return;
+        }
+        T = loop->X;
+    }
+    for (int64_t kb = k0; kb < a.count; kb += trip) {
+        uint32_t now[kU];
+#pragma unroll
+        for (int u = 0; u < kU; ++u) {
+            now[u] = st[u];
+            st_raw[u] = st_far[u];
+        }
+        float vt[kU][3], nt[kU][3];
+        bool have[kU];
+#pragma unroll
+        for (int u = 0; u < kU; ++u) {
+            const bool inside = (kb + (int64_t)u * stride) < a.count;
+            if (now[u] == 2u) {
+                have[u] = inside && ((m[u] >> lane) & 1ull) != 0ull;
+                vt[u][0] = rec[u][0].x;
+                vt[u][1] = rec[u][0].y;
+                vt[u][2] = rec[u][1].x;
+                nt[u][0] = rec[u][1].y;
+                nt[u][1] = rec[u][2].x;
+                nt[u][2] = rec[u][2].y;
+            } else {
+                have[u] = inside && j[u] >= 0;
+                trec_gather(a.trec, have[u] ? j[u] : 0, vt[u], nt[u]);
+            }
+        }
+        float vs[kU][3];
+#pragma unroll
+        for (int u = 0; u < kU; ++u) xform_point(T, px[u], py[u], pz[u], vs[u][0], vs[u][1], vs[u][2]);
+        settle(kb + trip, st_raw, st);
+        ask(kb + 2 * trip, st_far);
+        fetch(kb + trip);
+#pragma unroll
+        for (int u = 0; u < kU; ++u)
+            if (have[u]) pt2pl_rows<0>(acc, vs[u], vt[u], nt[u]);
+#pragma unroll
+        for (int u = 0; u < kU; ++u) {
+            const int64_t p = (kb + (int64_t)u * stride) >> 6;
+            if (now[u] == 1u) {
+                float2* wp = tpair + p * (kPairPlanes * 64) + lane;
+                wp[0] = make_float2(vt[u][0], vt[u][1]);
+                wp[64] = make_float2(vt[u][2], nt[u][0]);
+                wp[128] = make_float2(nt[u][1], nt[u][2]);
+                const uint64_t b = __ballot(have[u]);
+                if (lane == 0) {
+                    mask[p] = b;
+                    state[p] = 2;
+                }
+            } else if (now[u] == 0u) {
+                if (lane == 0) state[p] = 1;
+            }
+        }
+    }
+}
+
+template <int kU, int STEP, bool STAMP = false, bool PAIRS = false>
 __global__ __launch_bounds__(kReduceThreads) void reduce_pt2pl_kernel(ReduceArgs a, Xform Tv,
                                                                       DevLoop* __restrict__ loop,
                                                                       double* __restrict__ partial,
                                                                       uint32_t* __restrict__ ticket,
-                                                                      double* __restrict__ out32, MailArgs mail) {
+                                                                      double* __restrict__ out32, MailArgs mail, PairArgs pr) {
     const int64_t stride = (int64_t)gridDim.x * kReduceThreads;
     const int64_t k0 = (int64_t)blockIdx.x * kReduceThreads + threadIdx.x;
-    int32_t j[kU];
-    float px[kU], py[kU], pz[kU];
-    auto fetch = [&](int64_t kb) {
-#pragma unroll
-        for (int u = 0; u < kU; ++u) {
-            const int64_t k = kb + (int64_t)u * stride;
-            const int64_t kc = (k < a.count) ? k : 0;
-            j[u] = a.nn_idx[kc];
-            px[u] = a.sx[kc];
-            py[u] = a.sy[kc];
-            pz[u] = a.sz[kc];
-        }
-    };
-    fetch(k0);
     Xform T = Tv;
     unsigned long long* stamps = nullptr;
-    if (loop) {
-        if (loop->done) return;
-        T = loop->X;
-        if (STAMP) stamps = reinterpret_cast<unsigned long long*>(loop->stamps);
-    }
-    if (STAMP && stamps && threadIdx.x == 0) atomicMin(stamps + 2, stamp_now());
     double acc[30];
-#pragma unroll
-    for (int k = 0; k < 30; ++k) acc[k] = 0.0;
-    for (int64_t kb = k0; kb < a.count; kb += stride * kU) {
-        float vt[kU][3], nt[kU][3];
-        bool have[kU];
-#pragma unroll
-        for (int u = 0; u < kU; ++u) {
-            have[u] = (kb + (int64_t)u * stride) < a.count && j[u] >= 0;
-            trec_gather(a.trec, have[u] ? j[u] : 0, vt[u], nt[u]);
-        }
-        float vs[kU][3];
-#pragma unroll
-        for (int u = 0; u < kU; ++u) xform_point(T, px[u], py[u], pz[u], vs[u][0], vs[u][1], vs[u][2]);
-        fetch(kb + stride * kU);
-#pragma unroll
-        for (int u = 0; u < kU; ++u)
-            if (have[u]) pt2pl_rows<0>(acc, vs[u], vt[u], nt[u]);
+    if (PAIRS) {
+#pragma unroll
+        for (int k = 0; k < 30; ++k) acc[k] = 0.0;
+        bool finished = false;
+        pt2pl_pair_sums<kU>(a, pr, loop, T, finished, acc);
+        if (finished) return;
+    } else {
+        int32_t j[kU];
+        float px[kU], py[kU], pz[kU];
+        auto fetch = [&](int64_t kb) {
+#pragma unroll
+            for (int u = 0; u < kU; ++u) {
+                const int64_t k = kb + (int64_t)u * stride;
+                const int64_t kc = (k < a.count) ? k : 0;
+                j[u] = a.nn_idx[kc];
+                px[u] = a.sx[kc];
+                py[u] = a.sy[kc];
+                pz[u] = a.sz[kc];
+            }
+        };
+        fetch(k0);
+        if (loop) {
+            if (loop->done) return;
+            T = loop->X;
+            if (STAMP) stamps = reinterpret_cast<unsigned long long*>(loop->stamps);
+        }
+        if (STAMP && stamps && threadIdx.x == 0) atomicMin(stamps + 2, stamp_now());
+#pragma unroll
+        for (int k = 0; k < 30; ++k) acc[k] = 0.0;
+        for (int64_t kb = k0; kb < a.count; kb += stride * kU) {
+            float vt[kU][3], nt[kU][3];
+            bool have[kU];
+#pragma unroll
+            for (int u = 0; u < kU; ++u) {
+                have[u] = (kb + (int64_t)u * stride) < a.count && j[u] >= 0;
+                trec_gather(a.trec, have[u] ? j[u] : 0, vt[u], nt[u]);
+            }
+            float vs[kU][3];
+#pragma unroll
+            for (int u = 0; u < kU; ++u) xform_point(T, px[u], py[u], pz[u], vs[u][0], vs[u][1], vs[u][2]);
+            fetch(kb + stride * kU);
+#pragma unroll
+            for (int u = 0; u < kU; ++u)
+                if (have[u]) pt2pl_rows<0>(acc, vs[u], vt[u], nt[u]);
+        }
     }
     StepPre pre{STEP != 0, 0u, 0.0, 0u};
     const bool last = block_finish(acc, partial, ticket, out32, &pre, STEP ? loop : nullptr,
diff --git a/cupoch_amd/engine.py b/cupoch_amd/engine.py
--- a/cupoch_amd/engine.py
+++ b/cupoch_amd/engine.py
@@ -227,6 +227,17 @@
         with np.errstate(invalid="ignore"):
             will = (st[0] + st[1] < lim) if armed.value else np.zeros(n.value, bool)
         return {"travel": float(st[0]), "fuzz": float(st[1]), "limits": lim, "armed": bool(armed.value), "will_skip": will}
+
+    def pair_state(self):
+        n = C.c_int64(0)
+        self._chk(self._L.mi_icp_debug_pair_state(self._ctx, None, None, 0, C.byref(n)))
+        st, mk = np.zeros(n.value, np.uint8), np.zeros(n.value, np.uint64)
+        self._chk(self._L.mi_icp_debug_pair_state(self._ctx, st.ctypes.data_as(C.c_void_p), mk.ctypes.data_as(C.c_void_p),
+                                                  n.value, C.byref(n)))
+        return {"state": st, "mask": mk}
+
+    def drop_pairs(self):
+        self._chk(self._L.mi_icp_debug_drop_pairs(self._ctx))
 
     def last_search_kind(self):
         return int(self._L.mi_icp_debug_last_search_kind(self._ctx))
diff --git a/include/mi_icp_debug.h b/include/mi_icp_debug.h
--- a/include/mi_icp_debug.h
+++ b/include/mi_icp_debug.h
@@ -21,6 +21,9 @@
 MI_ICP_API int mi_icp_debug_loop_counters(mi_icp_ctx* ctx, int32_t* out4);
 MI_ICP_API int mi_icp_debug_search_skip(mi_icp_ctx* ctx, double* state2, double* limits_out, int64_t capacity,
                                         int64_t* npackets, int* armed);
+MI_ICP_API int mi_icp_debug_pair_state(mi_icp_ctx* ctx, uint8_t* state_out, uint64_t* mask_out, int64_t capacity,
+                                       int64_t* n_out);
+MI_ICP_API int mi_icp_debug_drop_pairs(mi_icp_ctx* ctx);
 MI_ICP_API int mi_icp_debug_locate(mi_icp_ctx* ctx, const float* T, int32_t* leaf_out);
 MI_ICP_API int mi_icp_debug_set_step_stamps(mi_icp_ctx* ctx, int enable);
 MI_ICP_API int mi_icp_debug_get_step_stamps(mi_icp_ctx* ctx, uint64_t* out32, double* ticks_per_us);
```
